# maksimt/rri_nmf

Hardware: NVIDIA B200
Metric: RRI sweeps/sec (higher is better)
Workload: dtype f32/tf32-mma

## Files before the change

### rri_nmf_b200/csrc/api.cu

```cuda
#include <dlfcn.h>
#include <stdarg.h>
#include <stdio.h>
#include <string.h>

#include <string>
#include <vector>

#include "../../include/rri_b200.h"
#include "gemm_tf32_sm100.h"
#include "common.cuh"
#include "devmem.h"
#include "kernels.h"
#include "wrri_tc_sm100.h"

using namespace rri;

static thread_local char g_err[1024] = "";
static int fail(const char* fmt, ...)
{
    va_list ap;
    va_start(ap, fmt);
    vsnprintf(g_err, sizeof(g_err), fmt, ap);
    va_end(ap);
    return 1;
}
#define CK(call)                                                                                \
    do {                                                                                        \
        cudaError_t e_ = (call);                                                                \
        if (e_ != cudaSuccess)                                                                  \
            return fail("%s failed: %s (%s:%d)", #call, cudaGetErrorString(e_), __FILE__, __LINE__); \
    } while (0)
#define CKL() CK(cudaGetLastError())

extern "C" const char* rri_last_error(void) { return g_err; }
extern "C" const char* rri_version(void) { return "rri_b200 0.1 (sm_100a; tcgen05 tf32 + simt f32/f64)"; }

struct Id128 { char b[128]; };
struct NcclApi {
    void* lib = nullptr;
    int (*AllReduce)(const void*, void*, size_t, int, int, void*, cudaStream_t) = nullptr;
    int (*GetUniqueId)(void*) = nullptr;
    int (*CommInitRank)(void**, int,  Id128, int) = nullptr;
    int (*CommDestroy)(void*) = nullptr;
    const char* (*GetErrorString)(int) = nullptr;
};
static NcclApi g_nccl;

static int nccl_load(const char* path)
{
    if (g_nccl.lib) return 0;
    void* lib = nullptr;
    if (path && *path) lib = dlopen(path, RTLD_NOW | RTLD_GLOBAL);
    if (!lib) lib = dlopen("libnccl.so.2", RTLD_NOW | RTLD_GLOBAL);
    if (!lib) return fail("cannot load NCCL (%s): %s", path ? path : "libnccl.so.2", dlerror());
    g_nccl.AllReduce = (decltype(g_nccl.AllReduce))dlsym(lib, "ncclAllReduce");
    g_nccl.GetUniqueId = (decltype(g_nccl.GetUniqueId))dlsym(lib, "ncclGetUniqueId");
    g_nccl.CommInitRank = (decltype(g_nccl.CommInitRank))dlsym(lib, "ncclCommInitRank");
    g_nccl.CommDestroy = (decltype(g_nccl.CommDestroy))dlsym(lib, "ncclCommDestroy");
    g_nccl.GetErrorString = (decltype(g_nccl.GetErrorString))dlsym(lib, "ncclGetErrorString");
    if (!g_nccl.AllReduce || !g_nccl.GetUniqueId || !g_nccl.CommInitRank || !g_nccl.CommDestroy)
        return fail("NCCL symbols missing in %s", path ? path : "libnccl.so.2");
    g_nccl.lib = lib;
    return 0;
}
#define NCK(call)                                                                                \
    do {                                                                                         \
        int r_ = (call);                                                                         \
        if (r_ != 0)                                                                             \
            return fail("%s failed: %s", #call, g_nccl.GetErrorString ? g_nccl.GetErrorString(r_) : "?"); \
    } while (0)

extern "C" int rri_nccl_unique_id(char id_out[128], const char* nccl_lib_path)
{
    if (nccl_load(nccl_lib_path)) return 1;
    NCK(g_nccl.GetUniqueId(id_out));
    return 0;
}
extern "C" int rri_nccl_comm_create(void** comm_out, const char id[128], int32_t rank, int32_t world,
                                    int32_t device, const char* nccl_lib_path)
{
    if (nccl_load(nccl_lib_path)) return 1;
    CK(cudaSetDevice(device));
    Id128 u;
    memcpy(u.b, id, 128);
    NCK(g_nccl.CommInitRank(comm_out, world, u, rank));
    return 0;
}
extern "C" int rri_nccl_comm_destroy(void* comm)
{
    if (!g_nccl.lib) return fail("NCCL not loaded");
    NCK(g_nccl.CommDestroy(comm));
    return 0;
}

struct PeerGroup {
    bool used = false;
    int device = -1, world = 0, rank = 0;
    void* xbuf = nullptr; size_t bytes = 0;
    void* peer_base[16] = {nullptr}; bool peer_open[16] = {false};
    char handles[16 * 64] = {0};
    bool mapped = false;
    unsigned epoch = 0;
};


struct rri_handle_s {
    int64_t n = 0, d = 0;
    int k = 0, dtype = 0, math = 0, order = 0, device = 0, sm_count = 148;
    size_t es = 4;
    const void* X = nullptr; int64_t ldx = 0;
    const void* M = nullptr; int mk = 0; int64_t ldm = 0;
    void* comm = nullptr; int rank = 0, world = 1;
    void* xbuf = nullptr; size_t xbuf_bytes = 0, xslot_elems = 0;
    size_t x_off_tt = 0, x_off_tk = 0, x_off_tsum = 0, x_off_flags = 0;
    int64_t ldtk = 0;
    void* peer_base[16] = {nullptr}; bool peer_open[16] = {false};
    void* Tt_own = nullptr;
    unsigned epoch = 0;
    bool p2p = false, peer_mapped = false;
    int* p2p_err = nullptr;
    char handles[16 * 64] = {0};
    PeerGroup parked; bool have_parked = false;
    unsigned* counters = nullptr;
    std::vector<void*> allocs;
    int64_t ws_bytes = 0, launches = 0;
    PassPlan pp{};
    int hb = 0, gbw = 0;
    void *ypart = nullptr, *ppart = nullptr, *gpart = nullptr, *hpart = nullptr, *stat = nullptr;
    void *Xt = nullptr; int64_t ldxt = 0, ldwt = 0;
    void* Xt_ext = nullptr; int64_t ldxt_ext = 0;
    bool x16 = false; int x_exp = 0;
    void *X16 = nullptr, *Xt16 = nullptr; int64_t ldx16 = 0, ldxt16 = 0;
    void* F16 = nullptr;
    unsigned *x16_scan = nullptr, *f16_part = nullptr; int* f16_exp = nullptr;
    void *Wt = nullptr, *Tt = nullptr, *Cpart = nullptr, *cg = nullptr , *Hm = nullptr;
    void *gram_part = nullptr, *colsum_part = nullptr;
    int splits_t = 1, splits_w = 1, ub_blocks_t = 1, ub_blocks_w = 1, gchunks_w = 1, gchunks_t = 1;
    double* sx_slots = nullptr;
    Tf32Gemm* tf32 = nullptr;
    bool fixT_cached = false;
    TilePlan tpl{}, wpl{};
    void *numer_part = nullptr, *denom_part = nullptr, *mstat = nullptr;
    WrriTc* wtc = nullptr; int wtc_groups_t = 1, wtc_groups_w = 1;
    bool sparse = false; int64_t nnz = 0;
    SpSide csr{}, csc{};
    void *sp_quad = nullptr;
    void *sp_told = nullptr;
    void *sp_wold = nullptr;
    void *sp_npart = nullptr, *sp_dpart = nullptr;
    uint32_t* sp_perm = nullptr;
    int sp_ldt = 0;
    bool sp_refresh_v2 = true;
    bool sp_batched_sums = true;
    int* sp_err = nullptr;
    bool zero_csr = false;
    SpmmPlan zrow{}, zcol{};
    SparsePassPlan spp{};
    bool spmm_planned = false;
    void* spmm_slots = nullptr; int spmm_slot_w = 0;
    double* sums = nullptr;
    int* flags = nullptr;
    double *obj_part = nullptr, *obj_out = nullptr;
    int oblocks = 1;
    bool xsq_valid = false, c2_valid = false;
    void* Gobj = nullptr;
};

static int ws_alloc(rri_handle_t h, void** p, size_t bytes)
{
    if (bytes == 0) bytes = 16;
    CK(cached_malloc(p, bytes));
    CK(cudaMemsetAsync(*p, 0, bytes, 0));
    h->allocs.push_back(*p);
    h->ws_bytes += (int64_t)bytes;
    return 0;
}

static void ws_release(rri_handle_t h, void* p, size_t bytes)
{
    if (bytes == 0) bytes = 16;
    for (size_t i = 0; i < h->allocs.size(); ++i)
        if (h->allocs[i] == p) { h->allocs.erase(h->allocs.begin() + (long)i); break; }
    cached_free(p);
    h->ws_bytes -= (int64_t)bytes;
}

extern "C" int rri_create(rri_handle_t* out, int64_t n_local, int64_t d, int32_t k, int32_t dtype,
                          int32_t math, int32_t order, int32_t device)
{
    if (!out) return fail("null handle pointer");
    if (n_local <= 0 || d <= 0) return fail("n_local and d must be positive (got %lld, %lld)", (long long)n_local, (long long)d);
    if (k <= 0 || k > 256) return fail("k must be in [1,256] (got %d)", k);
    if (dtype != RRI_F32 && dtype != RRI_F64) return fail("bad dtype %d", dtype);
    if (order != RRI_ORDER_RRI && order != RRI_ORDER_HALS) return fail("bad order %d", order);
    if (math != RRI_MATH_IEEE && math != RRI_MATH_TF32) return fail("bad math %d", math);
    if (math == RRI_MATH_TF32 && dtype != RRI_F32) return fail("TF32 math needs f32 data");
    int ndev = 0;
    cudaError_t e = cudaGetDeviceCount(&ndev);
    if (e != cudaSuccess || ndev == 0)
        return fail("no CUDA device available (%s); this library has no CPU fallback", cudaGetErrorString(e));
    if (device < 0 || device >= ndev) return fail("bad device %d", device);
    CK(cudaSetDevice(device));
    cudaDeviceProp prop;
    CK(cudaGetDeviceProperties(&prop, device));
    if (prop.major != 10)
        return fail("device %d is sm_%d%d; this build contains sm_100a code only", device, prop.major, prop.minor);
    rri_handle_t h = new rri_handle_s();
    h->n = n_local; h->d = d; h->k = k; h->dtype = dtype; h->math = math; h->order = order;
    h->device = device; h->sm_count = prop.multiProcessorCount;
    h->es = dtype == RRI_F32 ? 4 : 8;
    if (ws_alloc(h, (void**)&h->sums, sizeof(double) * 2 * k) || ws_alloc(h, (void**)&h->flags, sizeof(int) * 4) ||
        ws_alloc(h, (void**)&h->counters, sizeof(unsigned) * 8)) {
        rri_destroy(h);
        return 1;
    }
    cudaStreamSynchronize(0);
    *out = h;
    return 0;
}

static void peer_release(rri_handle_t h);

extern "C" int rri_destroy(rri_handle_t h)
{
    if (!h) return 0;
    cudaSetDevice(h->device);
    cudaDeviceSynchronize();
    peer_release(h);
    for (void* p : h->allocs) cached_free(p);
    if (h->tf32) tf32_gemm_destroy(h->tf32);
    if (h->wtc) wrri_tc_destroy(h->wtc);
    delete h;
    return 0;
}

extern "C" int rri_set_comm(rri_handle_t h, void* nccl_comm, int32_t rank, int32_t world, const char* nccl_lib_path)
{
    if (!h) return fail("null handle");
    if (world > 1) {
        if (!nccl_comm) return fail("world > 1 needs a communicator");
        if (nccl_load(nccl_lib_path)) return 1;
    }
    h->comm = nccl_comm; h->rank = rank; h->world = world;
    return 0;
}

static size_t round_up(size_t v, size_t a) { return (v + a - 1) / a * a; }

static PeerGroup g_groups[64];

static PeerGroup* group_take(int device, size_t bytes)
{
    for (PeerGroup& g : g_groups)
        if (g.used && g.device == device && g.bytes == bytes) { g.used = false; return &g; }
    return nullptr;
}
static PeerGroup* group_slot()
{
    for (PeerGroup& g : g_groups) if (!g.used) return &g;
    return nullptr;
}

static bool peer_rank_supported(rri_handle_t h)
{
    return h->dtype == RRI_F32 ? h->k <= 128 : h->k <= 64;
}

extern "C" int rri_peer_export(rri_handle_t h, char handle_out[64])
{
    if (!h) return fail("null handle");
    if (!h->X) return fail("rri_bind has not been called");
    if (h->order != RRI_ORDER_HALS || h->mk != MK_NONE) return fail("the peer-memory exchange serves unmasked hals handles");
    if (h->zero_csr) return fail("the peer-memory exchange serves dense data; zero-filled sparse handles use the NCCL all-reduce");
    if (!peer_rank_supported(h)) return fail("the fused peer-memory T update supports k <= 128 (f32) / 64 (f64)");
    CK(cudaSetDevice(h->device));
    if (!h->xbuf) {
        const size_t es = h->es;
        const int64_t v = 16 / (int64_t)es;
        h->ldtk = (h->d + v - 1) / v * v;
        h->xslot_elems = ((size_t)h->d * h->k + (size_t)h->k * h->k + 63) / 64 * 64;
        h->x_off_tt = round_up(2 * h->xslot_elems * es, 256);
        h->x_off_tk = round_up(h->x_off_tt + (size_t)h->d * h->k * es, 256);
        h->x_off_tsum = round_up(h->x_off_tk + (size_t)h->k * h->ldtk * es, 256);
        h->x_off_flags = round_up(h->x_off_tsum + (size_t)16 * h->k * es, 256);
        h->xbuf_bytes = h->x_off_flags + 2 * 16 * 32 * sizeof(unsigned);
        if (PeerGroup* g = group_take(h->device, h->xbuf_bytes)) {
            h->xbuf = g->xbuf;
// ... 60 lines not shown
    if (!h->xbuf) return;
    if (h->have_parked) {
        if (PeerGroup* g = group_slot()) { *g = h->parked; g->used = true; h->xbuf = nullptr; h->have_parked = false; return; }
    }
    PeerGroup* g = group_slot();
    if (g) {
        g->used = true; g->device = h->device; g->world = h->world; g->rank = h->rank;
        g->xbuf = h->xbuf; g->bytes = h->xbuf_bytes; g->mapped = h->peer_mapped; g->epoch = h->epoch;
        for (int r = 0; r < 16; ++r) { g->peer_base[r] = h->peer_base[r]; g->peer_open[r] = h->peer_open[r]; }
        memcpy(g->handles, h->handles, sizeof(g->handles));
    } else {
        for (int r = 0; r < 16; ++r)
            if (h->peer_open[r] && h->peer_base[r]) cudaIpcCloseMemHandle(h->peer_base[r]);
        cudaFree(h->xbuf);
    }
    h->xbuf = nullptr; h->peer_mapped = false;
    for (int r = 0; r < 16; ++r) { h->peer_open[r] = false; h->peer_base[r] = nullptr; }
}

extern "C" int rri_peer_close(rri_handle_t h)
{
    if (!h) return fail("null handle");
    CK(cudaSetDevice(h->device));
    h->p2p = false;
    if (h->Tt_own) { h->Tt = h->Tt_own; h->Tt_own = nullptr; }
    peer_release(h);
    return 0;
}

extern "C" int rri_peer_enable(rri_handle_t h, int32_t on)
{
    if (!h) return fail("null handle");
    if (on && !h->peer_mapped) return fail("rri_peer_import has not succeeded on this rank");
    h->p2p = on != 0;
    if (h->p2p) {
        if (!h->Tt_own) h->Tt_own = h->Tt;
        h->Tt = (char*)h->xbuf + h->x_off_tt;
    } else if (h->Tt_own) {
        h->Tt = h->Tt_own; h->Tt_own = nullptr;
    }
    return 0;
}

static void peer_row_range(int64_t d, int world, int r, int64_t& lo, int64_t& hi)
{
    const int64_t nb = (d + 127) / 128;
    const int64_t q = nb / world, rem = nb % world;
    const int64_t b0 = q * r + (r < rem ? r : rem), b1 = b0 + q + (r < rem ? 1 : 0);
    lo = b0 * 128 < d ? b0 * 128 : d;
    hi = b1 * 128 < d ? b1 * 128 : d;
}

static PeerExchange peer_args(rri_handle_t h, unsigned epoch)
{
    PeerExchange px;
    memset(&px, 0, sizeof(px));
    px.world = h->world; px.rank = h->rank; px.epoch = epoch; px.ldtk = h->ldtk; px.err = h->p2p_err;
    peer_row_range(h->d, h->world, h->rank, px.row_lo, px.row_hi);
    const int b = (int)(epoch & 1u);
    for (int r = 0; r < h->world; ++r) {
        char* base = (char*)h->peer_base[r];
        px.part[r] = base + (size_t)b * h->xslot_elems * h->es;
        px.Tt[r] = base + h->x_off_tt;
        px.Tk[r] = base + h->x_off_tk;
        px.tsum[r] = base + h->x_off_tsum;
        px.flag1[r] = (unsigned*)(base + h->x_off_flags);
        px.flag2[r] = (unsigned*)(base + h->x_off_flags) + 16 * 32;
    }
    return px;
}

static int allreduce(rri_handle_t h, void* buf, size_t count, cudaStream_t st)
{
    if (h->world <= 1) return 0;
    NCK(g_nccl.AllReduce(buf, buf, count, h->dtype == RRI_F32 ? 7 : 8,  0, h->comm, st));
    h->launches++;
    return 0;
}

static int alloc_halfstep_ws(rri_handle_t h)
{
    const int64_t n = h->n, d = h->d;
    const int k = h->k;
    const size_t es = h->es;
    const size_t a = (size_t)h->splits_w * n * k, b = (size_t)h->splits_t * d * k;
    if (ws_alloc(h, &h->Cpart, es * (a > b ? a : b))) return 1;
    const int64_t m = n > d ? n : d;
    if (ws_alloc(h, &h->cg, es * ((size_t)m * k + (size_t)k * k))) return 1;
    if (ws_alloc(h, &h->Hm, es * (size_t)k * k)) return 1;
    {
        const int64_t v = 16 / (int64_t)es;
        h->ldwt = (n + v - 1) / v * v;
    }
    if (ws_alloc(h, &h->Wt, es * (size_t)k * h->ldwt) || ws_alloc(h, &h->Tt, es * (size_t)d * k)) return 1;
    h->gchunks_w = gram_chunks(n, k, h->sm_count);
    h->gchunks_t = gram_chunks(d, k, h->sm_count);
    const int gc = h->gchunks_w > h->gchunks_t ? h->gchunks_w : h->gchunks_t;
    if (ws_alloc(h, &h->gram_part, es * (size_t)gc * k * k)) return 1;
    h->ub_blocks_w = update_rows_blocks(n, h->sm_count);
    h->ub_blocks_t = update_rows_blocks(d, h->sm_count);
    int ubm = h->ub_blocks_w > h->ub_blocks_t ? h->ub_blocks_w : h->ub_blocks_t;
    {
        const int pb = peer_update_blocks(d, h->sm_count);
        if (pb > ubm) ubm = pb;
    }
    if (ws_alloc(h, &h->colsum_part, es * (size_t)ubm * k)) return 1;
    if (h->order == RRI_ORDER_HALS && ws_alloc(h, (void**)&h->sx_slots, sizeof(double) * (size_t)simplex_T_slots(d))) return 1;
    return 0;
}

template <typename T>
static int bind_impl(rri_handle_t h, cudaStream_t st)
{
    const int64_t n = h->n, d = h->d;
    const int k = h->k, ks = k + 1;
    const size_t es = sizeof(T);
    h->oblocks = obj_blocks(n, d, h->sm_count);
    if (!h->obj_part) {
        size_t op = 2 * (size_t)(h->oblocks > 256 ? h->oblocks : 256);
        if (op < (size_t)8 * h->sm_count) op = (size_t)8 * h->sm_count;
        if (ws_alloc(h, (void**)&h->obj_part, sizeof(double) * op)) return 1;
        if (ws_alloc(h, (void**)&h->obj_out, sizeof(double) * 16)) return 1;
    }
    if (h->mk != MK_NONE) {
        if (!h->numer_part) {
            h->tpl = plan_tstats(n, d, h->sm_count);
            h->wpl = plan_wstats(n, d, h->sm_count);
            size_t a = (size_t)h->tpl.groups * d, b = (size_t)h->wpl.groups * n;
            if (h->math == RRI_MATH_TF32) {
                std::string err;
                h->wtc = wrri_tc_create(h->sm_count, n, d, k, err);
                if (!h->wtc) return fail("tensor-core WRRI path unavailable: %s", err.c_str());
                h->wtc_groups_t = wrri_tc_groups(h->wtc, 0);
                h->wtc_groups_w = wrri_tc_groups(h->wtc, 1);
                const size_t a2 = (size_t)h->wtc_groups_t * d, b2 = (size_t)h->wtc_groups_w * n;
                if (a2 > a) a = a2;
                if (b2 > b) b = b2;
            }
            const size_t m = a > b ? a : b;
            if (ws_alloc(h, &h->numer_part, es * m) || ws_alloc(h, &h->denom_part, es * m)) return 1;
            if (ws_alloc(h, &h->mstat, es * 2 * (size_t)d)) return 1;
        }
        return 0;
    }
    if (!h->Cpart) {
        h->splits_w = simt_gemm_splits(n, d, h->sm_count);
        h->splits_t = simt_gemm_splits(d, n, h->sm_count);
        if (h->math == RRI_MATH_TF32) { h->splits_w = 1; h->splits_t = 1; }
        if (alloc_halfstep_ws(h)) return 1;
        if (h->math == RRI_MATH_TF32) {
            std::string err;
            h->tf32 = tf32_gemm_create(h->sm_count, k + 16 < 256 ? k + 16 : 256, err);
            if (!h->tf32) return fail("tf32 contraction unavailable: %s", err.c_str());
            if (ws_alloc(h, (void**)&h->x16_scan, 4 * sizeof(unsigned)) || ws_alloc(h, (void**)&h->f16_exp, sizeof(int)) ||
                ws_alloc(h, (void**)&h->f16_part, sizeof(unsigned) * (size_t)f16_factor_parts(h->sm_count)))
                return 1;
            CK(cudaStreamSynchronize(0));
        }
    }
    if (h->order == RRI_ORDER_HALS) {
        const int64_t v = 16 / (int64_t)es;
        h->ldxt = (n + v - 1) / v * v;
        const int64_t ldx16 = (d + 7) / 8 * 8, ldxt16 = (n + 7) / 8 * 8;
        const size_t bytes16 = 2 * ((size_t)n * ldx16 + (size_t)d * ldxt16);
        size_t cap;
        if (h->Xt_ext) {
            if (h->ldxt_ext < h->ldxt || h->ldxt_ext % v != 0 || (reinterpret_cast<uintptr_t>(h->Xt_ext) & 15) != 0)
                return fail("caller-provided X' storage needs a 16-byte aligned base and a row stride >= %lld, multiple of %lld",
                            (long long)h->ldxt, (long long)v);
            h->Xt = h->Xt_ext; h->ldxt = h->ldxt_ext;
            cap = es * (size_t)d * h->ldxt;
        } else {
            cap = es * (size_t)d * h->ldxt > bytes16 ? es * (size_t)d * h->ldxt : bytes16;
            if (!h->Xt) {
                CK(cached_malloc(&h->Xt, cap));
                h->allocs.push_back(h->Xt);
                h->ws_bytes += (int64_t)cap;
            }
        }
        const char* ev = getenv("RRI_X16");
        h->x16 = false;
        if (h->math == RRI_MATH_TF32 && !(ev && *ev == '0') && bytes16 <= cap) {
            launch_x16_scan((const float*)h->X, n, d, h->ldx, h->x16_scan, h->sm_count, st);
            h->launches++;
            unsigned scan[3];
            CK(cudaMemcpyAsync(scan, h->x16_scan, sizeof(scan), cudaMemcpyDeviceToHost, st));
            CK(cudaStreamSynchronize(st));
            h->x16 = x16_exponent(scan, &h->x_exp);
        }
        if (h->x16) {
            if (!h->F16) {
                const int64_t m = n > d ? n : d;
                const int rows = k + 16 < 256 ? k + 16 : 256;
                if (ws_alloc(h, &h->F16, 2 * (size_t)rows * (size_t)((m + 7) / 8 * 8))) return 1;
                CK(cudaStreamSynchronize(0));
            }
            h->X16 = h->Xt; h->ldx16 = ldx16;
            h->Xt16 = (char*)h->Xt + 2 * (size_t)n * ldx16; h->ldxt16 = ldxt16;
            launch_x16_copy((const float*)h->X, n, d, h->ldx, h->x_exp, h->X16, ldx16, h->Xt16, ldxt16, st);
        } else {
            launch_transpose<T>((const T*)h->X, n, d, h->ldx, (T*)h->Xt, h->ldxt, st);
        }
        h->launches++;
        CKL();
    } else {
        h->pp = plan_pass(n, d, h->ldx, h->X, (int)es, h->sm_count);
        h->hb = tstep_blocks(d);
        h->gbw = wstep_blocks(n, h->sm_count);
        if (!h->ypart) {
            if (ws_alloc(h, &h->ypart, es * (size_t)h->pp.ct * n)) return 1;
            if (ws_alloc(h, &h->ppart, es * (size_t)h->pp.rg * d)) return 1;
            if (ws_alloc(h, &h->gpart, es * (size_t)h->gbw * ks)) return 1;
            if (ws_alloc(h, &h->hpart, es * (size_t)h->hb * ks)) return 1;
            if (ws_alloc(h, &h->stat, es * (size_t)(d + ks))) return 1;
        }
    }
    return 0;
}

extern "C" int rri_set_transpose_storage(rri_handle_t h, void* Xt_dev, int64_t ldXt)
{
    if (!h) return fail("null handle");
    if (h->X) return fail("rri_set_transpose_storage must be called before rri_bind");
    h->Xt_ext = Xt_dev; h->ldxt_ext = ldXt;
    return 0;
}

extern "C" int rri_bind(rri_handle_t h, const void* X_dev, int64_t ldX, const void* mask_dev,
                        int32_t mask_kind, int64_t ldM, void* stream)
{
    if (!h) return fail("null handle");
    if (!X_dev) return fail("X is null");
    if (ldX < h->d) return fail("ldX (%lld) < d (%lld)", (long long)ldX, (long long)h->d);
    if (mask_kind != RRI_MASK_NONE && !mask_dev) return fail("mask kind %d without a mask pointer", mask_kind);
    if (mask_kind != RRI_MASK_NONE && ldM < h->d) return fail("ldM < d");
    if (mask_kind < 0 || mask_kind > 2) return fail("bad mask kind %d", mask_kind);
    if (h->sparse) return fail("this handle is bound to observed-entries (CSR) data; create a new one for dense data");
    if (h->zero_csr) return fail("this handle is bound to zero-filled sparse (CSR) data; create a new one for dense data");
    if (h->X && ((h->mk != MK_NONE) != (mask_kind != RRI_MASK_NONE)))
        return fail("a handle cannot switch between masked and unmasked data; create a new one");
    CK(cudaSetDevice(h->device));
    h->X = X_dev; h->ldx = ldX;
    h->M = mask_kind == RRI_MASK_NONE ? nullptr : mask_dev;
    h->mk = mask_kind; h->ldm = ldM;
    h->fixT_cached = false;
    h->xsq_valid = false; h->c2_valid = false;
    cudaStream_t st = (cudaStream_t)stream;
    int rc = h->dtype == RRI_F32 ? bind_impl<float>(h, st) : bind_impl<double>(h, st);
    if (rc) return rc;
    CK(cudaStreamSynchronize(0));
    return 0;
}

template <typename T>
static int bind_csr_impl(rri_handle_t h, const int64_t* rowptr, const int32_t* col, const T* val, const T* wgt,
                         cudaStream_t st)
{
    const int64_t n = h->n, d = h->d, nnz = h->nnz;
    const int k = h->k;
    const size_t es = sizeof(T);
    const int64_t m = n > d ? n : d;
    const size_t ne = (size_t)(nnz > 0 ? nnz : 1);
    void *E_csr = nullptr, *E_csc = nullptr, *x_csc = nullptr, *w_csc = nullptr, *csc_row = nullptr, *colptr = nullptr;
    if (ws_alloc(h, (void**)&h->obj_part, sizeof(double) * 2 * 256) || ws_alloc(h, (void**)&h->obj_out, sizeof(double) * 8)) return 1;
    if (ws_alloc(h, &E_csr, es * ne) || ws_alloc(h, &E_csc, es * ne) || ws_alloc(h, &x_csc, es * ne)) return 1;
    if (wgt && ws_alloc(h, &w_csc, es * ne)) return 1;
    if (ws_alloc(h, &csc_row, sizeof(int32_t) * ne) || ws_alloc(h, &colptr, sizeof(int64_t) * (size_t)(d + 1))) return 1;
    if (ws_alloc(h, &h->sp_quad, 4 * es * (size_t)m) || ws_alloc(h, &h->sp_told, es * 2 * (size_t)d) ||
        ws_alloc(h, &h->sp_wold, es * 2 * (size_t)n) || ws_alloc(h, &h->mstat, es * 2 * (size_t)m) ||
        ws_alloc(h, (void**)&h->sp_err, sizeof(int)))
        return 1;
    {
        const int64_t v = 16 / (int64_t)es;
        h->ldwt = (n + v - 1) / v * v;
    }
    {
        const char* env = getenv("RRI_SP_REFRESH_V2");
        h->sp_refresh_v2 = !(env && *env == '0');
        const char* envb = getenv("RRI_SP_BATCHED_SUMS");
        h->sp_batched_sums = !(envb && *envb == '0');
        const int v = 16 / (int)es;
        h->sp_ldt = h->sp_refresh_v2 ? (k + v - 1) / v * v : k;
    }
    if (ws_alloc(h, &h->Wt, es * (size_t)k * h->ldwt) || ws_alloc(h, &h->Tt, es * (size_t)d * h->sp_ldt)) return 1;
    if (ws_alloc(h, (void**)&h->sp_perm, sizeof(uint32_t) * ne)) return 1;
    CK(cudaStreamSynchronize(0));
    const int rc = sp_build_csc<T>(rowptr, col, val, wgt, n, d, nnz, (int64_t*)colptr, (int32_t*)csc_row, (T*)x_csc,
                                   (T*)w_csc, h->sp_perm, h->sm_count, h->sp_err, st);
    if (rc < 0)
        return fail("malformed CSR input:%s%s%s", (-rc & 1) ? " rowptr is not a monotone [0..nnz] sequence;" : "",
                    (-rc & 2) ? " column index outside [0,d);" : "",
                    (-rc & 4) ? " column indices must be strictly ascending inside every row (sort and merge duplicates);" : "");
    if (rc > 0) return fail("building the column orientation failed: %s", cudaGetErrorString((cudaError_t)rc));
    h->csr = SpSide{n, rowptr, col, val, wgt, E_csr, nnz / n >= 512 ? 256 : 32, nullptr, 1, 0, d, nullptr};
    h->csc = SpSide{d, (const int64_t*)colptr, (const int32_t*)csc_row, x_csc, w_csc, E_csc, nnz / d >= 512 ? 256 : 32,
                    nullptr, 1, 0, n, nullptr};
    h->launches += 8;
    const char* env = getenv("RRI_SP_BLOCKED");
    const bool blocked = !(env && *env == '0');
    const char* env16 = getenv("RRI_SP_IDX16");
    const bool use16 = !(env16 && *env16 == '0');
    size_t part_elems = (size_t)m;
    for (SpSide* sd : {&h->csr, &h->csc}) {
        int nblk = 1;
        const int nb = sp_block_len((int)es, sd->nother, &nblk);
        if (!blocked || nblk > 64) continue;
        void* p2 = nullptr;
        void* i16 = nullptr;
        if (ws_alloc(h, &p2, sizeof(int64_t) * (size_t)sd->nseg * (size_t)(nblk + 1))) return 1;
        if (use16 && ws_alloc(h, &i16, sizeof(uint16_t) * ne)) return 1;
        CK(cudaStreamSynchronize(0));
        launch_sp_subptr(sd->ptr, sd->idx, sd->nseg, nblk, nb, (int64_t*)p2, h->sm_count, st);
        if (use16 && nnz > 0) {
            launch_sp_local_index(sd->idx, nnz, nb, (uint16_t*)i16, h->sm_count, st);
            sd->idx16 = (const uint16_t*)i16;
            h->launches++;
        }
        sd->ptr2 = (const int64_t*)p2; sd->nblk = nblk; sd->nb = nb;
        if ((size_t)nblk * (size_t)sd->nseg > part_elems) part_elems = (size_t)nblk * (size_t)sd->nseg;
        h->launches++;
    }
    if (ws_alloc(h, &h->sp_npart, es * part_elems) || ws_alloc(h, &h->sp_dpart, es * part_elems)) return 1;
    CK(cudaStreamSynchronize(0));
    CKL();
    CK(cudaStreamSynchronize(st));
    return 0;
}

extern "C" int rri_bind_csr(rri_handle_t h, int64_t nnz, const int64_t* rowptr_dev, const int32_t* col_dev,
                            const void* val_dev, const void* weight_dev, void* stream)
{
    if (!h) return fail("null handle");
    if (h->X) return fail("the handle is already bound; create a new one");
    if (nnz < 0 || nnz >= ((int64_t)1 << 31)) return fail("nnz must be in [0, 2^31) (got %lld)", (long long)nnz);
    if (!rowptr_dev) return fail("rowptr is null");
    if (nnz > 0 && (!col_dev || !val_dev)) return fail("col/val is null");
    if (h->math == RRI_MATH_TF32) return fail("the observed-entries path has no contraction: create the handle with RRI_MATH_IEEE");
    CK(cudaSetDevice(h->device));
    h->nnz = nnz;
    cudaStream_t st = (cudaStream_t)stream;
    const int rc = h->dtype == RRI_F32
                       ? bind_csr_impl<float>(h, rowptr_dev, col_dev, (const float*)val_dev, (const float*)weight_dev, st)
                       : bind_csr_impl<double>(h, rowptr_dev, col_dev, (const double*)val_dev, (const double*)weight_dev, st);
    if (rc) return rc;
    h->sparse = true;
    h->mk = MK_SPARSE;
    h->X = val_dev ? val_dev : (const void*)rowptr_dev;
// ... 141 lines not shown
            CK(cudaStreamSynchronize(0));
            h->spmm_slot_w = pw;
        }
        pl.slots = h->spmm_slots;
    }
    launch_spmm<T>(pl, B, ldb, width, C, ldc, st);
    h->launches += (width + SPMM_PANEL - 1) / SPMM_PANEL;
    CKL();
    return 0;
}

extern "C" int rri_spmm(rri_handle_t h, int32_t transpose, const void* B_dev, int64_t ldb, void* C_dev, int64_t ldc,
                        int32_t width, void* stream)
{
    if (!h) return fail("null handle");
    if (!h->X) return fail("rri_bind_csr / rri_bind_csr_zero has not been called");
    if (!h->sparse && !h->zero_csr)
        return fail("rri_spmm serves sparse handles (rri_bind_csr or rri_bind_csr_zero); this handle holds dense data");
    if (transpose != 0 && transpose != 1) return fail("transpose must be 0 or 1 (got %d)", transpose);
    if (width < 1) return fail("width must be at least 1 (got %d)", width);
    if (!B_dev || !C_dev) return fail("B and C must not be null");
    if (ldb < width || ldc < width)
        return fail("ldb and ldc must be at least width = %d (got %lld, %lld)", width, (long long)ldb, (long long)ldc);
    if (ldb >= ((int64_t)1 << 31) || ldc >= ((int64_t)1 << 31)) return fail("ldb and ldc must be below 2^31");
    if (((uintptr_t)B_dev % h->es) || ((uintptr_t)C_dev % h->es))
        return fail("B and C must be aligned to their %d-byte elements", (int)h->es);
    CK(cudaSetDevice(h->device));
    cudaStream_t st = (cudaStream_t)stream;
    return h->dtype == RRI_F32 ? spmm_impl<float>(h, transpose, (const float*)B_dev, ldb, (float*)C_dev, ldc, width, st)
                               : spmm_impl<double>(h, transpose, (const double*)B_dev, ldb, (double*)C_dev, ldc, width, st);
}

static SolveArgs solve_args(const rri_params_t* p, bool forT)
{
    SolveArgs a;
    a.reg_l1 = forT ? p->reg_t_l1 : p->reg_w_l1;
    a.reg_l2 = forT ? p->reg_t_l2 : p->reg_w_l2;
    a.eps = p->eps;
    const double ub = forT ? p->ub_t : p->ub_w;
    a.has_ub = ub > 0 ? 1 : 0;
    a.ub = ub > 0 ? ub : 0.0;
    return a;
}

static int check_params(rri_handle_t h, const rri_params_t* p)
{
    if (!p) return fail("null params");
    if (!h->X) return fail("rri_bind has not been called");
    if (p->fix_W && p->fix_T) return fail("fix_W and fix_T both set: nothing to update");
    if (p->fix_W) return fail("fix_W=True is not supported on the device path (the reference's T-only sweep also rescales W, nmf.py:450-452)");
    if (p->simplex_T && !(p->ub_t > 0)) return fail("simplex_T needs t_row_sum > 0");
    return 0;
}

template <typename T>
static void rri_pass(rri_handle_t h, const T* tvec, const T* W, int tn, bool do_y, bool do_p, cudaStream_t st)
{
    if (h->zero_csr)
        launch_sparse_rri_pass<T>(h->spp, h->zrow, h->zcol, tvec, W, h->k, tn, (T*)h->ypart, (T*)h->ppart, do_y, do_p, st);
    else
        launch_rri_pass<T>((const T*)h->X, h->ldx, h->n, h->d, tvec, W, h->k, tn, (T*)h->ypart, (T*)h->ppart, do_y, do_p,
                           h->pp, st);
    h->launches++;
}

template <typename T>
static int rri_prologue(rri_handle_t h, T* W, int t0, const rri_params_t* p, cudaStream_t st)
{
    rri_pass<T>(h, nullptr, W, t0, false, true, st);
    launch_rri_wstep<T>(W, h->n, h->k, 0, t0, (const T*)h->ypart, h->pp.ct, h->n, (const T*)h->hpart, h->hb,
                        solve_args(p, false), (T*)h->gpart, h->sums, h->flags, false, h->gbw, st);
    h->launches++;
    CKL();
    return 0;
}

template <typename T>
static int rri_finish(rri_handle_t h, int t_last, cudaStream_t st)
{
    if (h->world > 1) {
        launch_reduce_stat<T>((const T*)h->ppart, 0, 0, (const T*)h->gpart, h->gbw, h->k, (T*)h->stat, st);
        if (allreduce(h, h->stat, (size_t)(h->k + 1), st)) return 1;
        launch_finalize_sums<T>((const T*)h->stat, 1, h->k, t_last, h->sums, h->flags, st);
        h->launches += 2;
    } else {
        launch_finalize_sums<T>((const T*)h->gpart, h->gbw, h->k, t_last, h->sums, h->flags, st);
        h->launches++;
    }
    CKL();
    return 0;
}

template <typename T>
static int rri_topic_range(rri_handle_t h, T* W, T* Tm, int t0, int t1, bool first_has_prev,
                           const rri_params_t* p, cudaStream_t st)
{
    const int k = h->k;
    const int64_t n = h->n, d = h->d;
    const SolveArgs at = solve_args(p, true), aw = solve_args(p, false);
    for (int t = t0; t < t1; ++t) {
        const int tn = (t + 1) % k;
        const int t_prev = ((t == t0 && !first_has_prev) || k == 1) ? -1 : (t + k - 1) % k;
        const T* pp = (const T*)h->ppart; int rg = h->pp.rg;
        const T* gp = (const T*)h->gpart; int gb = h->gbw;
        if (h->world > 1) {
            launch_reduce_stat<T>(pp, rg, d, gp, gb, k, (T*)h->stat, st);
            h->launches++;
            if (allreduce(h, h->stat, (size_t)(d + k + 1), st)) return 1;
            pp = (const T*)h->stat; rg = 1;
            gp = (const T*)h->stat + d; gb = 1;
        }
        launch_rri_tstep<T>(Tm, d, k, t, pp, rg, d, gp, gb, at, (T*)h->hpart, h->sums, t_prev, h->flags, true, st);
        if (p->simplex_T) {
            launch_project_rows_simplex<T>(Tm + (int64_t)t * d, 1, d, p->ub_t, st);
            launch_rri_tstep<T>(Tm, d, k, t, pp, rg, d, gp, gb, at, (T*)h->hpart, h->sums, -1, h->flags, false, st);
            h->launches += 2;
        }
        rri_pass<T>(h, Tm + (int64_t)t * d, W, tn, true, k > 1, st);
        launch_rri_wstep<T>(W, n, k, t, tn, (const T*)h->ypart, h->pp.ct, n, (const T*)h->hpart, h->hb, aw,
                            (T*)h->gpart, h->sums, h->flags, true, h->gbw, st);
        h->launches += 2;
        if (k == 1) {
            if (rri_finish<T>(h, 0, st)) return 1;
            if (rri_prologue<T>(h, W, 0, p, st)) return 1;
        }
    }
    CKL();
    return 0;
}

template <typename T>
static int contraction(rri_handle_t h, const T* A, int64_t lda, const T* B, int64_t ldb, T* Cpart,
                       int64_t M, int N, int64_t K, int splits, cudaStream_t st, T* G = nullptr)
{
    if (h->math == RRI_MATH_TF32) {
        std::string err;
        int nl = tf32_gemm_run(h->tf32, (const float*)A, lda, (const float*)B, ldb, (float*)Cpart, N, M, N, K, st, err,
                               G ? (const float*)B : nullptr, ldb, G ? N : 0, (float*)G, N);
        if (nl < 0) return fail("tf32 contraction failed: %s", err.c_str());
        h->launches += nl;
    } else {
        launch_simt_gemm_nt<T>(A, lda, B, ldb, Cpart, M, N, K, splits, st);
        h->launches++;
    }
    return 0;
}

static bool gram_in_contraction(rri_handle_t h)
{
    static const bool off = [] { const char* e = getenv("RRI_TC_GRAM"); return e && *e == '0'; }();
    return h->math == RRI_MATH_TF32 && !off;
}

template <typename T>
static int data_contraction(rri_handle_t h, bool transpose, const T* B, int64_t ldb, int N, T* C, cudaStream_t st,
                            T* G = nullptr, bool convert = true)
{
    const int64_t M = transpose ? h->d : h->n, K = transpose ? h->n : h->d;
    if (!h->x16)
        return transpose ? contraction<T>(h, (const T*)h->Xt, h->ldxt, B, ldb, C, M, N, K, h->splits_t, st, G)
                         : contraction<T>(h, (const T*)h->X, h->ldx, B, ldb, C, M, N, K, h->splits_w, st, G);
    const int64_t ldf = (K + 7) / 8 * 8;
    if (convert) {
        launch_f16_factor((const float*)B, N, K, ldb, h->f16_part, f16_factor_parts(h->sm_count), h->F16, ldf, h->f16_exp, st);
        h->launches += 2;
    }
    const __half* F = (const __half*)h->F16;
    std::string err;
    const int nl = f16_gemm_run(h->tf32, (const __half*)(transpose ? h->Xt16 : h->X16), transpose ? h->ldxt16 : h->ldx16,
                                h->x_exp, F, ldf, h->f16_exp, (float*)C, N, M, N, K, st, err, G ? F : nullptr, ldf, G ? N : 0,
                                (float*)G, N);
    if (nl < 0) return fail("16-bit contraction failed: %s", err.c_str());
    h->launches += nl;
    return 0;
}

template <typename T>
static int hals_W_half(rri_handle_t h, T* W, const T* Tk, int64_t ldtk, const rri_params_t* p, bool recompute, cudaStream_t st)
{
    const int k = h->k;
    const int64_t n = h->n, d = h->d;
    if (recompute) {
        const bool tc_gram = gram_in_contraction(h);
        if (!tc_gram) { launch_gram<T>((const T*)h->Tt, d, k, (T*)h->gram_part, h->gchunks_t, (T*)h->Hm, st); h->launches += 2; }
        if (h->zero_csr) {
            launch_spmm<T>(h->zrow, (const T*)h->Tt, k, k, (T*)h->Cpart, k, st);
            h->launches++;
        } else if (data_contraction<T>(h, false, Tk, ldtk, k, (T*)h->Cpart, st, tc_gram ? (T*)h->Hm : nullptr)) {
            return 1;
        }
    }
    const int parts = h->math == RRI_MATH_TF32 ? 1 : h->splits_w;
    launch_update_rows<T>(W, n, k, (const T*)h->Cpart, parts, n * k, nullptr, (const T*)h->Hm, solve_args(p, false),
                          (T*)h->Wt, h->ldwt, (T*)h->colsum_part, h->flags, h->ub_blocks_w,
                          ColsumOut{nullptr, k, 0, h->counters + 0}, st);
    h->launches++;
    CKL();
    return 0;
}

template <typename T>
static int hals_T_half(rri_handle_t h, T* W, T* Tk, int64_t ldtk, const rri_params_t* p, cudaStream_t st)
{
    const int k = h->k;
    const int64_t n = h->n, d = h->d;
    T* cg = (T*)h->cg;
    T* G = cg + (size_t)d * k;
    const bool tc_gram = gram_in_contraction(h);
    const int psplits = h->math == RRI_MATH_TF32 ? 1 : h->splits_t;
    if (h->world > 1 && h->p2p && !p->simplex_T) {
        const unsigned e = ++h->epoch;
        const int b = (int)(e & 1u);
        T* myC = (T*)((char*)h->xbuf + (size_t)b * h->xslot_elems * h->es);
        T* myG = myC + (size_t)d * k;
        if (!tc_gram) { launch_gram<T>(W, n, k, (T*)h->gram_part, h->gchunks_w, myG, st); h->launches += 2; }
        T* Cdst = psplits == 1 ? myC : (T*)h->Cpart;
        if (data_contraction<T>(h, true, (const T*)h->Wt, h->ldwt, k, Cdst, st, tc_gram ? myG : nullptr)) return 1;
        if (psplits > 1) { launch_reduce_parts<T>((const T*)h->Cpart, psplits, d * k, d * k, myC, st); h->launches++; }
        const PeerExchange px = peer_args(h, e);
        const int blocks = peer_update_blocks(px.row_hi - px.row_lo, h->sm_count);
        const int nl = launch_peer_update_rows<T>(px, d, k, solve_args(p, true), G, (T*)h->colsum_part, h->flags, h->sums,
                                                  h->counters + 1, blocks, st);
        if (!nl) return fail("the fused peer-memory T update does not support k = %d", k);
        h->launches += nl;
        CKL();
        return 0;
    }
    if (!tc_gram) { launch_gram<T>(W, n, k, (T*)h->gram_part, h->gchunks_w, G, st); h->launches += 2; }
    T* Cout = (h->world > 1 && psplits == 1) ? cg : (T*)h->Cpart;
    if (h->zero_csr) {
        launch_spmm<T>(h->zcol, W, k, k, Cout, k, st);
        h->launches++;
    } else if (data_contraction<T>(h, true, (const T*)h->Wt, h->ldwt, k, Cout, st, tc_gram ? G : nullptr)) {
        return 1;
    }
    const T* C = Cout;
    int parts = psplits;
    if (h->world > 1) {
        if (psplits > 1) { launch_reduce_parts<T>(C, parts, d * k, d * k, cg, st); h->launches++; }
        if (allreduce(h, cg, (size_t)d * k + (size_t)k * k, st)) return 1;
        C = cg; parts = 1;
    }
    if (p->simplex_T) {
        const char* e = getenv("RRI_SIMPLEX_FUSED");
        int nl = 0;
        const int rc = launch_simplex_T_update<T>((T*)h->Tt, d, k, C, parts, d * k, G, solve_args(p, true), p->ub_t, Tk,
                                                  ldtk, h->sx_slots, h->flags, h->sm_count, !(e && *e == '0'), &nl, st);
        if (rc) return fail("constrained T update failed: %s", cudaGetErrorString((cudaError_t)rc));
        h->launches += nl;
        return 0;
    }
    launch_update_rows<T>((T*)h->Tt, d, k, C, parts, d * k, nullptr, G, solve_args(p, true), Tk, ldtk, (T*)h->colsum_part,
                          h->flags, h->ub_blocks_t, ColsumOut{nullptr, 0, 0, h->counters + 2}, st);
    h->launches++;
    CKL();
    return 0;
}

template <typename T>
static int hals_finish_sums(rri_handle_t h, const T* Tm, bool t_sums, cudaStream_t st)
{
    launch_rowsum_flag<T>((const T*)h->Wt, h->k, h->n, h->ldwt, h->sums, h->k, h->world > 1 ? 0 : 2, h->flags, st);
    h->launches++;
    if (t_sums) {
        launch_rowsum_flag<T>(Tm, h->k, h->d, h->d, h->sums, 0, 1, h->flags, st);
        h->launches++;
    }
    if (h->world <= 1) return 0;
    NCK(g_nccl.AllReduce(h->sums + h->k, h->sums + h->k, (size_t)h->k, 8, 0, h->comm, st));
    launch_flag_from_sums(h->sums, h->k, h->k, 2, h->flags, st);
    h->launches += 2;
    return 0;
}

template <typename T>
static void scale_row_to_sum(rri_handle_t h, T* row, T* row2, int64_t ld2, int t, const rri_params_t* p, cudaStream_t st)
{
    launch_vec_scale_to_sum<T>(row, h->d, 1, h->sums, t, p->ub_t, st);
    if (row2) { launch_vec_scale_to_sum<T>(row2, h->d, ld2, h->sums, t, p->ub_t, st); h->launches++; }
    launch_vec_sum_flag<T>(row, h->d, 1, h->sums, t, 1, h->flags, st);
    h->launches += 2;
}

template <typename T>
static int wrri_T_step(rri_handle_t h, T* W, T* Tm, int t, const rri_params_t* p, cudaStream_t st)
{
    const int64_t n = h->n, d = h->d;
    int parts = h->tpl.groups;
    if (h->wtc) {
        std::string err;
        parts = h->wtc_groups_t;
        if (wrri_tc_stats(h->wtc, 0, (const float*)h->X, h->ldx, h->M, h->mk, h->ldm, t, (const float*)Tm + (int64_t)t * d, (float*)h->numer_part,
                          (float*)h->denom_part, parts, st, err) < 0)
            return fail("tensor-core WRRI T statistics failed: %s", err.c_str());
    } else {
        launch_wrri_tstats<T>((const T*)h->X, h->ldx, h->M, h->mk, h->ldm, W, Tm, n, d, h->k, t, (T*)h->numer_part,
                              (T*)h->denom_part, h->tpl, st);
    }
    h->launches++;
    const T* nu = (const T*)h->numer_part; const T* de = (const T*)h->denom_part;
    if (h->world > 1) {
        T* ms = (T*)h->mstat;
        launch_reduce_parts<T>(nu, parts, d, d, ms, st);
        launch_reduce_parts<T>(de, parts, d, d, ms + d, st);
        h->launches += 2;
        if (allreduce(h, ms, (size_t)2 * d, st)) return 1;
        nu = ms; de = ms + d; parts = 1;
    }
    T* tp2 = h->wtc ? (T*)wrri_tc_Tp(h->wtc) + t : nullptr;
    launch_wrri_final<T>(nu, de, parts, d, solve_args(p, true), Tm + (int64_t)t * d, 1, tp2,
                         h->wtc ? wrri_tc_KP(h->wtc) : 0, h->flags, st);
    launch_vec_sum_flag<T>(Tm + (int64_t)t * d, d, 1, h->sums, t, p->simplex_T ? 0 : 1, h->flags, st);
    h->launches += 2;
    if (p->simplex_T) scale_row_to_sum<T>(h, Tm + (int64_t)t * d, tp2, h->wtc ? wrri_tc_KP(h->wtc) : 0, t, p, st);
    return 0;
}

template <typename T>
static int wrri_W_step(rri_handle_t h, T* W, T* Tm, int t, const rri_params_t* p, cudaStream_t st)
{
    const int64_t n = h->n, d = h->d;
    int parts = h->wpl.groups;
    if (h->wtc) {
        std::string err;
        parts = h->wtc_groups_w;
        if (wrri_tc_stats(h->wtc, 1, (const float*)h->X, h->ldx, h->M, h->mk, h->ldm, t, (const float*)Tm + (int64_t)t * d, (float*)h->numer_part,
                          (float*)h->denom_part, parts, st, err) < 0)
            return fail("tensor-core WRRI W statistics failed: %s", err.c_str());
    } else {
        launch_wrri_wstats<T>((const T*)h->X, h->ldx, h->M, h->mk, h->ldm, W, Tm, n, d, h->k, t, (T*)h->numer_part,
                              (T*)h->denom_part, h->wpl, st);
    }
    T* wp2 = h->wtc ? (T*)wrri_tc_Wp(h->wtc) + t : nullptr;
    launch_wrri_final<T>((const T*)h->numer_part, (const T*)h->denom_part, parts, n, solve_args(p, false),
                         W + t, h->k, wp2, h->wtc ? wrri_tc_KP(h->wtc) : 0, h->flags, st);
    launch_vec_sum_flag<T>(W + t, n, h->k, h->sums, h->k + t, h->world > 1 ? 0 : 2, h->flags, st);
    h->launches += 3;
    if (h->world > 1) {
        NCK(g_nccl.AllReduce(h->sums + h->k + t, h->sums + h->k + t, 1, 8, 0, h->comm, st));
        launch_flag_from_sums(h->sums, h->k + t, 1, 2, h->flags, st);
        h->launches += 2;
    }
    return 0;
}

struct SpPending {
    const void *wo = nullptr, *wn = nullptr, *to = nullptr, *tn = nullptr;
};
struct SpState {
    SpPending csr, csc;
    int ct = 0, cw = 0;
    const void* told_cur = nullptr;
};

template <typename T>
static void sp_refresh(rri_handle_t h, bool need_csr, bool need_csc, const T* W, cudaStream_t st)
{
    if (h->sp_refresh_v2) {
        launch_sp_residual_rows<T>(h->csr, W, h->k, (const T*)h->Tt, h->sp_ldt, h->k, h->sm_count, st);
        h->launches++;
        if (need_csc && h->nnz > 0) {
            launch_sp_gather<T>(h->sp_perm, (const T*)h->csr.E, (T*)h->csc.E, h->nnz, h->sm_count, st);
            h->launches++;
        }
        return;
    }
    if (need_csc) { launch_sp_residual<T>(h->csc, (const T*)h->Tt, W, h->k, h->sm_count, st); h->launches++; }
    if (need_csr) { launch_sp_residual<T>(h->csr, W, (const T*)h->Tt, h->k, h->sm_count, st); h->launches++; }
}

template <typename T>
static int sp_T_step(rri_handle_t h, T* W, T* Tm, int t, const rri_params_t* p, SpState& S, cudaStream_t st)
{
    const int64_t n = h->n, d = h->d;
    const T* wt = (const T*)h->Wt + (int64_t)t * h->ldwt;
    T* trow = Tm + (int64_t)t * d;
    T* told = (T*)h->sp_told + (int64_t)(S.ct & 1) * d;
    T* ms = (T*)h->mstat;
    launch_sp_pack<T>((const T*)S.csc.wo, (const T*)S.csc.wn, wt, wt, h->sp_quad, n, st);
    const T* nu = (const T*)h->sp_npart; const T* de = (const T*)h->sp_dpart;
    int parts = launch_sp_pass<T>(h->csc, h->sp_quad, (const T*)S.csc.to, (const T*)S.csc.tn, trow, told, (T*)h->sp_npart,
                                  (T*)h->sp_dpart, h->sm_count, st);
    h->launches += 2;
    if (h->world > 1) {
        launch_reduce_parts<T>(nu, parts, d, d, ms, st);
        launch_reduce_parts<T>(de, parts, d, d, ms + d, st);
        h->launches += 2;
        if (allreduce(h, ms, (size_t)2 * d, st)) return 1;
        nu = ms; de = ms + d; parts = 1;
    }
    launch_wrri_final<T>(nu, de, parts, d, solve_args(p, true), trow, 1, (T*)h->Tt + t, h->sp_ldt, h->flags, st);
    h->launches++;
    if (!h->sp_batched_sums || p->simplex_T) {
        launch_vec_sum_flag<T>(trow, d, 1, h->sums, t, p->simplex_T ? 0 : 1, h->flags, st);
        h->launches++;
    }
    if (p->simplex_T) scale_row_to_sum<T>(h, trow, (T*)h->Tt + t, h->sp_ldt, t, p, st);
    S.csc = SpPending{wt, wt, told, trow};
    S.told_cur = told;
    S.ct++;
    return 0;
}

template <typename T>
static int sp_W_step(rri_handle_t h, T* W, T* Tm, int t, const rri_params_t* p, SpState& S, cudaStream_t st)
{
    const int64_t n = h->n, d = h->d;
    T* wt = (T*)h->Wt + (int64_t)t * h->ldwt;
    const T* trow = Tm + (int64_t)t * d;
    const T* told = S.told_cur ? (const T*)S.told_cur : trow;
    T* wold = (T*)h->sp_wold + (int64_t)(S.cw & 1) * n;
    launch_sp_pack<T>((const T*)S.csr.to, (const T*)S.csr.tn, told, trow, h->sp_quad, d, st);
    const int parts = launch_sp_pass<T>(h->csr, h->sp_quad, (const T*)S.csr.wo, (const T*)S.csr.wn, wt, wold,
                                        (T*)h->sp_npart, (T*)h->sp_dpart, h->sm_count, st);
    launch_wrri_final<T>((const T*)h->sp_npart, (const T*)h->sp_dpart, parts, n, solve_args(p, false), W + t, h->k, wt, 1,
                         h->flags, st);
    h->launches += 3;
    if (!h->sp_batched_sums) {
        launch_vec_sum_flag<T>(wt, n, 1, h->sums, h->k + t, h->world > 1 ? 0 : 2, h->flags, st);
        h->launches++;
        if (h->world > 1) {
            NCK(g_nccl.AllReduce(h->sums + h->k + t, h->sums + h->k + t, 1, 8, 0, h->comm, st));
            launch_flag_from_sums(h->sums, h->k + t, 1, 2, h->flags, st);
            h->launches += 2;
        }
    }
    S.csr = SpPending{wold, wt, told, trow};
    if (S.told_cur) S.csc = S.csr;
    S.told_cur = nullptr;
    S.cw++;
    return 0;
}

template <typename T>
static int sp_topic_sums(rri_handle_t h, const T* Tm, int t0, int t1, bool did_T, bool did_W, cudaStream_t st)
{
    if (!h->sp_batched_sums) return 0;
    if (did_T) { launch_rowsum_flag<T>(Tm + (int64_t)t0 * h->d, t1 - t0, h->d, h->d, h->sums, t0, 1, h->flags, st); h->launches++; }
    if (did_W) {
        launch_rowsum_flag<T>((const T*)h->Wt + (int64_t)t0 * h->ldwt, t1 - t0, h->n, h->ldwt, h->sums, h->k + t0,
                              h->world > 1 ? 0 : 2, h->flags, st);
        h->launches++;
        if (h->world > 1) {
            NCK(g_nccl.AllReduce(h->sums + h->k + t0, h->sums + h->k + t0, (size_t)(t1 - t0), 8, 0, h->comm, st));
            launch_flag_from_sums(h->sums, h->k + t0, t1 - t0, 2, h->flags, st);
            h->launches += 2;
        }
    }
    return 0;
}

template <typename T>
static int sp_load_factors(rri_handle_t h, const T* W, const T* Tm, cudaStream_t st)
{
    launch_transpose<T>(Tm, h->k, h->d, h->d, (T*)h->Tt, h->sp_ldt, st);
    launch_transpose<T>(W, h->n, h->k, h->k, (T*)h->Wt, h->ldwt, st);
    h->launches += 2;
    CKL();
    return 0;
}

template <typename T>
static int sp_topic_range(rri_handle_t h, T* W, T* Tm, int t0, int t1, const rri_params_t* p, cudaStream_t st,
                          SpState* carried = nullptr, bool restart = true)
{
    SpState local;
    SpState& S = carried ? *carried : local;
    if (restart) { S = SpState(); sp_refresh<T>(h, true, true, W, st); }
    for (int t = t0; t < t1; ++t) {
        if (sp_T_step<T>(h, W, Tm, t, p, S, st)) return 1;
        if (sp_W_step<T>(h, W, Tm, t, p, S, st)) return 1;
    }
    if (sp_topic_sums<T>(h, Tm, t0, t1, true, true, st)) return 1;
    CKL();
    return 0;
}

template <typename T>
static int sp_sweeps(rri_handle_t h, T* W, T* Tm, int n_sweeps, const rri_params_t* p, cudaStream_t st)
{
    const int k = h->k;
    if (sp_load_factors<T>(h, W, Tm, st)) return 1;
    const int every = p->sp_refresh_every > 1 ? p->sp_refresh_every : 1;
    SpState carried;
    for (int s = 0; s < n_sweeps; ++s) {
        if (!p->fix_T && h->order == RRI_ORDER_RRI) {
            if (sp_topic_range<T>(h, W, Tm, 0, k, p, st, &carried, s % every == 0)) return 1;
            continue;
        }
        if (!p->fix_T) {
            SpState S;
            sp_refresh<T>(h, false, true, W, st);
            for (int t = 0; t < k; ++t) {
                if (sp_T_step<T>(h, W, Tm, t, p, S, st)) return 1;
                S.told_cur = nullptr;
            }
        }
        SpState S;
        sp_refresh<T>(h, true, false, W, st);
        for (int t = 0; t < k; ++t)
            if (sp_W_step<T>(h, W, Tm, t, p, S, st)) return 1;
        if (sp_topic_sums<T>(h, Tm, 0, k, !p->fix_T, true, st)) return 1;
    }
    CKL();
    return 0;
}

template <typename T>
static int sweeps_impl(rri_handle_t h, T* W, T* Tm, int n_sweeps, const rri_params_t* p, cudaStream_t st)
{
    const int k = h->k;
    const int64_t n = h->n, d = h->d;
    if (h->sparse) return sp_sweeps<T>(h, W, Tm, n_sweeps, p, st);
    if (h->mk != MK_NONE) {
        if (h->wtc) { wrri_tc_load_factors(h->wtc, (const float*)W, (const float*)Tm, st); h->launches += 2; }
        for (int s = 0; s < n_sweeps; ++s) {
            if (h->order == RRI_ORDER_RRI) {
                for (int t = 0; t < k; ++t) {
                    if (!p->fix_T && wrri_T_step<T>(h, W, Tm, t, p, st)) return 1;
                    if (!p->fix_W && wrri_W_step<T>(h, W, Tm, t, p, st)) return 1;
                }
            } else {
                if (!p->fix_T) for (int t = 0; t < k; ++t) if (wrri_T_step<T>(h, W, Tm, t, p, st)) return 1;
                if (!p->fix_W) for (int t = 0; t < k; ++t) if (wrri_W_step<T>(h, W, Tm, t, p, st)) return 1;
            }
        }
        CKL();
        return 0;
    }
    if (p->fix_T) {
        launch_transpose<T>(Tm, k, d, d, (T*)h->Tt, k, st);
        h->launches++;
        for (int s = 0; s < n_sweeps; ++s)
            if (hals_W_half<T>(h, W, Tm, d, p, s == 0, st)) return 1;
        return n_sweeps > 0 ? hals_finish_sums<T>(h, Tm, false, st) : 0;
    }
    if (h->order == RRI_ORDER_HALS) {
        launch_transpose<T>(Tm, k, d, d, (T*)h->Tt, k, st);
        launch_transpose<T>(W, n, k, k, (T*)h->Wt, h->ldwt, st);
        h->launches += 2;
        const bool px = h->world > 1 && h->p2p;
        T* Tk = px ? (T*)((char*)h->xbuf + h->x_off_tk) : Tm;
        const int64_t ldtk = px ? h->ldtk : d;
        if (px) CK(cudaMemcpy2DAsync(Tk, (size_t)ldtk * sizeof(T), Tm, (size_t)d * sizeof(T), (size_t)d * sizeof(T), (size_t)k,
                                     cudaMemcpyDeviceToDevice, st));
        for (int s = 0; s < n_sweeps; ++s) {
            if (hals_T_half<T>(h, W, Tk, ldtk, p, st)) return 1;
            if (hals_W_half<T>(h, W, Tk, ldtk, p, true, st)) return 1;
        }
        if (px) CK(cudaMemcpy2DAsync(Tm, (size_t)d * sizeof(T), Tk, (size_t)ldtk * sizeof(T), (size_t)d * sizeof(T), (size_t)k,
                                     cudaMemcpyDeviceToDevice, st));
        h->c2_valid = n_sweeps > 0;
        return n_sweeps > 0 ? hals_finish_sums<T>(h, Tm, !(px && !p->simplex_T), st) : 0;
    }
    if (rri_prologue<T>(h, W, 0, p, st)) return 1;
    for (int s = 0; s < n_sweeps; ++s)
        if (rri_topic_range<T>(h, W, Tm, 0, k, s > 0, p, st)) return 1;
    return k == 1 ? 0 : rri_finish<T>(h, k - 1, st);
}

static int read_flags(rri_handle_t h, int32_t* flags_host, cudaStream_t st)
{
    if (!flags_host) return 0;
    CK(cudaMemcpyAsync(flags_host, h->flags, sizeof(int), cudaMemcpyDeviceToHost, st));
    CK(cudaStreamSynchronize(st));
    return 0;
}

extern "C" int rri_sweeps(rri_handle_t h, void* W_dev, void* T_dev, int32_t n_sweeps, const rri_params_t* p,
                          int32_t* flags_host, void* stream)
{
    if (!h) return fail("null handle");
    if (!W_dev || !T_dev) return fail("W or T is null");
    if (n_sweeps < 0) return fail("n_sweeps < 0");
    if (check_params(h, p)) return 1;
    CK(cudaSetDevice(h->device));
    cudaStream_t st = (cudaStream_t)stream;
    CK(cudaMemsetAsync(h->flags, 0, sizeof(int), st));
    h->c2_valid = false;
    if (n_sweeps > 0) {
        int rc = h->dtype == RRI_F32 ? sweeps_impl<float>(h, (float*)W_dev, (float*)T_dev, n_sweeps, p, st)
                                     : sweeps_impl<double>(h, (double*)W_dev, (double*)T_dev, n_sweeps, p, st);
        if (rc) return rc;
    }
    return read_flags(h, flags_host, st);
}

template <typename T>
static int topics_impl(rri_handle_t h, T* W, T* Tm, int t0, int t1, const rri_params_t* p, cudaStream_t st)
{
    if (h->sparse) {
        if (sp_load_factors<T>(h, W, Tm, st)) return 1;
        return sp_topic_range<T>(h, W, Tm, t0, t1, p, st);
    }
    if (h->mk != MK_NONE) {
        if (h->wtc) { wrri_tc_load_factors(h->wtc, (const float*)W, (const float*)Tm, st); h->launches += 2; }
        for (int t = t0; t < t1; ++t) {
            if (wrri_T_step<T>(h, W, Tm, t, p, st)) return 1;
            if (wrri_W_step<T>(h, W, Tm, t, p, st)) return 1;
        }
        CKL();
        return 0;
    }
    if (rri_prologue<T>(h, W, t0, p, st)) return 1;
    if (rri_topic_range<T>(h, W, Tm, t0, t1, false, p, st)) return 1;
    return h->k == 1 ? 0 : rri_finish<T>(h, t1 - 1, st);
}

extern "C" int rri_topics(rri_handle_t h, void* W_dev, void* T_dev, int32_t t_begin, int32_t t_end,
                          const rri_params_t* p, int32_t* flags_host, void* stream)
{
    if (!h) return fail("null handle");
    if (!W_dev || !T_dev) return fail("W or T is null");
    if (check_params(h, p)) return 1;
    if (h->zero_csr && h->order != RRI_ORDER_RRI)
        return fail("rri_topics does not serve zero-filled sparse handles of the block order (create one with RRI_ORDER_RRI)");
    if (h->order != RRI_ORDER_RRI) return fail("rri_topics needs a handle created with RRI_ORDER_RRI");
    if (p->fix_T) return fail("rri_topics does not take fix_T");
    if (t_begin < 0 || t_end > h->k || t_begin >= t_end) return fail("bad topic range [%d,%d)", t_begin, t_end);
    CK(cudaSetDevice(h->device));
    cudaStream_t st = (cudaStream_t)stream;
    CK(cudaMemsetAsync(h->flags, 0, sizeof(int), st));
    int rc = h->dtype == RRI_F32 ? topics_impl<float>(h, (float*)W_dev, (float*)T_dev, t_begin, t_end, p, st)
                                 : topics_impl<double>(h, (double*)W_dev, (double*)T_dev, t_begin, t_end, p, st);
    if (rc) return rc;
    return read_flags(h, flags_host, st);
}

extern "C" int rri_topic_sums(rri_handle_t h, double* sum_T_host, double* sum_W_host, void* stream)
{
    if (!h) return fail("null handle");
    cudaStream_t st = (cudaStream_t)stream;
    CK(cudaSetDevice(h->device));
    if (sum_T_host) CK(cudaMemcpyAsync(sum_T_host, h->sums, sizeof(double) * h->k, cudaMemcpyDeviceToHost, st));
    if (sum_W_host) CK(cudaMemcpyAsync(sum_W_host, h->sums + h->k, sizeof(double) * h->k, cudaMemcpyDeviceToHost, st));
    CK(cudaStreamSynchronize(st));
    return 0;
}

template <typename T>
static int objective_contraction_impl(rri_handle_t h, const T* W, const T* Tm, bool reuse, cudaStream_t st);

template <typename T>
static int objective_impl(rri_handle_t h, const T* W, const T* Tm, cudaStream_t st)
{
    if (h->zero_csr) return objective_contraction_impl<T>(h, W, Tm, false, st);
    if (h->sparse) {
        launch_transpose<T>(Tm, h->k, h->d, h->d, (T*)h->Tt, h->sp_ldt, st);
        sp_refresh<T>(h, true, false, W, st);
        launch_sp_objective<T>(h->csr, h->nnz, h->obj_part, h->obj_out, st);
        launch_norms<T>(W, h->n * h->k, h->obj_part, h->obj_out + 2, st);
        launch_norms<T>(Tm, (int64_t)h->k * h->d, h->obj_part, h->obj_out + 4, st);
        h->launches += 7;
        CKL();
        return 0;
    }
    launch_objective<T>((const T*)h->X, h->ldx, h->M, h->mk, h->ldm, W, Tm, h->n, h->d, h->k, h->obj_part,
                        h->oblocks, h->obj_out, st);
    launch_norms<T>(W, h->n * h->k, h->obj_part, h->obj_out + 2, st);
    launch_norms<T>(Tm, (int64_t)h->k * h->d, h->obj_part, h->obj_out + 4, st);
    h->launches += 6;
    CKL();
    return 0;
}

extern "C" int rri_objective(rri_handle_t h, const void* W_dev, const void* T_dev, double* out_host, void* stream)
{
    if (!h) return fail("null handle");
    if (!h->X) return fail("rri_bind has not been called");
    if (!W_dev || !T_dev || !out_host) return fail("null argument");
    CK(cudaSetDevice(h->device));
    cudaStream_t st = (cudaStream_t)stream;
    int rc = h->dtype == RRI_F32 ? objective_impl<float>(h, (const float*)W_dev, (const float*)T_dev, st)
                                 : objective_impl<double>(h, (const double*)W_dev, (const double*)T_dev, st);
    if (rc) return rc;
    CK(cudaMemcpyAsync(out_host, h->obj_out, sizeof(double) * 6, cudaMemcpyDeviceToHost, st));
    CK(cudaStreamSynchronize(st));
    return 0;
}

template <typename T>
static int objective_contraction_impl(rri_handle_t h, const T* W, const T* Tm, bool reuse, cudaStream_t st)
{
    const int64_t n = h->n, d = h->d;
    const int k = h->k;
    if (!h->Gobj && ws_alloc(h, &h->Gobj, sizeof(T) * 2 * (size_t)k * k)) return 1;
    CK(cudaStreamSynchronize(0));
    double* acc = h->obj_out + 8;
    if (!h->xsq_valid) {
        if (h->zero_csr) launch_sumsq_rows<T>((const T*)h->zrow.val, 1, h->nnz, h->nnz, h->obj_part, acc, h->sm_count, st);
        else launch_sumsq_rows<T>((const T*)h->X, n, d, h->ldx, h->obj_part, acc, h->sm_count, st);
        h->xsq_valid = true;
        h->launches += 2;
// ... 82 lines not shown
        T* G = (T*)h->cg + (size_t)d * k;
        launch_spmm<T>(h->zcol, W, k, k, (T*)h->Cpart, k, st);
        launch_gram<T>(W, h->n, k, (T*)h->gram_part, h->gchunks_w, G, st);
        partials_unmasked_kernel<T><<<(unsigned)((d + 255) / 256), 256, 0, st>>>((const T*)h->Cpart + t, k, G + (size_t)t * k,
                                                                                  Tm, d, k, t, wR, nw);
        h->launches += 4;
        CKL();
        return 0;
    }
    if (h->mk != MK_NONE) {
        launch_wrri_tstats<T>((const T*)h->X, h->ldx, h->M, h->mk, h->ldm, W, Tm, h->n, d, h->k, t,
                              (T*)h->numer_part, (T*)h->denom_part, h->tpl, st);
        launch_reduce_parts<T>((const T*)h->numer_part, h->tpl.groups, d, d, wR, st);
        launch_reduce_parts<T>((const T*)h->denom_part, h->tpl.groups, d, d, nw, st);
        h->launches += 3;
    } else {
        if (h->order != RRI_ORDER_RRI) return fail("rri_partials_T (unmasked) needs a handle created with RRI_ORDER_RRI");
        if (rri_prologue<T>(h, const_cast<T*>(W), t, &p, st)) return 1;
        launch_reduce_stat<T>((const T*)h->ppart, h->pp.rg, d, (const T*)h->gpart, h->gbw, h->k, (T*)h->stat, st);
        partials_unmasked_kernel<T><<<(unsigned)((d + 255) / 256), 256, 0, st>>>((const T*)h->stat, 1, (const T*)h->stat + d,
                                                                                  Tm, d, h->k, t, wR, nw);
        h->launches += 2;
    }
    CKL();
    return 0;
}

extern "C" int rri_partials_T(rri_handle_t h, const void* W_dev, const void* T_dev, int32_t t, void* out_wR_dev,
                              void* out_nw_dev, void* stream)
{
    if (!h) return fail("null handle");
    if (!h->X) return fail("rri_bind has not been called");
    if (t < 0 || t >= h->k) return fail("bad topic %d", t);
    CK(cudaSetDevice(h->device));
    cudaStream_t st = (cudaStream_t)stream;
    return h->dtype == RRI_F32
               ? partials_impl<float>(h, (const float*)W_dev, (const float*)T_dev, t, (float*)out_wR_dev, (float*)out_nw_dev, st)
               : partials_impl<double>(h, (const double*)W_dev, (const double*)T_dev, t, (double*)out_wR_dev, (double*)out_nw_dev, st);
}

extern "C" int rri_project_rows_simplex(rri_handle_t h, void* A_dev, int64_t rows, int64_t cols, double s, void* stream)
{
    if (!h) return fail("null handle");
    if (!A_dev || rows <= 0 || cols <= 0) return fail("bad matrix");
    if (!(s > 0)) return fail("Radius s must be strictly positive");
    CK(cudaSetDevice(h->device));
    cudaStream_t st = (cudaStream_t)stream;
    if (h->dtype == RRI_F32) launch_project_rows_simplex<float>((float*)A_dev, rows, cols, s, st);
    else launch_project_rows_simplex<double>((double*)A_dev, rows, cols, s, st);
    h->launches++;
    CKL();
    return 0;
}

extern "C" int rri_cache_trim(int32_t device)
{
    CK(cudaSetDevice(device));
    cache_trim();
    for (PeerGroup& g : g_groups) {
        if (!g.used || g.device != device) continue;
        for (int r = 0; r < 16; ++r)
            if (g.peer_open[r] && g.peer_base[r]) cudaIpcCloseMemHandle(g.peer_base[r]);
        cudaFree(g.xbuf);
        g = PeerGroup();
    }
    return 0;
}

extern "C" int rri_stats(rri_handle_t h, int64_t* kernel_launches, int64_t* workspace_bytes)
{
    if (!h) return fail("null handle");
    if (kernel_launches) *kernel_launches = h->launches;
    if (workspace_bytes) *workspace_bytes = h->ws_bytes;
    return 0;
}

extern "C" int rri_x_operand_bits(rri_handle_t h, int32_t* bits)
{
    if (!h || !bits) return fail("null argument");
    *bits = h->x16 ? 16 : 8 * (int32_t)h->es;
    return 0;
}

template <typename T>
static int contract_x_impl(rri_handle_t h, bool transpose, const T* B, int64_t ldb, int N, T* C, cudaStream_t st)
{
    if (h->math == RRI_MATH_TF32) return data_contraction<T>(h, transpose, B, ldb, N, C, st);
    const int64_t M = transpose ? h->d : h->n, K = transpose ? h->n : h->d;
    launch_simt_gemm_nt<T>(transpose ? (const T*)h->Xt : (const T*)h->X, transpose ? h->ldxt : h->ldx, B, ldb, C, M, N, K, 1, st);
    h->launches++;
    return 0;
}

extern "C" int rri_contract_x(rri_handle_t h, int32_t transpose, const void* B_dev, int64_t ldb, int32_t N, void* C_dev,
                              void* stream)
{
    if (!h) return fail("null handle");
    if (!h->X) return fail("rri_bind has not been called");
    if (h->order != RRI_ORDER_HALS || h->mk != MK_NONE || !h->Xt)
        return fail("rri_contract_x needs a dense, unmasked handle created with RRI_ORDER_HALS");
    const int nmax = h->k + 16 < 256 ? h->k + 16 : 256;
    if (N < 1 || N > nmax) return fail("N must be in [1, %d] (got %d)", nmax, N);
    if (!B_dev || !C_dev || ldb < (transpose ? h->n : h->d)) return fail("bad operand");
    CK(cudaSetDevice(h->device));
    cudaStream_t st = (cudaStream_t)stream;
    const int rc = h->dtype == RRI_F32
                       ? contract_x_impl<float>(h, transpose != 0, (const float*)B_dev, ldb, N, (float*)C_dev, st)
                       : contract_x_impl<double>(h, transpose != 0, (const double*)B_dev, ldb, N, (double*)C_dev, st);
    if (rc) return rc;
    CKL();
    return 0;
}

extern "C" int rri_gemm_nt(rri_handle_t h, const void* A_dev, int64_t lda, const void* B_dev, int64_t ldb,
                           void* C_dev, int64_t ldc, int64_t M, int32_t N, int64_t K, void* stream)
{
    if (!h) return fail("null handle");
    if (N <= 0 || N > 256 || M <= 0 || K <= 0) return fail("bad shape");
    if (ldc != N) return fail("ldc must equal N");
    CK(cudaSetDevice(h->device));
    cudaStream_t st = (cudaStream_t)stream;
    if (h->math == RRI_MATH_TF32) {
        if (!h->tf32) {
            std::string err;
            h->tf32 = tf32_gemm_create(h->sm_count, N > h->k ? N : h->k, err);
            if (!h->tf32) return fail("tf32 contraction unavailable: %s", err.c_str());
        }
        std::string err;
        int nl = tf32_gemm_run(h->tf32, (const float*)A_dev, lda, (const float*)B_dev, ldb, (float*)C_dev, N, M, N, K, st, err);
        if (nl < 0) return fail("tf32 contraction failed: %s", err.c_str());
        h->launches += nl;
    } else if (h->dtype == RRI_F32) {
        launch_simt_gemm_nt<float>((const float*)A_dev, lda, (const float*)B_dev, ldb, (float*)C_dev, M, N, K, 1, st);
        h->launches++;
    } else {
        launch_simt_gemm_nt<double>((const double*)A_dev, lda, (const double*)B_dev, ldb, (double*)C_dev, M, N, K, 1, st);
        h->launches++;
    }
    CKL();
    return 0;
}

template <typename T>
static int profile_impl(rri_handle_t h, int which, const T* W, const T* Tm, int iters, float* avg_ms, cudaStream_t st)
{
    const int64_t n = h->n, d = h->d;
    const int k = h->k;
    cudaEvent_t e0, e1;
    CK(cudaEventCreate(&e0));
    CK(cudaEventCreate(&e1));
    if (which == 2 && h->mk == MK_NONE && h->order == RRI_ORDER_HALS) {
        launch_transpose<T>(W, n, k, k, (T*)h->Wt, h->ldwt, st);
        h->launches++;
    }
    if (which == 1 && h->zero_csr) {
        launch_transpose<T>(Tm, k, d, d, (T*)h->Tt, k, st);
        h->launches++;
    }
    rri_params_t prm;
    memset(&prm, 0, sizeof(prm));
    prm.eps = 1.7763568394002505e-15;
    const bool halves = which == 3 || which == 4;
    T* Tk = const_cast<T*>(Tm);
    int64_t ldtk = d;
    if (halves) {
        if (h->mk != MK_NONE || h->order != RRI_ORDER_HALS) return fail("which=3/4 need an unmasked hals-order handle");
        launch_transpose<T>(Tm, k, d, d, (T*)h->Tt, k, st);
        launch_transpose<T>(W, n, k, k, (T*)h->Wt, h->ldwt, st);
        h->launches += 2;
        if (h->world > 1 && h->p2p) {
            Tk = (T*)((char*)h->xbuf + h->x_off_tk); ldtk = h->ldtk;
            CK(cudaMemcpy2DAsync(Tk, (size_t)ldtk * sizeof(T), Tm, (size_t)d * sizeof(T), (size_t)d * sizeof(T), (size_t)k,
                                 cudaMemcpyDeviceToDevice, st));
        }
    }
    SpState spS;
    if (which == 5 || which == 6) {
        if (h->mk == MK_NONE) return fail("which=5/6 need a masked or observed-entries handle");
        prm.ub_t = 1.0;
        if (h->sparse) {
            if (sp_load_factors<T>(h, W, Tm, st)) return 1;
            sp_refresh<T>(h, true, true, W, st);
        } else if (h->wtc) {
            wrri_tc_load_factors(h->wtc, (const float*)W, (const float*)Tm, st);
            h->launches += 2;
        }
    }
    for (int it = -1; it < iters; ++it) {
        if (it == 0) CK(cudaEventRecord(e0, st));
        if (which == 5 || which == 6) {
            T* Wm = const_cast<T*>(W); T* Tw = const_cast<T*>(Tm);
            int rc;
            if (h->sparse) rc = which == 5 ? sp_T_step<T>(h, Wm, Tw, 0, &prm, spS, st) : sp_W_step<T>(h, Wm, Tw, 0, &prm, spS, st);
            else rc = which == 5 ? wrri_T_step<T>(h, Wm, Tw, 0, &prm, st) : wrri_W_step<T>(h, Wm, Tw, 0, &prm, st);
            if (rc) return 1;
            continue;
        }
        if (which == 0) {
            if (h->mk != MK_NONE || h->order != RRI_ORDER_RRI) return fail("which=0 needs an unmasked rri-order handle");
            rri_pass<T>(h, Tm, W, 1 % k, true, true, st);
        } else if (which == 1) {
            if (h->mk != MK_NONE) return fail("which=1 needs an unmasked handle");
            if (h->zero_csr) { launch_spmm<T>(h->zrow, (const T*)h->Tt, k, k, (T*)h->Cpart, k, st); h->launches++; continue; }
            if (data_contraction<T>(h, false, Tm, d, k, (T*)h->Cpart, st, nullptr, it < 0)) return 1;
        } else if (which == 2) {
            if (h->mk != MK_NONE || h->order != RRI_ORDER_HALS) return fail("which=2 needs an unmasked hals-order handle");
            if (h->zero_csr) { launch_spmm<T>(h->zcol, W, k, k, (T*)h->Cpart, k, st); h->launches++; continue; }
            if (data_contraction<T>(h, true, (const T*)h->Wt, h->ldwt, k, (T*)h->Cpart, st, nullptr, it < 0)) return 1;
        } else if (which == 3) {
            if (hals_T_half<T>(h, const_cast<T*>(W), Tk, ldtk, &prm, st)) return 1;
        } else if (which == 4) {
            if (hals_W_half<T>(h, const_cast<T*>(W), Tk, ldtk, &prm, true, st)) return 1;
        } else {
            return fail("bad kernel selector %d", which);
        }
    }
    CK(cudaEventRecord(e1, st));
    CK(cudaEventSynchronize(e1));
    float ms = 0.f;
    CK(cudaEventElapsedTime(&ms, e0, e1));
    CK(cudaEventDestroy(e0));
    CK(cudaEventDestroy(e1));
    CKL();
    *avg_ms = ms / (float)iters;
    return 0;
}

extern "C" int rri_profile_kernel(rri_handle_t h, int32_t which, const void* W_dev, const void* T_dev, int32_t iters,
                                  float* avg_ms_host, void* stream)
{
    if (!h) return fail("null handle");
    if (!h->X) return fail("rri_bind has not been called");
    if (!W_dev || !T_dev || !avg_ms_host || iters <= 0) return fail("bad argument");
    CK(cudaSetDevice(h->device));
    cudaStream_t st = (cudaStream_t)stream;
    return h->dtype == RRI_F32 ? profile_impl<float>(h, which, (const float*)W_dev, (const float*)T_dev, iters, avg_ms_host, st)
                               : profile_impl<double>(h, which, (const double*)W_dev, (const double*)T_dev, iters, avg_ms_host, st);
}
```

### rri_nmf_b200/csrc/common.cuh

```cuda
#pragma once
#include <cuda_runtime.h>
#include <stdint.h>

#define RRI_DEVINL __device__ __forceinline__

namespace rri {

constexpr int WARP = 32;

template <typename T> struct Vec;
template <> struct Vec<float>  { using type = float4;  static constexpr int N = 4; };
template <> struct Vec<double> { using type = double2; static constexpr int N = 2; };

template <typename T> RRI_DEVINL T warp_sum(T v) {
#pragma unroll
    for (int o = 16; o > 0; o >>= 1) v += __shfl_xor_sync(0xffffffffu, v, o);
    return v;
}

RRI_DEVINL float4 ld_stream(const float4* p) { return __ldcs(p); }
RRI_DEVINL double2 ld_stream(const double2* p) { return __ldcs(p); }
RRI_DEVINL float ld_stream(const float* p) { return __ldcs(p); }
RRI_DEVINL double ld_stream(const double* p) { return __ldcs(p); }

RRI_DEVINL void unpack(const float4& v, float* o) { o[0] = v.x; o[1] = v.y; o[2] = v.z; o[3] = v.w; }
RRI_DEVINL void unpack(const double2& v, double* o) { o[0] = v.x; o[1] = v.y; }

template <typename T> RRI_DEVINL T tmax(T a, T b) { return a > b ? a : b; }
template <typename T> RRI_DEVINL T tmin(T a, T b) { return a < b ? a : b; }

RRI_DEVINL void part_range(int64_t n, int parts, int p, int64_t& b, int64_t& e) {
    int64_t q = n / parts, r = n % parts;
    b = q * p + (p < r ? p : r);
    e = b + q + (p < r ? 1 : 0);
}

template <typename T>
RRI_DEVINL T solve_scalar_c(T numer, T denom, T eps, T ub, bool has_ub, bool& unbounded) {
    if (denom > T(0)) return tmax(numer, T(0)) / (denom + eps);
    if (!has_ub) { unbounded = true; return T(0); }
    return ((denom - numer) < T(0)) ? ub : T(0);
}

template <typename T>
RRI_DEVINL T solve_vector_c(T numer, T denom, T eps, T ub, bool has_ub, bool& unbounded) {
    T x = T(0);
    if (denom > T(0)) x = tmax(numer, T(0)) / (denom + eps);
    else if (denom < T(0) && !has_ub) unbounded = true;
    if (has_ub) x = tmin(x, ub);
    return x;
}

}
```

### rri_nmf_b200/csrc/gemm_tf32_sm100.cu

```cuda
#include <cuda.h>
#include <cuda_runtime.h>
#include <stdio.h>
#include <stdlib.h>

#include "devmem.h"
#include "gemm_tf32_sm100.h"
#include "tc_sm100.cuh"

namespace rri {

namespace {

constexpr int BM = 128;
constexpr int BK = 32;
constexpr int ROW_BYTES = 128;
constexpr int FLUSH = 4;
constexpr int A_TILE_BYTES = BM * ROW_BYTES;
constexpr int SMEM_LIMIT = 227 * 1024;

struct GemmParams {
    int64_t M, K;
    int N, NPAD;
    int64_t n_super, nk, units;
    int64_t n_super_main;
    float* C;
    int64_t ldc;
    float* C2;
    int64_t ldc2;
    int M2;
    float* ws;
    int* ctr;
    int stages;
    int tmem_cols;
    int nbuf;
    int flush;
    int reverse_tail;
    int a_exp;
    const int* b_exp;
};

using namespace tc;

__host__ __device__ __forceinline__ int64_t part_start(int64_t units, int parts, int64_t c)
{
    const int64_t q = units / parts, r = units % parts;
    return c * q + (c < r ? c : r);
}
__host__ __device__ __forceinline__ int64_t part_of(int64_t units, int parts, int64_t u)
{
    const int64_t q = units / parts, r = units % parts;
    if (u < r * (q + 1)) return u / (q + 1);
    return r + (u - r * (q + 1)) / q;
}

template <int MT, int NPAD, int EWQ, bool F16>
__global__ void __launch_bounds__(64 + 128 * EWQ, 1)
tf32_gemm_kernel(const __grid_constant__ CUtensorMap tmA, const __grid_constant__ CUtensorMap tmB,
                 const __grid_constant__ CUtensorMap tmA2, GemmParams p, int* err)
{
    constexpr int BKE = F16 ? 2 * BK : BK;
    constexpr int UK = F16 ? 16 : 8;
    extern __shared__ __align__(1024) uint8_t smem_raw[];
    uint8_t* smem = reinterpret_cast<uint8_t*>((reinterpret_cast<uintptr_t>(smem_raw) + 1023) & ~(uintptr_t)1023);
    constexpr int a_stage = MT * A_TILE_BYTES;
    constexpr int b_stage = NPAD * ROW_BYTES;
    uint8_t* smA = smem;
    uint8_t* smB = smem + (size_t)p.stages * a_stage;
    uint64_t* full = reinterpret_cast<uint64_t*>(smB + (size_t)p.stages * b_stage);
    uint64_t* empty = full + p.stages;
    uint64_t* tfull = empty + p.stages;
    uint64_t* tempty = tfull + 2;
    uint32_t* tmem_slot = reinterpret_cast<uint32_t*>(tempty + 2);
    int* fix_info = reinterpret_cast<int*>(tmem_slot + 1);
    const float** fix_src = reinterpret_cast<const float**>(full + 64);

    const int warp = threadIdx.x >> 5, lane = threadIdx.x & 31;
    const int64_t u_begin = part_start(p.units, gridDim.x, blockIdx.x);
    const int64_t u_end = part_start(p.units, gridDim.x, blockIdx.x + 1);

    if (warp == 0 && lane == 0) {
        prefetch_tmap(&tmA);
        prefetch_tmap(&tmB);
        if (p.n_super > p.n_super_main) prefetch_tmap(&tmA2);
        for (int s = 0; s < p.stages; ++s) { mbar_init(&full[s], 1); mbar_init(&empty[s], 1); }
        for (int b = 0; b < 2; ++b) { mbar_init(&tfull[b], 1); mbar_init(&tempty[b], 4 * EWQ); }
        fence_barrier_init();
    }
    if (warp == 1) {
        asm volatile("tcgen05.alloc.cta_group::1.sync.aligned.shared::cta.b32 [%0], %1;" ::"r"(smem_u32(tmem_slot)), "r"(p.tmem_cols) : "memory");
        asm volatile("tcgen05.relinquish_alloc_permit.cta_group::1.sync.aligned;" ::: "memory");
    }
    tc_fence_before();
    __syncthreads();
    tc_fence_after();
    const uint32_t tmem_base = *tmem_slot;

    if (warp == 0) {
        if (lane == 0) {
            const uint64_t polA = policy_evict_first(), polB = policy_evict_last();
            int stage = 0; uint32_t phase = 0;
            for (int64_t u = u_begin; u < u_end;) {
                const int64_t s = u / p.nk, kc0 = u % p.nk;
                const int64_t len = (u_end - u) < (p.nk - kc0) ? (u_end - u) : (p.nk - kc0);
                const bool down = p.reverse_tail && kc0 != 0;
                for (int64_t i = 0; i < len; ++i) {
                    const int64_t kc = down ? (kc0 + len - 1 - i) : (kc0 + i);
                    mbar_wait(&empty[stage], phase ^ 1, err, 1);
                    mbar_expect_tx(&full[stage], (uint32_t)(a_stage + b_stage));
                    if (s < p.n_super_main)
                        tma_load_2d(&tmA, smA + (size_t)stage * a_stage, &full[stage], (int)(kc * BKE), (int)(s * MT * BM), polA);
                    else
                        tma_load_2d(&tmA2, smA + (size_t)stage * a_stage, &full[stage], (int)(kc * BKE),
                                    (int)((s - p.n_super_main) * MT * BM), polB);
                    tma_load_2d(&tmB, smB + (size_t)stage * b_stage, &full[stage], (int)(kc * BKE), 0, polB);
                    if (++stage == p.stages) { stage = 0; phase ^= 1; }
                }
                u += len;
            }
        }
    } else if (warp == 1) {
        if (lane == 0) {
            const uint32_t idesc = F16 ? make_idesc_f16(BM, NPAD) : make_idesc_tf32(BM, NPAD);
            int stage = 0; uint32_t phase = 0;
            uint32_t run = 0;
            for (int64_t u = u_begin; u < u_end;) {
                const int64_t kc0 = u % p.nk;
                const int64_t len = (u_end - u) < (p.nk - kc0) ? (u_end - u) : (p.nk - kc0);
                for (int64_t i0 = 0; i0 < len; i0 += p.flush, ++run) {
                    const int64_t i1 = (i0 + p.flush) < len ? (i0 + p.flush) : len;
                    const uint32_t b = p.nbuf == 2 ? (run & 1u) : 0u;
                    const uint32_t use = p.nbuf == 2 ? (run >> 1) : run;
                    mbar_wait(&tempty[b], (use & 1u) ^ 1u, err, 2);
                    tc_fence_after();
                    const uint32_t tacc = tmem_base + b * (uint32_t)(MT * NPAD);
                    for (int64_t i = i0; i < i1; ++i) {
                        mbar_wait(&full[stage], phase, err, 3);
                        tc_fence_after();
                        const uint32_t a0 = smem_u32(smA + (size_t)stage * a_stage);
                        const uint32_t b0 = smem_u32(smB + (size_t)stage * b_stage);
#pragma unroll
                        for (int mt = 0; mt < MT; ++mt) {
#pragma unroll
                            for (int ks = 0; ks < BKE / UK; ++ks) {
                                const uint64_t ad = make_desc(a0 + mt * A_TILE_BYTES + ks * 32);
                                const uint64_t bd = make_desc(b0 + ks * 32);
                                const uint32_t accum = (i > i0 || ks > 0) ? 1u : 0u;
                                if (F16) umma_f16(tacc + (uint32_t)(mt * NPAD), ad, bd, idesc, accum);
                                else umma_tf32(tacc + (uint32_t)(mt * NPAD), ad, bd, idesc, accum);
                            }
                        }
                        umma_commit(&empty[stage]);
                        if (++stage == p.stages) { stage = 0; phase ^= 1; }
                    }
                    umma_commit(&tfull[b]);
                }
                u += len;
            }
        }
    } else {
        const int q = warp & 3;
        const int h = (warp - 2) >> 2;
        constexpr int HC = NPAD / EWQ;
        constexpr int EPI_THREADS = 128 * EWQ;
        constexpr int NACC = MT * HC;
        float acc[NACC];
        uint32_t run = 0;
        const int64_t slot_elems = (int64_t)MT * BM * p.N;
        for (int64_t u = u_begin; u < u_end;) {
            const int64_t s = u / p.nk, kc0 = u % p.nk;
            const int64_t len = (u_end - u) < (p.nk - kc0) ? (u_end - u) : (p.nk - kc0);
            const bool complete = (len == p.nk);
#pragma unroll
            for (int i = 0; i < NACC; ++i) acc[i] = 0.f;
            for (int64_t i0 = 0; i0 < len; i0 += p.flush, ++run) {
                const uint32_t b = p.nbuf == 2 ? (run & 1u) : 0u;
                const uint32_t use = p.nbuf == 2 ? (run >> 1) : run;
                mbar_wait(&tfull[b], use & 1u, err, 4);
                tc_fence_after();
                const uint32_t tacc = tmem_base + ((uint32_t)(q * 32) << 16) + b * (uint32_t)(MT * NPAD) + (uint32_t)(h * HC);
#pragma unroll
                for (int mt = 0; mt < MT; ++mt) {
#pragma unroll
                    for (int c0 = 0; c0 < HC; c0 += 16) {
                        float v[16];
                        tmem_ld16(tacc + (uint32_t)(mt * NPAD + c0), v);
#pragma unroll
                        for (int j = 0; j < 16; ++j) acc[mt * HC + c0 + j] += v[j];
                    }
                }
                tc_fence_before();
                __syncwarp();
                if (lane == 0) mbar_arrive(&tempty[b]);
            }
            const bool aux = s >= p.n_super_main;
            if (F16) {
                const float sb = __int_as_float((127 - *p.b_exp) << 23);
                const float sa = aux ? sb : __int_as_float((127 - p.a_exp) << 23);
#pragma unroll
                for (int i = 0; i < NACC; ++i) acc[i] = acc[i] * sa * sb;
            }
            float* out = aux ? p.C2 : p.C;
            const int64_t out_ld = aux ? p.ldc2 : p.ldc;
            const int64_t out_row0 = (aux ? s - p.n_super_main : s) * MT * BM;
            const int64_t out_rows = aux ? (int64_t)p.M2 : p.M;
            int c_lo = 0, c_hi = 0;
            if (!complete) {
                const int slot = (u == u_begin) ? 0 : 1;
                float* dst = p.ws + ((int64_t)blockIdx.x * 2 + slot) * slot_elems;
#pragma unroll
                for (int mt = 0; mt < MT; ++mt) {
                    const int row = mt * BM + q * 32 + lane;
#pragma unroll
                    for (int c0 = 0; c0 < HC; c0 += 4) {
                        const int col = h * HC + c0;
                        float* o = dst + (int64_t)row * p.N + col;
                        if ((col + 4 <= p.N) && ((p.N & 3) == 0)) {
                            __stcg(reinterpret_cast<float4*>(o), make_float4(acc[mt * HC + c0], acc[mt * HC + c0 + 1], acc[mt * HC + c0 + 2], acc[mt * HC + c0 + 3]));
                        } else {
#pragma unroll
                            for (int j = 0; j < 4; ++j) if (col + j < p.N) __stcg(o + j, acc[mt * HC + c0 + j]);
                        }
                    }
                }
                __threadfence();
                asm volatile("bar.sync 1, %0;" ::"n"(EPI_THREADS) : "memory");
                if (threadIdx.x == 64) {
                    const int64_t u0 = s * p.nk;
                    const int lo = (int)part_of(p.units, gridDim.x, u0), hi = (int)part_of(p.units, gridDim.x, u0 + p.nk - 1);
                    fix_info[0] = atomicAdd(p.ctr + s, 1);
                    fix_info[1] = lo; fix_info[2] = hi;
                }
                asm volatile("bar.sync 1, %0;" ::"n"(EPI_THREADS) : "memory");
                c_lo = fix_info[1]; c_hi = fix_info[2];
                if (fix_info[0] == c_hi - c_lo) {
                    __threadfence();
                    const int et = (int)threadIdx.x - 64;
                    const int64_t u0 = s * p.nk;
                    const int ncontrib = c_hi - c_lo + 1;
                    for (int i = et; i < ncontrib; i += EPI_THREADS) {
                        const int64_t cta = c_lo + i;
                        const int cslot = part_start(p.units, gridDim.x, cta) >= u0 ? 0 : 1;
                        fix_src[i] = p.ws + (cta * 2 + cslot) * slot_elems;
                    }
                    asm volatile("bar.sync 1, %0;" ::"n"(EPI_THREADS) : "memory");
                    const int64_t rows_left = out_rows - out_row0;
                    const int nvalid = (int)(rows_left < (int64_t)MT * BM ? rows_left : (int64_t)MT * BM) * p.N;
                    float* tile = out + out_row0 * out_ld;
                    if (out_ld == p.N && (p.N & 3) == 0) {
                        for (int e = et * 4; e < nvalid; e += EPI_THREADS * 4) {
                            float4 a4 = make_float4(0.f, 0.f, 0.f, 0.f);
                            for (int i = 0; i < ncontrib; ++i) {
                                const float4 v = __ldcg(reinterpret_cast<const float4*>(fix_src[i] + e));
                                a4.x += v.x; a4.y += v.y; a4.z += v.z; a4.w += v.w;
                            }
                            *reinterpret_cast<float4*>(tile + e) = a4;
                        }
                    } else {
                        for (int e = et; e < nvalid; e += EPI_THREADS) {
                            float a1 = 0.f;
                            for (int i = 0; i < ncontrib; ++i) a1 += __ldcg(fix_src[i] + e);
                            const int r = e / p.N, c = e - r * p.N;
                            tile[(int64_t)r * out_ld + c] = a1;
                        }
                    }
                    if (threadIdx.x == 64) p.ctr[s] = 0;
                }
                asm volatile("bar.sync 1, %0;" ::"n"(EPI_THREADS) : "memory");
            }
            if (complete) {
#pragma unroll
                for (int mt = 0; mt < MT; ++mt) {
                    const int64_t row = out_row0 + mt * BM + q * 32 + lane;
                    if (row < out_rows) {
#pragma unroll
                        for (int c0 = 0; c0 < HC; c0 += 4) {
                            const int col = h * HC + c0;
                            float* o = out + row * out_ld + col;
                            if ((col + 4 <= p.N) && ((out_ld & 3) == 0)) {
                                *reinterpret_cast<float4*>(o) = make_float4(acc[mt * HC + c0], acc[mt * HC + c0 + 1], acc[mt * HC + c0 + 2], acc[mt * HC + c0 + 3]);
                            } else {
#pragma unroll
                                for (int j = 0; j < 4; ++j) if (col + j < p.N) o[j] = acc[mt * HC + c0 + j];
                            }
                        }
                    }
                }
            }
            u += len;
        }
    }
    tc_fence_before();
    __syncthreads();
    if (warp == 1) {
        tc_fence_after();
        asm volatile("tcgen05.dealloc.cta_group::1.sync.aligned.b32 %0, %1;" ::"r"(tmem_base), "r"(p.tmem_cols) : "memory");
    }
}

typedef CUresult (*EncodeTiledFn)(CUtensorMap*, CUtensorMapDataType, cuuint32_t, void*, const cuuint64_t*, const cuuint64_t*,
                                  const cuuint32_t*, const cuuint32_t*, CUtensorMapInterleave, CUtensorMapSwizzle,
                                  CUtensorMapL2promotion, CUtensorMapFloatOOBfill);

}

struct Tf32Gemm {
    int sm_count = 148;
    int nmax = 0;
    EncodeTiledFn encode = nullptr;
    float* ws = nullptr;
    size_t ws_bytes = 0;
    int* err = nullptr;
    CUtensorMapDataType dtype = CU_TENSOR_MAP_DATA_TYPE_TFLOAT32;
    int force_mt = 0;
    int flush = FLUSH;
    int reverse_tail = -1;
    int* ctr = nullptr;
    size_t ctr_len = 0;
};

Tf32Gemm* tf32_gemm_create(int sm_count, int nmax, std::string& err)
{
    Tf32Gemm* g = new Tf32Gemm();
    g->sm_count = sm_count;
    g->nmax = nmax;
    void* fn = nullptr;
    cudaDriverEntryPointQueryResult qres;
    cudaError_t e = cudaGetDriverEntryPoint("cuTensorMapEncodeTiled", &fn, cudaEnableDefault, &qres);
    if (e != cudaSuccess || qres != cudaDriverEntryPointSuccess || !fn) {
        err = "cuTensorMapEncodeTiled is not available from the driver";
        delete g;
        return nullptr;
    }
    g->encode = (EncodeTiledFn)fn;
    g->ws_bytes = (size_t)sm_count * 2 * 2 * BM * (size_t)(nmax < 32 ? 32 : nmax) * sizeof(float);
    if (cached_malloc((void**)&g->ws, g->ws_bytes) != cudaSuccess || cached_malloc((void**)&g->err, sizeof(int)) != cudaSuccess) {
        err = "workspace allocation failed";
        delete g;
        return nullptr;
    }
    cudaMemset(g->err, 0, sizeof(int));
    const char* ev = getenv("RRI_TMA_F32");
    if (ev && ev[0] == '1') g->dtype = CU_TENSOR_MAP_DATA_TYPE_FLOAT32;
    const char* mt = getenv("RRI_GEMM_MT");
    if (mt) g->force_mt = atoi(mt);
    const char* rt = getenv("RRI_GEMM_REVERSE_TAIL");
    if (rt) g->reverse_tail = atoi(rt);
    const char* fl = getenv("RRI_GEMM_FLUSH");
    if (fl) g->flush = atoi(fl);
    return g;
}

void tf32_gemm_destroy(Tf32Gemm* g)
{
    if (!g) return;
    if (g->ws) cached_free(g->ws);
    if (g->err) cached_free(g->err);
    if (g->ctr) cached_free(g->ctr);
    delete g;
}

static bool encode_2d(Tf32Gemm* g, CUtensorMap* tm, const void* base, int64_t rows, int64_t cols, int64_t ld,
                      int box_rows, bool f16, std::string& err)
{
    const int es = f16 ? 2 : 4;
    if ((reinterpret_cast<uintptr_t>(base) & 15) != 0 || (ld * es) % 16 != 0) {
        err = "TMA needs 16-byte aligned rows (leading dimension a multiple of 16 bytes, base 16-byte aligned)";
        return false;
    }
    cuuint64_t gdim[2] = {(cuuint64_t)cols, (cuuint64_t)rows};
    cuuint64_t gstr[1] = {(cuuint64_t)(ld * es)};
    cuuint32_t box[2] = {(cuuint32_t)(ROW_BYTES / es), (cuuint32_t)box_rows};
    cuuint32_t estr[2] = {1, 1};
    CUresult r = g->encode(tm, f16 ? CU_TENSOR_MAP_DATA_TYPE_FLOAT16 : g->dtype, 2, const_cast<void*>(base), gdim, gstr, box,
                           estr, CU_TENSOR_MAP_INTERLEAVE_NONE,
                           CU_TENSOR_MAP_SWIZZLE_128B, CU_TENSOR_MAP_L2_PROMOTION_L2_256B, CU_TENSOR_MAP_FLOAT_OOB_FILL_NONE);
    if (r != CUDA_SUCCESS) {
        char buf[128];
        snprintf(buf, sizeof(buf), "cuTensorMapEncodeTiled failed with CUresult %d (rows=%lld cols=%lld ld=%lld box=%d)", (int)r,
                 (long long)rows, (long long)cols, (long long)ld, box_rows);
        err = buf;
        return false;
    }
    return true;
}

template <int MT, int NPAD, bool F16>
static int run_cfg(Tf32Gemm* g, const CUtensorMap& tmA, const CUtensorMap& tmB, const CUtensorMap& tmA2, GemmParams p,
                   cudaStream_t st, std::string& err)
{
    const int a_stage = MT * A_TILE_BYTES, b_stage = NPAD * ROW_BYTES;
    const int bar_bytes = 4096;
    int stages = (SMEM_LIMIT - 1024  - bar_bytes) / (a_stage + b_stage);
    if (stages > 8) stages = 8;
    if (stages < 2) { err = "not enough shared memory for two pipeline stages"; return -1; }
    p.stages = stages;
    const size_t smem = (size_t)stages * (a_stage + b_stage) + bar_bytes + 1024;
    p.nbuf = (2 * MT * NPAD <= 512) ? 2 : 1;
    int cols = 32;
    while (cols < p.nbuf * MT * NPAD) cols <<= 1;
    p.tmem_cols = cols;
    p.flush = g->flush > 0 ? (F16 ? (g->flush + 1) / 2 : g->flush) : (1 << 30);
    p.reverse_tail = g->reverse_tail >= 0 ? g->reverse_tail : (NPAD >= 128 ? 1 : 0);
    int64_t grid = p.units < g->sm_count ? p.units : g->sm_count;
    constexpr int EWQ = NPAD >= 128 ? 4 : 2;
    auto kern = tf32_gemm_kernel<MT, NPAD, EWQ, F16>;
    if (cudaFuncSetAttribute(kern, cudaFuncAttributeMaxDynamicSharedMemorySize, (int)smem) != cudaSuccess) {
        err = "cudaFuncSetAttribute(max dynamic smem) failed";
        return -1;
    }
    kern<<<(unsigned)grid, 64 + 128 * EWQ, smem, st>>>(tmA, tmB, tmA2, p, g->err);
    cudaError_t e = cudaGetLastError();
    if (e != cudaSuccess) { err = cudaGetErrorString(e); return -1; }
    return 1;
}

static int gemm_run(Tf32Gemm* g, bool f16, const void* A, int64_t lda, int a_exp, const void* B, int64_t ldb,
                    const int* b_exp, float* C, int64_t ldc, int64_t M, int N, int64_t K, cudaStream_t st, std::string& err,
                    const void* A2, int64_t lda2, int M2, float* C2, int64_t ldc2)
{
    if (!g) { err = "null contraction handle"; return -1; }
    if (N < 1 || N > 256) { err = "N must be in [1,256]"; return -1; }
    const int npad = N <= 32 ? 32 : (N <= 64 ? 64 : (N <= 128 ? 128 : 256));
    if (N > g->nmax && N > 32) { err = "N exceeds the rank this handle was created for"; return -1; }
    int mt = (M > BM) ? 2 : 1;
    if (npad == 256) mt = 1;
    if (npad <= 64 && (M + 2 * BM - 1) / (2 * BM) < g->sm_count && (int64_t)npad * K * 4 <= ((int64_t)16 << 20)) mt = 1;
    if (g->force_mt == 1 || (g->force_mt == 2 && npad < 256)) mt = g->force_mt;
    CUtensorMap tmA, tmB, tmA2;
    if (!encode_2d(g, &tmA, A, M, K, lda, mt * BM, f16, err)) return -1;
    if (!encode_2d(g, &tmB, B, N, K, ldb, npad, f16, err)) return -1;
    const bool aux = A2 != nullptr && M2 > 0 && C2 != nullptr;
    if (aux) { if (!encode_2d(g, &tmA2, A2, M2, K, lda2, mt * BM, f16, err)) return -1; }
    else tmA2 = tmA;
    GemmParams p;
    p.M = M; p.K = K; p.N = N; p.NPAD = npad;
    p.n_super_main = (M + (int64_t)mt * BM - 1) / ((int64_t)mt * BM);
    p.n_super = p.n_super_main + (aux ? (M2 + mt * BM - 1) / (mt * BM) : 0);
    const int bke = f16 ? 2 * BK : BK;
    p.nk = (K + bke - 1) / bke;
    p.units = p.n_super * p.nk;
    p.C = C; p.ldc = ldc; p.ws = g->ws;
    p.C2 = aux ? C2 : C; p.ldc2 = aux ? ldc2 : ldc; p.M2 = aux ? M2 : 0;
    if (p.n_super > (int64_t)g->ctr_len) {
        if (g->ctr) cached_free(g->ctr);
        g->ctr = nullptr; g->ctr_len = 0;
        const size_t len = (size_t)(p.n_super + 1023) / 1024 * 1024;
        if (cached_malloc((void**)&g->ctr, len * sizeof(int)) != cudaSuccess) { err = "tile counter allocation failed"; return -1; }
        if (cudaMemsetAsync(g->ctr, 0, len * sizeof(int), st) != cudaSuccess) { err = "tile counter reset failed"; return -1; }
        g->ctr_len = len;
    }
    p.ctr = g->ctr;
    p.stages = 0; p.tmem_cols = 0;
    p.nbuf = 1; p.flush = 0;
    p.a_exp = a_exp; p.b_exp = b_exp;
#define RRI_GEMM_CASE(MTv, NP)                                                                              \
    if (mt == MTv && npad == NP)                                                                            \
        return f16 ? run_cfg<MTv, NP, true>(g, tmA, tmB, tmA2, p, st, err) : run_cfg<MTv, NP, false>(g, tmA, tmB, tmA2, p, st, err)
    RRI_GEMM_CASE(2, 32); RRI_GEMM_CASE(2, 64); RRI_GEMM_CASE(2, 128);
    RRI_GEMM_CASE(1, 32); RRI_GEMM_CASE(1, 64); RRI_GEMM_CASE(1, 128); RRI_GEMM_CASE(1, 256);
#undef RRI_GEMM_CASE
    err = "no contraction kernel for this shape";
    return -1;
}

int tf32_gemm_run(Tf32Gemm* g, const float* A, int64_t lda, const float* B, int64_t ldb, float* C, int64_t ldc,
                  int64_t M, int N, int64_t K, cudaStream_t st, std::string& err, const float* A2, int64_t lda2, int M2,
                  float* C2, int64_t ldc2)
{
    return gemm_run(g, false, A, lda, 0, B, ldb, nullptr, C, ldc, M, N, K, st, err, A2, lda2, M2, C2, ldc2);
}

int f16_gemm_run(Tf32Gemm* g, const __half* A, int64_t lda, int a_exp, const __half* B, int64_t ldb, const int* b_exp,
                 float* C, int64_t ldc, int64_t M, int N, int64_t K, cudaStream_t st, std::string& err, const __half* A2,
                 int64_t lda2, int M2, float* C2, int64_t ldc2)
{
    if (!b_exp) { err = "16-bit contraction without the factor's scale"; return -1; }
    return gemm_run(g, true, A, lda, a_exp, B, ldb, b_exp, C, ldc, M, N, K, st, err, A2, lda2, M2, C2, ldc2);
}

}
```

### rri_nmf_b200/csrc/hals_kernels.cu

```cuda
#include "common.cuh"
#include "kernels.h"

namespace rri {

constexpr int G_BM = 64, G_BK = 16, G_THREADS = 256;

template <typename T, int KT>
__global__ void __launch_bounds__(G_THREADS)
simt_gemm_nt_kernel(const T* __restrict__ A, int64_t lda, const T* __restrict__ B, int64_t ldb,
                    T* __restrict__ Cpart, int64_t M, int N, int64_t K)
{
    constexpr int BN = 16 * KT;
    __shared__ T As[G_BK][G_BM + 4];
    __shared__ T Bs[G_BK][BN + 4];
    const int tid = threadIdx.x, tx = tid & 15, ty = tid >> 4;
    const int64_t m0 = (int64_t)blockIdx.x * G_BM;
    int64_t k0, k1;
    part_range((K + G_BK - 1) / G_BK, gridDim.y, blockIdx.y, k0, k1);
    k0 *= G_BK; k1 = (k1 * G_BK < K) ? k1 * G_BK : K;

    T acc[4][KT];
#pragma unroll
    for (int i = 0; i < 4; ++i)
#pragma unroll
        for (int j = 0; j < KT; ++j) acc[i][j] = T(0);

    const int arow = tid >> 2, akk = (tid & 3) * 4;
    for (int64_t kb = k0; kb < k1; kb += G_BK) {
        {
            const int64_t gm = m0 + arow;
#pragma unroll
            for (int e = 0; e < 4; ++e) {
                const int64_t gk = kb + akk + e;
                As[akk + e][arow] = (gm < M && gk < k1) ? ld_stream(A + gm * lda + gk) : T(0);
            }
        }
        for (int e = tid; e < BN * G_BK; e += G_THREADS) {
            const int row = e / G_BK, kk = e % G_BK;
            const int64_t gk = kb + kk;
            Bs[kk][row] = (row < N && gk < k1) ? B[(int64_t)row * ldb + gk] : T(0);
        }
        __syncthreads();
#pragma unroll
        for (int kk = 0; kk < G_BK; ++kk) {
            T a[4], b[KT];
#pragma unroll
            for (int i = 0; i < 4; ++i) a[i] = As[kk][ty * 4 + i];
#pragma unroll
            for (int j = 0; j < KT; ++j) b[j] = Bs[kk][tx + 16 * j];
#pragma unroll
            for (int i = 0; i < 4; ++i)
#pragma unroll
                for (int j = 0; j < KT; ++j) acc[i][j] = fma(a[i], b[j], acc[i][j]);
        }
        __syncthreads();
    }
    T* C = Cpart + (int64_t)blockIdx.y * M * N;
#pragma unroll
    for (int i = 0; i < 4; ++i) {
        const int64_t gm = m0 + ty * 4 + i;
        if (gm < M) {
#pragma unroll
            for (int j = 0; j < KT; ++j) {
                const int gn = tx + 16 * j;
                if (gn < N) C[gm * N + gn] = acc[i][j];
            }
        }
    }
}

int simt_gemm_splits(int64_t M, int64_t K, int sm_count)
{
    const int64_t tiles = (M + G_BM - 1) / G_BM;
    int64_t s = (2 * sm_count + tiles - 1) / tiles;
    const int64_t maxs = (K + 8 * G_BK - 1) / (8 * G_BK);
    if (s > maxs) s = maxs;
    if (s > 64) s = 64;
    return (int)(s < 1 ? 1 : s);
}

template <typename T>
void launch_simt_gemm_nt(const T* A, int64_t lda, const T* B, int64_t ldb, T* Cpart, int64_t M, int N,
                         int64_t K, int splits, cudaStream_t st)
{
    dim3 grid((unsigned)((M + G_BM - 1) / G_BM), splits);
    const int kt = (N + 15) / 16;
#define RRI_G_CASE(KT) simt_gemm_nt_kernel<T, KT><<<grid, G_THREADS, 0, st>>>(A, lda, B, ldb, Cpart, M, N, K)
    if (kt <= 1) RRI_G_CASE(1);
    else if (kt <= 2) RRI_G_CASE(2);
    else if (kt <= 4) RRI_G_CASE(4);
    else if (kt <= 8) RRI_G_CASE(8);
    else RRI_G_CASE(16);
#undef RRI_G_CASE
}

template <typename T>
__device__ __forceinline__ void colsum_tail(const T* __restrict__ colsum_part, int k, double* __restrict__ sums, int off,
                                            int zero_flag, int* __restrict__ flags, unsigned* __restrict__ counter)
{
    __shared__ unsigned s_arrival;
    __threadfence();
    __syncthreads();
    if (threadIdx.x == 0) s_arrival = atomicAdd(counter, 1u);
    __syncthreads();
    if (s_arrival != gridDim.x - 1) return;
    __threadfence();
    const int warp = threadIdx.x >> 5, lane = threadIdx.x & 31, nw = blockDim.x >> 5;
    for (int col = warp; col < k; col += nw) {
        T s = T(0);
        for (int b = lane; b < (int)gridDim.x; b += 32) s += __ldcg(colsum_part + (int64_t)b * k + col);
        s = warp_sum(s);
        if (lane == 0) {
            const double v = (double)s;
            sums[off + col] = v;
            if (zero_flag && !(v > 1e-10)) atomicOr(flags, zero_flag);
            if (!isfinite(v)) atomicOr(flags, 8);
        }
    }
    if (threadIdx.x == 0) *counter = 0u;
}

constexpr int U_THREADS = 256, U_NW = U_THREADS / WARP, U_GROUP = 32;

int update_rows_blocks(int64_t m, int sm_count)
{
    int64_t b = (m + 127) / 128;
    if (b > 4 * sm_count) b = 4 * sm_count;
    return (int)(b < 1 ? 1 : b);
}

template <typename T, int KL, bool S_SMEM>
__global__ void __launch_bounds__(U_THREADS)
update_rows_kernel(T* __restrict__ F, int64_t m, int k, const T* __restrict__ Cpart, int parts,
                   int64_t part_stride, const T* const* __restrict__ srcs, const T* __restrict__ S,
                   T reg_l1, T reg_l2, T eps, T ub, int has_ub,
                   T* __restrict__ Ft, int64_t ldft, T* __restrict__ colsum_part, int* __restrict__ flags,
                   double* __restrict__ sums, int sums_off, int zero_flag, unsigned* __restrict__ counter)
{
    extern __shared__ __align__(16) unsigned char smem_raw[];
    T* ftile = reinterpret_cast<T*>(smem_raw);
    T* csm = ftile + (size_t)k * (U_GROUP + 1);
    T* Ss = csm + (size_t)U_NW * k;
    const int tid = threadIdx.x, lane = tid & 31, warp = tid >> 5;
    if (S_SMEM) {
        for (int e = tid; e < k * k; e += U_THREADS) Ss[e] = S[e];
        __syncthreads();
    }
    const T* Sp = S_SMEM ? Ss : S;

    T csum[KL];
#pragma unroll
    for (int l = 0; l < KL; ++l) csum[l] = T(0);
// ... 220 lines not shown
        __syncthreads();
        {
            const int tot = nrow * k;
            int rr = tid / k, cc = tid - rr * k;
            const int dr = TPR_ROWS / k, dc = TPR_ROWS - dr * k;
            T* Frow = F + i0 * k;
            for (int e = tid; e < tot; e += TPR_ROWS) {
                Frow[e] = ftile[rr * LD + cc];
                rr += dr; cc += dc;
                if (cc >= k) { cc -= k; ++rr; }
            }
            if (tid < k) {
                T cs = T(0);
#pragma unroll 8
                for (int ii = 0; ii < nrow; ++ii) cs += ftile[ii * LD + tid];
                csum += cs;
            }
            if (Ft) {
                if (tid < nrow)
                    for (int tp = 0; tp < k; ++tp) Ft[(int64_t)tp * ldft + i0 + tid] = ftile[tid * LD + tp];
            }
        }
        __syncthreads();
    }
    if (unb) atomicOr(flags, 4);
    if (tid < k) colsum_part[(int64_t)blockIdx.x * k + tid] = csum;
    if (sums) colsum_tail<T>(colsum_part, k, sums, sums_off, zero_flag, flags, counter);
}

template <typename T, int KM>
static void launch_update_rows_tpr(T* F, int64_t m, int k, const T* Cpart, int parts, int64_t part_stride,
                                   const T* const* srcs, const T* S, const SolveArgs& a, T* Ft, int64_t ldft, T* colsum_part,
                                   int* flags, int blocks, const ColsumOut& co, cudaStream_t st)
{
    const size_t smem = sizeof(T) * ((size_t)KM * KM + 2 * (size_t)TPR_ROWS * (KM + 1));
    auto kern = update_rows_tpr_kernel<T, KM>;
    if (smem > 48 * 1024) cudaFuncSetAttribute(kern, cudaFuncAttributeMaxDynamicSharedMemorySize, (int)smem);
    kern<<<blocks, TPR_ROWS, smem, st>>>(F, m, k, Cpart, parts, part_stride, srcs, S, (T)a.reg_l1, (T)a.reg_l2,
                                        (T)a.eps, (T)a.ub, a.has_ub, Ft, ldft, colsum_part, flags, co.sums, co.off,
                                        co.zero_flag, co.counter);
}

template <typename T, int KM>
__global__ void __launch_bounds__(128)
update_rows_reg_kernel(T* __restrict__ F, int64_t m, int k, const T* __restrict__ C, const T* __restrict__ S,
                       T reg_l1, T reg_l2, T eps, T ub, int has_ub, T* __restrict__ Ft, int64_t ldft,
                       int* __restrict__ flags)
{
    using V = typename Vec<T>::type;
    constexpr int VN = Vec<T>::N;
    extern __shared__ __align__(16) unsigned char smem_raw[];
    T* Ss = reinterpret_cast<T*>(smem_raw);
    const int tid = threadIdx.x;
    for (int e = tid; e < KM * KM; e += 128) {
        const int a = e / KM, b = e % KM;
        Ss[e] = (a < k && b < k) ? S[a * k + b] : T(0);
    }
    __syncthreads();
    bool unb = false;
    for (int64_t row = (int64_t)blockIdx.x * 128 + tid; row < m; row += (int64_t)gridDim.x * 128) {
        T f[KM];
        const V* frowv = reinterpret_cast<const V*>(F + row * k);
#pragma unroll
        for (int jv = 0; jv < KM / VN; ++jv) {
            T fv[VN];
#pragma unroll
            for (int v = 0; v < VN; ++v) fv[v] = T(0);
            if (VN * jv < k) unpack(frowv[jv], fv);
#pragma unroll
            for (int v = 0; v < VN; ++v) f[VN * jv + v] = fv[v];
        }
        const V* crowv = reinterpret_cast<const V*>(C + row * k);
        constexpr int GV = 8 / VN;
        T cn[8];
#pragma unroll
        for (int v = 0; v < GV; ++v) {
            T cv[VN];
#pragma unroll
            for (int x = 0; x < VN; ++x) cv[x] = T(0);
            if (VN * v < k) unpack(crowv[v], cv);
#pragma unroll
            for (int x = 0; x < VN; ++x) cn[VN * v + x] = cv[x];
        }
#pragma unroll 1
        for (int c = 0; c < (k + 7) / 8; ++c) {
            T cc[8];
#pragma unroll
            for (int u = 0; u < 8; ++u) cc[u] = cn[u];
#pragma unroll
            for (int v = 0; v < GV; ++v) {
                const int jv = GV * (c + 1) + v;
                if (VN * jv < k) {
                    T cv[VN];
                    unpack(crowv[jv], cv);
#pragma unroll
                    for (int x = 0; x < VN; ++x) cn[VN * v + x] = cv[x];
                }
            }
#pragma unroll
            for (int u = 0; u < 8; ++u) {
                const int t = 8 * c + u;
                if (t < k) {
                    const V* srow = reinterpret_cast<const V*>(Ss + t * KM);
                    T acc[4] = {T(0), T(0), T(0), T(0)};
#pragma unroll
                    for (int jv = 0; jv < KM / VN; ++jv) {
                        T sv[VN];
                        unpack(srow[jv], sv);
#pragma unroll
                        for (int v = 0; v < VN; ++v) acc[(jv * VN + v) & 3] = fma(f[jv * VN + v], sv[v], acc[(jv * VN + v) & 3]);
                    }
                    T ft = f[u];
#pragma unroll
                    for (int jj = 1; jj < KM / 8; ++jj) ft = (jj == c) ? f[8 * jj + u] : ft;
                    const T stt = Ss[t * KM + t];
                    const T dot = ((acc[0] + acc[1]) + (acc[2] + acc[3])) - ft * stt;
                    const T x = solve_scalar_c<T>(cc[u] - dot - reg_l1, stt + reg_l2, eps, ub, has_ub != 0, unb);
#pragma unroll
                    for (int jj = 0; jj < KM / 8; ++jj) f[8 * jj + u] = (jj == c) ? x : f[8 * jj + u];
                }
            }
        }
        V* fout = reinterpret_cast<V*>(F + row * k);
#pragma unroll
        for (int jv = 0; jv < KM / VN; ++jv)
            if (VN * jv < k) {
                V o;
                T* op = reinterpret_cast<T*>(&o);
#pragma unroll
                for (int v = 0; v < VN; ++v) op[v] = f[VN * jv + v];
                fout[jv] = o;
            }
        if (Ft) {
#pragma unroll
            for (int t = 0; t < KM; ++t)
                if (t < k) Ft[(int64_t)t * ldft + row] = f[t];
        }
    }
    if (unb) atomicOr(flags, 4);
}

__device__ __forceinline__ void ffma2(unsigned long long& acc, unsigned long long a, unsigned long long b)
{
    asm("fma.rn.f32x2 %0, %1, %2, %0;" : "+l"(acc) : "l"(a), "l"(b));
}
__device__ __forceinline__ float lo_f(unsigned long long v) { return __uint_as_float((unsigned)v); }
__device__ __forceinline__ float hi_f(unsigned long long v) { return __uint_as_float((unsigned)(v >> 32)); }
__device__ __forceinline__ unsigned long long pack_f(float lo, float hi)
{
    return (unsigned long long)__float_as_uint(lo) | ((unsigned long long)__float_as_uint(hi) << 32);
}

template <int KM>
__global__ void __launch_bounds__(128)
update_rows_reg_x2_kernel(float* __restrict__ F, int64_t m, int k, const float* __restrict__ C, const float* __restrict__ S,
                          float reg_l1, float reg_l2, float eps, float ub, int has_ub, float* __restrict__ Ft, int64_t ldft,
                          int* __restrict__ flags)
{
    using U64 = unsigned long long;
    extern __shared__ __align__(16) unsigned char smem_raw[];
    float* Ss = reinterpret_cast<float*>(smem_raw);
    const int tid = threadIdx.x;
    for (int e = tid; e < KM * KM; e += 128) {
        const int a = e / KM, b = e % KM;
        Ss[e] = (a < k && b < k) ? S[a * k + b] : 0.f;
    }
    __syncthreads();
    bool unb = false;
    for (int64_t row = (int64_t)blockIdx.x * 128 + tid; row < m; row += (int64_t)gridDim.x * 128) {
        U64 fp[KM / 2];
        const ulonglong2* frowv = reinterpret_cast<const ulonglong2*>(F + row * k);
#pragma unroll
        for (int jv = 0; jv < KM / 4; ++jv) {
            ulonglong2 v = make_ulonglong2(0ull, 0ull);
            if (4 * jv < k) v = frowv[jv];
            fp[2 * jv] = v.x; fp[2 * jv + 1] = v.y;
        }
        const float4* crowv = reinterpret_cast<const float4*>(C + row * k);
        float cn[8];
#pragma unroll
        for (int v = 0; v < 2; ++v) {
            float4 cv = make_float4(0.f, 0.f, 0.f, 0.f);
            if (4 * v < k) cv = crowv[v];
            cn[4 * v] = cv.x; cn[4 * v + 1] = cv.y; cn[4 * v + 2] = cv.z; cn[4 * v + 3] = cv.w;
        }
#pragma unroll 1
        for (int c = 0; c < (k + 7) / 8; ++c) {
            float cc[8];
#pragma unroll
            for (int u = 0; u < 8; ++u) cc[u] = cn[u];
#pragma unroll
            for (int v = 0; v < 2; ++v) {
                const int jv = 2 * (c + 1) + v;
                if (4 * jv < k) {
                    const float4 cv = crowv[jv];
                    cn[4 * v] = cv.x; cn[4 * v + 1] = cv.y; cn[4 * v + 2] = cv.z; cn[4 * v + 3] = cv.w;
                }
            }
#pragma unroll
            for (int u = 0; u < 8; ++u) {
                const int t = 8 * c + u;
                if (t < k) {
                    const ulonglong2* srow = reinterpret_cast<const ulonglong2*>(Ss + t * KM);
                    U64 a01 = 0ull, a23 = 0ull;
#pragma unroll
                    for (int jv = 0; jv < KM / 4; ++jv) {
                        const ulonglong2 sv = srow[jv];
                        ffma2(a01, fp[2 * jv], sv.x);
                        ffma2(a23, fp[2 * jv + 1], sv.y);
                    }
                    U64 fpair = fp[u / 2];
#pragma unroll
                    for (int jj = 1; jj < KM / 8; ++jj) fpair = (jj == c) ? fp[4 * jj + u / 2] : fpair;
                    const float ft = (u & 1) ? hi_f(fpair) : lo_f(fpair);
                    const float stt = Ss[t * KM + t];
                    const float dot = ((lo_f(a01) + hi_f(a01)) + (lo_f(a23) + hi_f(a23))) - ft * stt;
                    const float x = solve_scalar_c<float>(cc[u] - dot - reg_l1, stt + reg_l2, eps, ub, has_ub != 0, unb);
#pragma unroll
                    for (int jj = 0; jj < KM / 8; ++jj) {
                        const U64 old = fp[4 * jj + u / 2];
                        const U64 upd = (u & 1) ? pack_f(lo_f(old), x) : pack_f(x, hi_f(old));
                        fp[4 * jj + u / 2] = (jj == c) ? upd : old;
                    }
                }
            }
        }
        ulonglong2* fout = reinterpret_cast<ulonglong2*>(F + row * k);
#pragma unroll
        for (int jv = 0; jv < KM / 4; ++jv)
            if (4 * jv < k) fout[jv] = make_ulonglong2(fp[2 * jv], fp[2 * jv + 1]);
        if (Ft) {
#pragma unroll
            for (int t = 0; t < KM; ++t)
                if (t < k) Ft[(int64_t)t * ldft + row] = (t & 1) ? hi_f(fp[t / 2]) : lo_f(fp[t / 2]);
        }
    }
    if (unb) atomicOr(flags, 4);
}

template <typename T, int KM>
static void launch_update_rows_reg(T* F, int64_t m, int k, const T* C, const T* S, const SolveArgs& a, T* Ft, int64_t ldft,
                                   int* flags, const ColsumOut& co, cudaStream_t st)
{
    const size_t smem = sizeof(T) * KM * KM;
    const int64_t nb = (m + 127) / 128;
    if constexpr (sizeof(T) == 4) {
        static const bool x2 = [] { const char* e = getenv("RRI_UPDATE_X2"); return !(e && *e == '0'); }();
        if (x2) {
            auto kx = update_rows_reg_x2_kernel<KM>;
            if (smem > 48 * 1024) cudaFuncSetAttribute(kx, cudaFuncAttributeMaxDynamicSharedMemorySize, (int)smem);
            kx<<<(unsigned)nb, 128, smem, st>>>(F, m, k, C, S, (T)a.reg_l1, (T)a.reg_l2, (T)a.eps, (T)a.ub, a.has_ub, Ft, ldft, flags);
            if (co.sums) launch_rowsum_flag<T>(Ft, k, m, ldft, co.sums, co.off, co.zero_flag, flags, st);
            return;
        }
    }
    auto kern = update_rows_reg_kernel<T, KM>;
    if (smem > 48 * 1024) cudaFuncSetAttribute(kern, cudaFuncAttributeMaxDynamicSharedMemorySize, (int)smem);
    kern<<<(unsigned)nb, 128, smem, st>>>(F, m, k, C, S, (T)a.reg_l1, (T)a.reg_l2, (T)a.eps, (T)a.ub, a.has_ub, Ft, ldft, flags);
    if (co.sums) launch_rowsum_flag<T>(Ft, k, m, ldft, co.sums, co.off, co.zero_flag, flags, st);
}

__device__ __forceinline__ void peer_flag_store(unsigned* p, unsigned v)
{
    asm volatile("st.release.sys.global.u32 [%0], %1;" ::"l"(p), "r"(v) : "memory");
}
__device__ __forceinline__ unsigned peer_flag_load(const unsigned* p)
{
    unsigned v;
    asm volatile("ld.acquire.sys.global.u32 %0, [%1];" : "=r"(v) : "l"(p) : "memory");
    return v;
}
__device__ __forceinline__ void peer_wait_all(const unsigned* flags_local, int world, unsigned epoch, int* err)
{
    const int r = threadIdx.x;
    if (r < world) {
        const long long t0 = clock64();
        while ((int)(peer_flag_load(flags_local + 32 * r) - epoch) < 0) {
            if (clock64() - t0 > 200000000000LL) {
                atomicExch(err, 1 + r);
                __trap();
            }
            __nanosleep(100);
        }
    }
}

template <typename T>
__global__ void __launch_bounds__(256)
peer_gram_kernel(PeerExchange px, int64_t d, int k, T* __restrict__ Gsum)
{
    const int tid = threadIdx.x;
    const int world = px.world, rank = px.rank;
    if (blockIdx.x == 0 && tid < world) {
        __threadfence_system();
        peer_flag_store(px.flag1[tid] + 32 * rank, px.epoch);
    }
    peer_wait_all(px.flag1[rank], world, px.epoch, px.err);
    __syncthreads();
    const int64_t goff = d * (int64_t)k;
    constexpr int GB = 4;
    const int e0 = (blockIdx.x * 256 + tid) * GB;
    if (e0 >= k * k) return;
    T v[16][GB];
#pragma unroll
    for (int r = 0; r < 16; ++r)
        if (r < world) {
            const T* Gp = reinterpret_cast<const T*>(px.part[r]) + goff;
#pragma unroll
            for (int u = 0; u < GB; ++u) v[r][u] = (e0 + u < k * k) ? __ldcg(Gp + e0 + u) : T(0);
        }
#pragma unroll
    for (int u = 0; u < GB; ++u)
        if (e0 + u < k * k) {
            T acc = T(0);
#pragma unroll
            for (int r = 0; r < 16; ++r)
                if (r < world) acc += v[r][u];
            Gsum[e0 + u] = acc;
        }
}

constexpr int PEER_ROWS = 32;
constexpr int PEER_THREADS = 128;

template <typename T, int KM>
__global__ void __launch_bounds__(PEER_THREADS)
peer_update_rows_kernel(PeerExchange px, int64_t d, int k, const T* __restrict__ Gsum, T reg_l1, T reg_l2, T eps, T ub,
                        int has_ub, T* __restrict__ colsum_part, int* __restrict__ flags, double* __restrict__ sums,
                        unsigned* __restrict__ counter)
{
    constexpr int LD = KM + 1;
    extern __shared__ __align__(16) unsigned char smem_raw[];
    T* Ss = reinterpret_cast<T*>(smem_raw);
    T* ctile = Ss + KM * KM;
    T* ftile = ctile + PEER_ROWS * LD;
    __shared__ unsigned s_arrival;
    const int tid = threadIdx.x;
    const int world = px.world, rank = px.rank;
    for (int e = tid; e < KM * KM; e += PEER_THREADS) {
        const int a = e / KM, b = e % KM;
        Ss[e] = (a < k && b < k) ? Gsum[a * k + b] : T(0);
    }
    T csum = T(0);
    bool unb = false;
    __syncthreads();
    const int64_t m = px.row_hi - px.row_lo;
    const int64_t ngroups = (m + PEER_ROWS - 1) / PEER_ROWS;
    T* Floc = reinterpret_cast<T*>(px.Tt[rank]);
    for (int64_t g = blockIdx.x; g < ngroups; g += gridDim.x) {
        const int64_t i0 = px.row_lo + g * PEER_ROWS;
        const int nrow = (int)((px.row_hi - i0) < PEER_ROWS ? (px.row_hi - i0) : PEER_ROWS);
        {
            const int tot = nrow * k;
            int rr = tid / k, cc = tid - rr * k;
            const int dr = PEER_THREADS / k, dc = PEER_THREADS - dr * k;
            const T* Frow = Floc + i0 * k;
            constexpr int UB = sizeof(T) == 8 ? 4 : 8;
            for (int e0 = tid; e0 < tot; e0 += UB * PEER_THREADS) {
                T acc[UB], fv[UB];
#pragma unroll
                for (int u = 0; u < UB; ++u) {
                    const int e = e0 + u * PEER_THREADS;
                    acc[u] = T(0);
                    fv[u] = e < tot ? Frow[e] : T(0);
                }
                for (int r0 = 0; r0 < world; r0 += 8) {
                    T cv[8][UB];
#pragma unroll
                    for (int r = 0; r < 8; ++r)
                        if (r0 + r < world) {
                            const T* Cp = reinterpret_cast<const T*>(px.part[r0 + r]) + i0 * k;
#pragma unroll
                            for (int u = 0; u < UB; ++u) {
                                const int e = e0 + u * PEER_THREADS;
                                cv[r][u] = e < tot ? __ldcg(Cp + e) : T(0);
                            }
                        }
#pragma unroll
                    for (int r = 0; r < 8; ++r)
                        if (r0 + r < world) {
#pragma unroll
                            for (int u = 0; u < UB; ++u) acc[u] += cv[r][u];
                        }
                }
#pragma unroll
                for (int u = 0; u < UB; ++u) {
                    const int e = e0 + u * PEER_THREADS;
                    if (e < tot) {
                        ctile[rr * LD + cc] = acc[u];
                        ftile[rr * LD + cc] = fv[u];
                    }
                    rr += dr; cc += dc;
                    while (cc >= k) { cc -= k; ++rr; }
                }
            }
        }
        __syncthreads();
        if (tid < nrow) tpr_solve_row<T, KM>(Ss, ctile, ftile, tid, k, reg_l1, reg_l2, eps, ub, has_ub != 0, unb);
        __syncthreads();
        {
            const int tot = nrow * k;
            for (int r = 0; r < world; ++r) {
                const int pr = (rank + r) % world;
                T* Frow = reinterpret_cast<T*>(px.Tt[pr]) + i0 * k;
                int rr = tid / k, cc = tid - rr * k;
                const int dr = PEER_THREADS / k, dc = PEER_THREADS - dr * k;
                for (int e = tid; e < tot; e += PEER_THREADS) {
                    Frow[e] = ftile[rr * LD + cc];
                    rr += dr; cc += dc;
                    while (cc >= k) { cc -= k; ++rr; }
                }
                T* Ft = reinterpret_cast<T*>(px.Tk[pr]);
                const int ii = tid % PEER_ROWS, tp0 = tid / PEER_ROWS;
                if (ii < nrow)
                    for (int tp = tp0; tp < k; tp += PEER_THREADS / PEER_ROWS) Ft[(int64_t)tp * px.ldtk + i0 + ii] = ftile[ii * LD + tp];
            }
            if (tid < k) {
                T cs = T(0);
#pragma unroll 8
                for (int ii = 0; ii < nrow; ++ii) cs += ftile[ii * LD + tid];
                csum += cs;
            }
        }
        __syncthreads();
    }
    if (unb) atomicOr(flags, 4);
    if (tid < k) colsum_part[(int64_t)blockIdx.x * k + tid] = csum;
    __threadfence_system();
    __syncthreads();
    if (tid == 0) s_arrival = atomicAdd(counter, 1u);
    __syncthreads();
    if (s_arrival != gridDim.x - 1) return;
    __threadfence();
    if (tid < k) {
        T s = T(0);
        for (int b = 0; b < (int)gridDim.x; ++b) s += __ldcg(colsum_part + (int64_t)b * k + tid);
        for (int r = 0; r < world; ++r) reinterpret_cast<T*>(px.tsum[r])[rank * k + tid] = s;
    }
    __threadfence_system();
    __syncthreads();
    if (tid < world) {
        __threadfence_system();
        peer_flag_store(px.flag2[tid] + 32 * rank, px.epoch);
    }
    peer_wait_all(px.flag2[rank], world, px.epoch, px.err);
    __syncthreads();
    if (tid < k) {
        const T* ts = reinterpret_cast<const T*>(px.tsum[rank]);
        T s = T(0);
        for (int r = 0; r < world; ++r) s += __ldcg(ts + r * k + tid);
        const double v = (double)s;
        sums[tid] = v;
        if (!(v > 1e-10)) atomicOr(flags, 1);
        if (!isfinite(v)) atomicOr(flags, 8);
    }
    if (tid == 0) *counter = 0u;
}

int peer_update_blocks(int64_t rows, int sm_count)
{
    int64_t b = (rows + PEER_ROWS - 1) / PEER_ROWS;
    if (b > 4 * sm_count) b = 4 * sm_count;
    return (int)(b < 1 ? 1 : b);
}

template <typename T>
int launch_peer_update_rows(const PeerExchange& px, int64_t d, int k, const SolveArgs& a, T* Gsum, T* colsum_part,
                            int* flags, double* sums, unsigned* counter, int blocks, cudaStream_t st)
{
    const bool ok = sizeof(T) == 4 ? k <= 128 : k <= 64;
    if (!ok) return 0;
    peer_gram_kernel<T><<<(k * k + 1023) / 1024, 256, 0, st>>>(px, d, k, Gsum);
#define RRI_PEER(KM)                                                                                                  \
    do {                                                                                                              \
        const size_t smem = sizeof(T) * ((size_t)KM * KM + 2 * (size_t)PEER_ROWS * (KM + 1));                         \
        auto kern = peer_update_rows_kernel<T, KM>;                                                                   \
        if (smem > 48 * 1024) cudaFuncSetAttribute(kern, cudaFuncAttributeMaxDynamicSharedMemorySize, (int)smem);     \
        kern<<<blocks, PEER_THREADS, smem, st>>>(px, d, k, Gsum, (T)a.reg_l1, (T)a.reg_l2, (T)a.eps, (T)a.ub,         \
                                                a.has_ub, colsum_part, flags, sums, counter);                         \
        return 2;                                                                                                     \
    } while (0)
    if (k <= 16) RRI_PEER(16);
    if (k <= 32) RRI_PEER(32);
    if (k <= 64) RRI_PEER(64);
    if constexpr (sizeof(T) == 4) { if (k <= 128) RRI_PEER(128); }
#undef RRI_PEER
    return 0;
}

template <typename T>
void launch_update_rows(T* F, int64_t m, int k, const T* Cpart, int parts, int64_t part_stride,
                        const T* const* srcs, const T* S, const SolveArgs& a, T* Ft, int64_t ldft,
                        T* colsum_part, int* flags, int blocks, const ColsumOut& co, cudaStream_t st)
{
    {
        static const bool reg_off = [] { const char* e = getenv("RRI_UPDATE_REG"); return e && *e == '0'; }();
        constexpr int VN = Vec<T>::N;
        if (!reg_off && parts == 1 && !srcs && Ft && (k % VN) == 0 && k <= (sizeof(T) == 4 ? 128 : 64)) {
            if (k <= 16) launch_update_rows_reg<T, 16>(F, m, k, Cpart, S, a, Ft, ldft, flags, co, st);
            else if (k <= 32) launch_update_rows_reg<T, 32>(F, m, k, Cpart, S, a, Ft, ldft, flags, co, st);
            else if (k <= 64) launch_update_rows_reg<T, 64>(F, m, k, Cpart, S, a, Ft, ldft, flags, co, st);
            else if constexpr (sizeof(T) == 4) launch_update_rows_reg<T, 128>(F, m, k, Cpart, S, a, Ft, ldft, flags, co, st);
            return;
        }
    }
#define RRI_TPR(KM) launch_update_rows_tpr<T, KM>(F, m, k, Cpart, parts, part_stride, srcs, S, a, Ft, ldft, colsum_part, flags, blocks, co, st)
    if (k <= 16) { RRI_TPR(16); return; }
    if (k <= 32) { RRI_TPR(32); return; }
    if (k <= 64) { RRI_TPR(64); return; }
    if (k <= 128 && sizeof(T) == 4) { RRI_TPR(128); return; }
#undef RRI_TPR
    const int kl = (k + 31) / 32;
    if (kl <= 1) launch_update_rows_kl<T, 1>(F, m, k, Cpart, parts, part_stride, srcs, S, a, Ft, ldft, colsum_part, flags, blocks, co, st);
    else if (kl <= 2) launch_update_rows_kl<T, 2>(F, m, k, Cpart, parts, part_stride, srcs, S, a, Ft, ldft, colsum_part, flags, blocks, co, st);
    else if (kl <= 4) launch_update_rows_kl<T, 4>(F, m, k, Cpart, parts, part_stride, srcs, S, a, Ft, ldft, colsum_part, flags, blocks, co, st);
    else launch_update_rows_kl<T, 8>(F, m, k, Cpart, parts, part_stride, srcs, S, a, Ft, ldft, colsum_part, flags, blocks, co, st);
}

constexpr int GR_ROWS = 32;

int gram_chunks(int64_t m, int k, int sm_count)
{
    const int kb = (k + 63) / 64;
    int64_t c = (2 * sm_count) / (kb * kb);
    const int64_t maxc = (m + 4 * GR_ROWS - 1) / (4 * GR_ROWS);
    if (c > maxc) c = maxc;
    return (int)(c < 1 ? 1 : c);
}

template <typename T>
__global__ void __launch_bounds__(256)
gram_kernel(const T* __restrict__ F, int64_t m, int k, T* __restrict__ part)
{
    __shared__ T Fa[GR_ROWS][64 + 1];
    __shared__ T Fb[GR_ROWS][64 + 1];
    const int kb = (k + 63) / 64;
    const int a0 = (blockIdx.y / kb) * 64, b0 = (blockIdx.y % kb) * 64;
    const int tid = threadIdx.x, tx = tid & 15, ty = tid >> 4;
    int64_t r0, r1;
    part_range(m, gridDim.x, blockIdx.x, r0, r1);
    T acc[4][4];
#pragma unroll
    for (int i = 0; i < 4; ++i)
#pragma unroll
        for (int j = 0; j < 4; ++j) acc[i][j] = T(0);
    for (int64_t rb = r0; rb < r1; rb += GR_ROWS) {
        {
            T va[GR_ROWS * 64 / 256], vb[GR_ROWS * 64 / 256];
#pragma unroll
            for (int u = 0; u < GR_ROWS * 64 / 256; ++u) {
                const int e = tid + u * 256;
                const int rr = e / 64, cc = e % 64;
                const int64_t gr = rb + rr;
                va[u] = (gr < r1 && a0 + cc < k) ? F[gr * k + a0 + cc] : T(0);
                vb[u] = (a0 == b0) ? va[u] : ((gr < r1 && b0 + cc < k) ? F[gr * k + b0 + cc] : T(0));
            }
#pragma unroll
            for (int u = 0; u < GR_ROWS * 64 / 256; ++u) {
                const int e = tid + u * 256;
                Fa[e / 64][e % 64] = va[u];
                Fb[e / 64][e % 64] = vb[u];
            }
        }
        __syncthreads();
#pragma unroll 8
        for (int rr = 0; rr < GR_ROWS; ++rr) {
            T a[4], b[4];
#pragma unroll
            for (int i = 0; i < 4; ++i) a[i] = Fa[rr][ty + 16 * i];
#pragma unroll
            for (int j = 0; j < 4; ++j) b[j] = Fb[rr][tx + 16 * j];
#pragma unroll
            for (int i = 0; i < 4; ++i)
#pragma unroll
                for (int j = 0; j < 4; ++j) acc[i][j] = fma(a[i], b[j], acc[i][j]);
        }
        __syncthreads();
    }
    T* P = part + (int64_t)blockIdx.x * k * k;
#pragma unroll
    for (int i = 0; i < 4; ++i)
#pragma unroll
        for (int j = 0; j < 4; ++j) {
            const int a = a0 + ty + 16 * i, b = b0 + tx + 16 * j;
            if (a < k && b < k) P[a * k + b] = acc[i][j];
        }
}

template <typename T>
__global__ void reduce_parts_kernel(const T* __restrict__ part, int parts, int64_t stride, int64_t len,
                                    T* __restrict__ out)
{
    const int64_t c = (int64_t)blockIdx.x * blockDim.x + threadIdx.x;
    if (c < len) {
        T s = T(0);
        for (int p = 0; p < parts; ++p) s += part[(int64_t)p * stride + c];
        out[c] = s;
    }
}

template <typename T>
__global__ void __launch_bounds__(256)
reduce_parts_warp_kernel(const T* __restrict__ part, int parts, int64_t stride, int64_t len, T* __restrict__ out)
{
    const int64_t c = ((int64_t)blockIdx.x * blockDim.x + threadIdx.x) >> 5;
    const int lane = threadIdx.x & 31;
    if (c >= len) return;
    T s = T(0);
    for (int p = lane; p < parts; p += 32) s += part[(int64_t)p * stride + c];
    s = warp_sum(s);
    if (lane == 0) out[c] = s;
}

template <typename T>
void launch_reduce_parts(const T* part, int parts, int64_t stride, int64_t len, T* out, cudaStream_t st)
{
    if (parts >= 16 && len <= 65536)
        reduce_parts_warp_kernel<T><<<(unsigned)((len * 32 + 255) / 256), 256, 0, st>>>(part, parts, stride, len, out);
    else
        reduce_parts_kernel<T><<<(unsigned)((len + 255) / 256), 256, 0, st>>>(part, parts, stride, len, out);
}

template <typename T>
__global__ void sum_sources_kernel(const T* const* __restrict__ srcs, int parts, int64_t len, T* __restrict__ out)
{
    const int64_t c = (int64_t)blockIdx.x * blockDim.x + threadIdx.x;
    if (c < len) {
        T s = T(0);
        for (int p = 0; p < parts; ++p) s += srcs[p][c];
        out[c] = s;
    }
}

template <typename T>
void launch_sum_sources(const T* const* srcs, int parts, int64_t len, T* out, cudaStream_t st)
{
    sum_sources_kernel<T><<<(unsigned)((len + 255) / 256), 256, 0, st>>>(srcs, parts, len, out);
}

template <typename T>
void launch_gram(const T* F, int64_t m, int k, T* part, int chunks, T* G, cudaStream_t st)
{
    const int kb = (k + 63) / 64;
    dim3 grid(chunks, kb * kb);
    gram_kernel<T><<<grid, 256, 0, st>>>(F, m, k, part);
    launch_reduce_parts<T>(part, chunks, (int64_t)k * k, (int64_t)k * k, G, st);
}

template <typename T>
__global__ void __launch_bounds__(256)
colsum_finalize_kernel(const T* __restrict__ colsum_part, int blocks, int k, double* __restrict__ sums,
                       int off, int zero_flag, int* __restrict__ flags)
{
    const int warp = (blockIdx.x * blockDim.x + threadIdx.x) >> 5, lane = threadIdx.x & 31;
    if (warp >= k) return;
    T s = T(0);
    for (int b = lane; b < blocks; b += 32) s += colsum_part[(int64_t)b * k + warp];
    s = warp_sum(s);
    if (lane == 0) {
        const double v = (double)s;
        sums[off + warp] = v;
        if (zero_flag && !(v > 1e-10)) atomicOr(flags, zero_flag);
        if (!isfinite(v)) atomicOr(flags, 8);
    }
}

template <typename T>
void launch_colsum_finalize(const T* colsum_part, int blocks, int k, double* sums, int off,
                            int zero_flag, int* flags, cudaStream_t st)
{
    colsum_finalize_kernel<T><<<(k * 32 + 255) / 256, 256, 0, st>>>(colsum_part, blocks, k, sums, off, zero_flag, flags);
}

template <typename T>
__global__ void __launch_bounds__(256)
transpose_kernel(const T* __restrict__ A, int64_t rows, int64_t cols, int64_t lda, T* __restrict__ B, int64_t ldb)
{
    __shared__ T tile[32][33];
    const int tx = threadIdx.x & 31, ty = threadIdx.x >> 5;
    const int64_t c0 = (int64_t)blockIdx.x * 32, r0 = (int64_t)blockIdx.y * 32;
#pragma unroll
    for (int j = 0; j < 32; j += 8) {
        const int64_t r = r0 + ty + j, c = c0 + tx;
        if (r < rows && c < cols) tile[ty + j][tx] = A[r * lda + c];
    }
    __syncthreads();
#pragma unroll
    for (int j = 0; j < 32; j += 8) {
        const int64_t c = c0 + ty + j, r = r0 + tx;
        if (r < rows && c < cols) B[c * ldb + r] = tile[tx][ty + j];
    }
}

template <typename T>
void launch_transpose(const T* A, int64_t rows, int64_t cols, int64_t lda, T* B, int64_t ldb, cudaStream_t st)
{
    const int64_t bx = (cols + 31) / 32, by = (rows + 31) / 32;
    if (by <= 65535) {
        dim3 grid((unsigned)bx, (unsigned)by);
        transpose_kernel<T><<<grid, 256, 0, st>>>(A, rows, cols, lda, B, ldb);
    } else {
        for (int64_t r = 0; r < rows; r += 65535LL * 32) {
            const int64_t rr = (rows - r) < 65535LL * 32 ? (rows - r) : 65535LL * 32;
            dim3 grid((unsigned)bx, (unsigned)((rr + 31) / 32));
            transpose_kernel<T><<<grid, 256, 0, st>>>(A + r * lda, rr, cols, lda, B + r, ldb);
        }
    }
}

#define RRI_INST(T)                                                                                       \
    template void launch_simt_gemm_nt<T>(const T*, int64_t, const T*, int64_t, T*, int64_t, int, int64_t, \
                                         int, cudaStream_t);                                              \
    template void launch_update_rows<T>(T*, int64_t, int, const T*, int, int64_t, const T* const*,        \
                                        const T*, const SolveArgs&, T*, int64_t, T*, int*, int,            \
                                        const ColsumOut&, cudaStream_t);                                   \
    template int launch_peer_update_rows<T>(const PeerExchange&, int64_t, int, const SolveArgs&, T*, T*,    \
                                            int*, double*, unsigned*, int, cudaStream_t);                  \
    template void launch_sum_sources<T>(const T* const*, int, int64_t, T*, cudaStream_t);                  \
    template void launch_gram<T>(const T*, int64_t, int, T*, int, T*, cudaStream_t);                      \
    template void launch_reduce_parts<T>(const T*, int, int64_t, int64_t, T*, cudaStream_t);              \
    template void launch_colsum_finalize<T>(const T*, int, int, double*, int, int, int*, cudaStream_t);   \
    template void launch_transpose<T>(const T*, int64_t, int64_t, int64_t, T*, int64_t, cudaStream_t);
RRI_INST(float)
RRI_INST(double)

}
```

### rri_nmf_b200/csrc/kernels.h

```cpp
#pragma once
#include <cuda_runtime.h>
#include <stdint.h>

namespace rri {

struct PassPlan {
    int vec;
    int nch;
    int ct;
    int rg;
    int64_t cw;
};
PassPlan plan_pass(int64_t n, int64_t d, int64_t ldx, const void* X, int elem_size, int sm_count);

template <typename T>
void launch_rri_pass(const T* X, int64_t ldx, int64_t n, int64_t d, const T* tvec, const T* W, int k,
                     int tn, T* ypart, T* ppart, bool do_y, bool do_p, const PassPlan& pl,
                     cudaStream_t st);

struct SolveArgs {
    double reg_l1, reg_l2, eps, ub;
    int has_ub;
};

int tstep_blocks(int64_t d);
int wstep_blocks(int64_t n, int sm_count);

template <typename T>
void launch_rri_tstep(T* Tm, int64_t d, int k, int t, const T* ppart, int rg, int64_t pstride,
                      const T* gpart, int gb, const SolveArgs& a, T* hpart, double* sums, int t_prev,
                      int* flags, bool do_update, cudaStream_t st);

template <typename T>
void launch_rri_wstep(T* W, int64_t n, int k, int t, int tn, const T* ypart, int ct, int64_t ystride,
                      const T* hpart, int hb, const SolveArgs& a, T* gpart, double* sums, int* flags,
                      bool do_update, int blocks, cudaStream_t st);

template <typename T>
void launch_reduce_stat(const T* ppart, int rg, int64_t d, const T* gpart, int gb, int k, T* stat,
                        cudaStream_t st);

template <typename T>
void launch_finalize_sums(const T* gpart, int gb, int k, int t_prev, double* sums, int* flags,
                          cudaStream_t st);

}

namespace rri {
int simt_gemm_splits(int64_t M, int64_t K, int sm_count);
template <typename T>
void launch_simt_gemm_nt(const T* A, int64_t lda, const T* B, int64_t ldb, T* Cpart, int64_t M, int N,
                         int64_t K, int splits, cudaStream_t st);

int update_rows_blocks(int64_t m, int sm_count);
struct ColsumOut {
    double* sums;
    int off, zero_flag;
    unsigned* counter;
};
template <typename T>
void launch_update_rows(T* F, int64_t m, int k, const T* Cpart, int parts, int64_t part_stride,
                        const T* const* srcs, const T* S, const SolveArgs& a, T* Ft, int64_t ldft,
                        T* colsum_part, int* flags, int blocks, const ColsumOut& co, cudaStream_t st);

struct PeerExchange {
    int world, rank;
    unsigned epoch;
    int64_t row_lo, row_hi;
    int64_t ldtk;
    const void* part[16];
    void* Tt[16];
    void* Tk[16];
    void* tsum[16];
    unsigned* flag1[16];
    unsigned* flag2[16];
    int* err;
};
int peer_update_blocks(int64_t rows, int sm_count);
template <typename T>
int launch_peer_update_rows(const PeerExchange& px, int64_t d, int k, const SolveArgs& a, T* Gsum, T* colsum_part,
                            int* flags, double* sums, unsigned* counter, int blocks, cudaStream_t st);

template <typename T>
void launch_sum_sources(const T* const* srcs, int parts, int64_t len, T* out, cudaStream_t st);

int gram_chunks(int64_t m, int k, int sm_count);
template <typename T>
void launch_gram(const T* F, int64_t m, int k, T* part, int chunks, T* G, cudaStream_t st);

template <typename T>
void launch_reduce_parts(const T* part, int parts, int64_t stride, int64_t len, T* out, cudaStream_t st);

template <typename T>
void launch_colsum_finalize(const T* colsum_part, int blocks, int k, double* sums, int off,
                            int zero_flag, int* flags, cudaStream_t st);

template <typename T>
void launch_transpose(const T* A, int64_t rows, int64_t cols, int64_t lda, T* B, int64_t ldb,
                      cudaStream_t st);

void launch_x16_scan(const float* X, int64_t rows, int64_t cols, int64_t ld, unsigned* out, int sm_count, cudaStream_t st);
bool x16_exponent(const unsigned scan[3], int* e);
void launch_x16_copy(const float* X, int64_t rows, int64_t cols, int64_t ldx, int e, void* Y, int64_t ldy, void* Yt,
                     int64_t ldyt, cudaStream_t st);
int f16_factor_parts(int sm_count);
void launch_f16_factor(const float* F, int rows, int64_t cols, int64_t ld, unsigned* part, int nparts, void* out,
                       int64_t ldo, int* e_out, cudaStream_t st);
}

namespace rri {
enum { MK_NONE = 0, MK_REAL = 1, MK_U8 = 2, MK_SPARSE = 3  };

struct TilePlan { int tiles_r, tiles_c, groups; };
TilePlan plan_tstats(int64_t n, int64_t d, int sm_count);
TilePlan plan_wstats(int64_t n, int64_t d, int sm_count);

template <typename T>
void launch_wrri_tstats(const T* X, int64_t ldx, const void* M, int mk, int64_t ldm, const T* W,
                        const T* Tm, int64_t n, int64_t d, int k, int t, T* numer_part, T* denom_part,
                        const TilePlan& pl, cudaStream_t st);
template <typename T>
void launch_wrri_wstats(const T* X, int64_t ldx, const void* M, int mk, int64_t ldm, const T* W,
                        const T* Tm, int64_t n, int64_t d, int k, int t, T* numer_part, T* denom_part,
                        const TilePlan& pl, cudaStream_t st);
template <typename T>
void launch_wrri_final(const T* numer_part, const T* denom_part, int parts, int64_t len,
                       const SolveArgs& a, T* out, int64_t out_stride, T* out2, int64_t out2_stride,
                       int* flags, cudaStream_t st);
template <typename T>
void launch_vec_sum_flag(const T* v, int64_t len, int64_t stride, double* sums, int slot, int zero_flag,
                         int* flags, cudaStream_t st);
template <typename T>
void launch_rowsum_flag(const T* A, int rows, int64_t len, int64_t ld, double* sums, int slot0, int zero_flag,
                        int* flags, cudaStream_t st);
template <typename T>
void launch_vec_scale_to_sum(T* v, int64_t len, int64_t stride, const double* sums, int slot, double s,
                             cudaStream_t st);

int obj_blocks(int64_t n, int64_t d, int sm_count);
template <typename T>
void launch_objective(const T* X, int64_t ldx, const void* M, int mk, int64_t ldm, const T* W,
                      const T* Tm, int64_t n, int64_t d, int k, double* part, int blocks, double* out,
                      cudaStream_t st);
template <typename T>
void launch_sumsq_rows(const T* A, int64_t rows, int64_t cols, int64_t lda, double* part, double* out, int sm_count,
                       cudaStream_t st);
template <typename T>
void launch_dot_parts(const T* C, int parts, int64_t stride, const T* W, int64_t len, double* part, double* out,
                      int sm_count, cudaStream_t st);
template <typename T>
void launch_objective_identity(const T* G, const T* H, int k, const double* acc, double* out, cudaStream_t st);
template <typename T>
void launch_norms(const T* v, int64_t len, double* part, double* out, cudaStream_t st);
}

namespace rri {
void launch_flag_from_sums(const double* sums, int off, int k, int zero_flag, int* flags, cudaStream_t st);

template <typename T>
void launch_project_rows_simplex(T* A, int64_t rows, int64_t cols, double s, cudaStream_t st);

int simplex_T_slots(int64_t d);
template <typename T>
int launch_simplex_T_update(T* Tt, int64_t d, int k, const T* C, int parts, int64_t pstride, const T* G, const SolveArgs& a,
                            double s, T* Tout, int64_t ldo, double* slots, int* flags, int sm_count, bool allow_fused,
                            int* launches, cudaStream_t st);
}

namespace rri {
struct SpSide {
    int64_t nseg;
    const int64_t* ptr;
    const int32_t* idx;
    const void* x;
    const void* wgt;
    void* E;
    int group;
    const int64_t* ptr2;
    int nblk, nb;
    int64_t nother;
    const uint16_t* idx16;
};
int sp_block_len(int elem_size, int64_t nother, int* nblk_out);
void launch_sp_local_index(const int32_t* idx, int64_t nnz, int nb, uint16_t* out, int sm_count, cudaStream_t st);
void launch_sp_subptr(const int64_t* ptr, const int32_t* idx, int64_t nseg, int nblk, int nb, int64_t* ptr2,
                      int sm_count, cudaStream_t st);

template <typename T>
int sp_build_csc(const int64_t* rowptr, const int32_t* col, const T* x, const T* w, int64_t n, int64_t d,
                 int64_t nnz, int64_t* colptr, int32_t* csc_row, T* x_csc, T* w_csc, uint32_t* perm, int sm_count,
                 int* err_dev, cudaStream_t st);

template <typename T>
void launch_sp_residual(const SpSide& s, const T* A, const T* B, int k, int sm_count, cudaStream_t st);

template <typename T>
void launch_sp_residual_rows(const SpSide& s, const T* A, int64_t lda, const T* B, int ldb, int k, int sm_count,
                             cudaStream_t st);
template <typename T>
void launch_sp_gather(const uint32_t* perm, const T* src, T* dst, int64_t nnz, int sm_count, cudaStream_t st);

template <typename T>
void launch_sp_pack(const T* po, const T* pn, const T* vold, const T* vnew, void* quad, int64_t len, cudaStream_t st);

template <typename T>
int launch_sp_pass(const SpSide& s, const void* quad, const T* own_po, const T* own_pn, const T* own_cur,
                    T* own_save, T* numer, T* denom, int sm_count, cudaStream_t st);

template <typename T>
void launch_sp_objective(const SpSide& s, int64_t nnz, double* part, double* out, cudaStream_t st);
}

namespace rri {
constexpr int SPMM_CHUNK = 1024;
constexpr int SPMM_PANEL = 256;
struct SpmmPlan {
    int64_t nseg;
    const int64_t* ptr;
    const int32_t* idx;
    const void* val;
    int64_t nlong_items;
    const int2* litem;
    const int32_t* lseg;
    const int64_t* lslot;
    void* slots;
    unsigned* counters;
};
template <typename T>
void launch_spmm(const SpmmPlan& p, const T* B, int64_t ldb, int width, T* C, int64_t ldc, cudaStream_t st);
template <typename T>
void launch_spmm_weighted_values(const T* x, const T* w, int64_t nnz, T* out, int sm_count, cudaStream_t st);

struct SparsePassPlan {
    int gy, gp;
    int blocks;
    int blocks_y, blocks_p;
};
template <typename T>
SparsePassPlan plan_sparse_rri_pass(const SpmmPlan& rows, const SpmmPlan& cols, int64_t nnz, int sm_count);
template <typename T>
void launch_sparse_rri_pass(const SparsePassPlan& pl, const SpmmPlan& rows, const SpmmPlan& cols, const T* trow,
                            const T* W, int k, int tn, T* y, T* p, bool do_y, bool do_p, cudaStream_t st);
}
```

### rri_nmf_b200/csrc/x16_kernels.cu

```cuda
#include <cuda_fp16.h>

#include "kernels.h"

namespace rri {

namespace {

__device__ __forceinline__ float to_tf32(float x)
{
    const uint32_t b = __float_as_uint(x);
    if ((b & 0x7f800000u) == 0x7f800000u) return x;
    return __uint_as_float((b + 0xfffu + ((b >> 13) & 1u)) & ~0x1fffu);
}

__device__ __forceinline__ float pow2(int e) { return __int_as_float((127 + e) << 23); }

__global__ void x16_scan_kernel(const float* __restrict__ X, int64_t rows, int64_t cols, int64_t ld, unsigned* out)
{
    unsigned mx = 0u, mn = 0xffffffffu, bad = 0u;
    for (int64_t r = blockIdx.x; r < rows; r += gridDim.x) {
        const float* row = X + r * ld;
        for (int64_t c = threadIdx.x; c < cols; c += blockDim.x) {
            const unsigned b = __float_as_uint(fabsf(to_tf32(__ldcs(row + c))));
            if (b >= 0x7f800000u) bad = 1u;
            else {
                mx = b > mx ? b : mx;
                if (b) mn = b < mn ? b : mn;
            }
        }
    }
    mx = __reduce_max_sync(0xffffffffu, mx);
    mn = __reduce_min_sync(0xffffffffu, mn);
    bad = __reduce_or_sync(0xffffffffu, bad);
    if ((threadIdx.x & 31) == 0) {
        if (mx) atomicMax(out + 0, mx);
        if (mn != 0xffffffffu) atomicMin(out + 1, mn);
        if (bad) atomicOr(out + 2, bad);
    }
}

__global__ void x16_copy_kernel(const float* __restrict__ X, int64_t rows, int64_t cols, int64_t ldx, int e,
                                __half* __restrict__ Y, int64_t ldy, __half* __restrict__ Yt, int64_t ldyt)
{
    __shared__ __half tile[32][34];
    const int64_t c0 = (int64_t)blockIdx.x * 32, r0 = (int64_t)blockIdx.y * 32;
    const int tx = threadIdx.x & 31, ty = threadIdx.x >> 5;
    const float s = pow2(e);
    for (int i = ty; i < 32; i += 8) {
        const int64_t r = r0 + i, c = c0 + tx;
        if (r < rows && c < cols) {
            const __half h = __float2half_rn(to_tf32(X[r * ldx + c]) * s);
            Y[r * ldy + c] = h;
            tile[i][tx] = h;
        }
    }
    __syncthreads();
    for (int i = ty; i < 32; i += 8) {
        const int64_t c = c0 + i, r = r0 + tx;
        if (r < rows && c < cols) Yt[c * ldyt + r] = tile[tx][i];
    }
}

__device__ __forceinline__ int factor_exp(unsigned m)
{
    if (m == 0u || m >= 0x7f800000u) return 0;
    const int e = 15 - ((int)(m >> 23) - 127);
    return e < -126 ? -126 : (e > 126 ? 126 : e);
}

__device__ __forceinline__ unsigned block_max(unsigned v, unsigned* sh)
{
    v = __reduce_max_sync(0xffffffffu, v);
    if ((threadIdx.x & 31) == 0) sh[threadIdx.x >> 5] = v;
    __syncthreads();
    if (threadIdx.x < 32) {
        unsigned w = threadIdx.x < (blockDim.x >> 5) ? sh[threadIdx.x] : 0u;
        w = __reduce_max_sync(0xffffffffu, w);
        if (threadIdx.x == 0) sh[32] = w;
    }
    __syncthreads();
    return sh[32];
}

__global__ void f16_absmax_kernel(const float* __restrict__ F, int rows, int64_t cols, int64_t ld, unsigned* __restrict__ part)
{
    __shared__ unsigned sh[33];
    unsigned m = 0u;
    for (int r = 0; r < rows; ++r)
        for (int64_t c = (int64_t)blockIdx.x * blockDim.x + threadIdx.x; c < cols; c += (int64_t)gridDim.x * blockDim.x) {
            const unsigned b = __float_as_uint(fabsf(to_tf32(F[(int64_t)r * ld + c])));
            m = b > m ? b : m;
        }
    m = block_max(m, sh);
    if (threadIdx.x == 0) part[blockIdx.x] = m;
}

__global__ void f16_factor_kernel(const float* __restrict__ F, int rows, int64_t cols, int64_t ld,
                                  const unsigned* __restrict__ part, int nparts, __half* __restrict__ out, int64_t ldo,
                                  int* __restrict__ e_out)
{
    __shared__ unsigned sh[33];
    unsigned m = 0u;
    for (int i = threadIdx.x; i < nparts; i += blockDim.x) m = part[i] > m ? part[i] : m;
    const int e = factor_exp(block_max(m, sh));
    const float s = pow2(e);
    for (int r = 0; r < rows; ++r)
        for (int64_t c = (int64_t)blockIdx.x * blockDim.x + threadIdx.x; c < cols; c += (int64_t)gridDim.x * blockDim.x)
            out[(int64_t)r * ldo + c] = __float2half_rn(to_tf32(F[(int64_t)r * ld + c]) * s);
    if (blockIdx.x == 0 && threadIdx.x == 0) *e_out = e;
}

}

void launch_x16_scan(const float* X, int64_t rows, int64_t cols, int64_t ld, unsigned* out, int sm_count, cudaStream_t st)
{
    cudaMemsetAsync(out, 0, 3 * sizeof(unsigned), st);
    cudaMemsetAsync(out + 1, 0xff, sizeof(unsigned), st);
    const int64_t blocks = rows < (int64_t)sm_count * 8 ? rows : (int64_t)sm_count * 8;
    x16_scan_kernel<<<(unsigned)blocks, 512, 0, st>>>(X, rows, cols, ld, out);
}

bool x16_exponent(const unsigned scan[3], int* e)
{
    const unsigned mx = scan[0], mn = scan[1];
    *e = 0;
    if (scan[2]) return false;
    if (mx == 0u) return true;
    if (mn < 0x00800000u) return false;
    const int emax = (int)(mx >> 23) - 127, emin = (int)(mn >> 23) - 127;
    int s = 15 - emax;
    if (s > 126) s = 126;
    *e = s;
    return emin + s >= -14;
}

void launch_x16_copy(const float* X, int64_t rows, int64_t cols, int64_t ldx, int e, void* Y, int64_t ldy, void* Yt,
                     int64_t ldyt, cudaStream_t st)
{
    const int64_t bx = (cols + 31) / 32;
    for (int64_t r = 0; r < rows; r += 65535LL * 32) {
        const int64_t rr = (rows - r) < 65535LL * 32 ? (rows - r) : 65535LL * 32;
        dim3 grid((unsigned)bx, (unsigned)((rr + 31) / 32));
        x16_copy_kernel<<<grid, 256, 0, st>>>(X + r * ldx, rr, cols, ldx, e, (__half*)Y + r * ldy, ldy, (__half*)Yt + r, ldyt);
    }
}

int f16_factor_parts(int sm_count) { return 4 * sm_count < 1024 ? 4 * sm_count : 1024; }

void launch_f16_factor(const float* F, int rows, int64_t cols, int64_t ld, unsigned* part, int nparts, void* out,
                       int64_t ldo, int* e_out, cudaStream_t st)
{
    f16_absmax_kernel<<<nparts, 256, 0, st>>>(F, rows, cols, ld, part);
    f16_factor_kernel<<<nparts, 256, 0, st>>>(F, rows, cols, ld, part, nparts, (__half*)out, ldo, e_out);
}

}
```

Baseline: 354.0.

## Use per-128-column fp16 factor groups and convert factors inside the row updates

Replaces the global two-kernel absmax+convert of the factor matrix with a single kernel that scales each 128-column group with its own exponent. The fp16 copy of W/T is now produced right after the factor update (fused into update_rows where possible) and stored persistently, so the contraction reuses it instead of re-converting. The GEMM MMA and epilogue loops are restructured so accumulation runs break at exponent-group boundaries (pairs of K chunks), and the per-group exponent is applied in the epilogue. This removes a grid-wide reduction pass and redundant conversions, at the cost of more TMEM accumulator flushes and extra workspace.

```diff
diff --git a/rri_nmf_b200/csrc/api.cu b/rri_nmf_b200/csrc/api.cu
--- a/rri_nmf_b200/csrc/api.cu
+++ b/rri_nmf_b200/csrc/api.cu
@@ -131,8 +131,9 @@
     void* Xt_ext = nullptr; int64_t ldxt_ext = 0;
     bool x16 = false; int x_exp = 0;
     void *X16 = nullptr, *Xt16 = nullptr; int64_t ldx16 = 0, ldxt16 = 0;
-    void* F16 = nullptr;
-    unsigned *x16_scan = nullptr, *f16_part = nullptr; int* f16_exp = nullptr;
+    F16Out t16{}, w16{};
+    void* F16 = nullptr; int* f16_exp = nullptr;
+    unsigned* x16_scan = nullptr;
     void *Wt = nullptr, *Tt = nullptr, *Cpart = nullptr, *cg = nullptr , *Hm = nullptr;
     void *gram_part = nullptr, *colsum_part = nullptr;
     int splits_t = 1, splits_w = 1, ub_blocks_t = 1, ub_blocks_w = 1, gchunks_w = 1, gchunks_t = 1;
@@ -499,9 +500,7 @@
             std::string err;
             h->tf32 = tf32_gemm_create(h->sm_count, k + 16 < 256 ? k + 16 : 256, err);
             if (!h->tf32) return fail("tf32 contraction unavailable: %s", err.c_str());
-            if (ws_alloc(h, (void**)&h->x16_scan, 4 * sizeof(unsigned)) || ws_alloc(h, (void**)&h->f16_exp, sizeof(int)) ||
-                ws_alloc(h, (void**)&h->f16_part, sizeof(unsigned) * (size_t)f16_factor_parts(h->sm_count)))
-                return 1;
+            if (ws_alloc(h, (void**)&h->x16_scan, 4 * sizeof(unsigned))) return 1;
             CK(cudaStreamSynchronize(0));
         }
     }
@@ -539,7 +538,15 @@
             if (!h->F16) {
                 const int64_t m = n > d ? n : d;
                 const int rows = k + 16 < 256 ? k + 16 : 256;
-                if (ws_alloc(h, &h->F16, 2 * (size_t)rows * (size_t)((m + 7) / 8 * 8))) return 1;
+                h->t16.ld = (d + 7) / 8 * 8;
+                h->w16.ld = (n + 7) / 8 * 8;
+                if (ws_alloc(h, &h->F16, 2 * (size_t)rows * (size_t)((m + 7) / 8 * 8)) ||
+                    ws_alloc(h, (void**)&h->f16_exp, sizeof(int) * (size_t)((m + 127) / 128)) ||
+                    ws_alloc(h, &h->t16.out, 2 * (size_t)k * (size_t)h->t16.ld) ||
+                    ws_alloc(h, (void**)&h->t16.exp, sizeof(int) * (size_t)((d + 127) / 128)) ||
+                    ws_alloc(h, &h->w16.out, 2 * (size_t)k * (size_t)h->w16.ld) ||
+                    ws_alloc(h, (void**)&h->w16.exp, sizeof(int) * (size_t)((n + 127) / 128)))
+                    return 1;
                 CK(cudaStreamSynchronize(0));
             }
             h->X16 = h->Xt; h->ldx16 = ldx16;
@@ -987,23 +994,32 @@
     return h->math == RRI_MATH_TF32 && !off;
 }
 
+static const F16Out* factor16(rri_handle_t h, bool w) { return h->x16 ? (w ? &h->w16 : &h->t16) : nullptr; }
+
+static void convert_factor16(rri_handle_t h, const float* B, int N, int64_t K, int64_t ldb, const F16Out& f, cudaStream_t st)
+{
+    launch_f16_groups(B, N, K, ldb, f.out, f.ld, f.exp, st);
+    h->launches++;
+}
+
 template <typename T>
 static int data_contraction(rri_handle_t h, bool transpose, const T* B, int64_t ldb, int N, T* C, cudaStream_t st,
-                            T* G = nullptr, bool convert = true)
+                            T* G = nullptr, const F16Out* b16 = nullptr)
 {
     const int64_t M = transpose ? h->d : h->n, K = transpose ? h->n : h->d;
     if (!h->x16)
         return transpose ? contraction<T>(h, (const T*)h->Xt, h->ldxt, B, ldb, C, M, N, K, h->splits_t, st, G)
                          : contraction<T>(h, (const T*)h->X, h->ldx, B, ldb, C, M, N, K, h->splits_w, st, G);
-    const int64_t ldf = (K + 7) / 8 * 8;
-    if (convert) {
-        launch_f16_factor((const float*)B, N, K, ldb, h->f16_part, f16_factor_parts(h->sm_count), h->F16, ldf, h->f16_exp, st);
-        h->launches += 2;
-    }
-    const __half* F = (const __half*)h->F16;
+    F16Out scratch{h->F16, (K + 7) / 8 * 8, h->f16_exp};
+    if (!b16) {
+        convert_factor16(h, (const float*)B, N, K, ldb, scratch, st);
+        b16 = &scratch;
+    }
+    const __half* F = (const __half*)b16->out;
+    const int64_t ldf = b16->ld;
     std::string err;
     const int nl = f16_gemm_run(h->tf32, (const __half*)(transpose ? h->Xt16 : h->X16), transpose ? h->ldxt16 : h->ldx16,
-                                h->x_exp, F, ldf, h->f16_exp, (float*)C, N, M, N, K, st, err, G ? F : nullptr, ldf, G ? N : 0,
+                                h->x_exp, F, ldf, b16->exp, (float*)C, N, M, N, K, st, err, G ? F : nullptr, ldf, G ? N : 0,
                                 (float*)G, N);
     if (nl < 0) return fail("16-bit contraction failed: %s", err.c_str());
     h->launches += nl;
@@ -1021,15 +1037,15 @@
         if (h->zero_csr) {
             launch_spmm<T>(h->zrow, (const T*)h->Tt, k, k, (T*)h->Cpart, k, st);
             h->launches++;
-        } else if (data_contraction<T>(h, false, Tk, ldtk, k, (T*)h->Cpart, st, tc_gram ? (T*)h->Hm : nullptr)) {
+        } else if (data_contraction<T>(h, false, Tk, ldtk, k, (T*)h->Cpart, st, tc_gram ? (T*)h->Hm : nullptr,
+                                       factor16(h, false))) {
             return 1;
         }
     }
     const int parts = h->math == RRI_MATH_TF32 ? 1 : h->splits_w;
-    launch_update_rows<T>(W, n, k, (const T*)h->Cpart, parts, n * k, nullptr, (const T*)h->Hm, solve_args(p, false),
-                          (T*)h->Wt, h->ldwt, (T*)h->colsum_part, h->flags, h->ub_blocks_w,
-                          ColsumOut{nullptr, k, 0, h->counters + 0}, st);
-    h->launches++;
+    h->launches += launch_update_rows<T>(W, n, k, (const T*)h->Cpart, parts, n * k, nullptr, (const T*)h->Hm,
+                                         solve_args(p, false), (T*)h->Wt, h->ldwt, (T*)h->colsum_part, h->flags,
+                                         h->ub_blocks_w, ColsumOut{nullptr, k, 0, h->counters + 0}, st, factor16(h, true));
     CKL();
     return 0;
 }
@@ -1050,7 +1066,8 @@
         T* myG = myC + (size_t)d * k;
         if (!tc_gram) { launch_gram<T>(W, n, k, (T*)h->gram_part, h->gchunks_w, myG, st); h->launches += 2; }
         T* Cdst = psplits == 1 ? myC : (T*)h->Cpart;
-        if (data_contraction<T>(h, true, (const T*)h->Wt, h->ldwt, k, Cdst, st, tc_gram ? myG : nullptr)) return 1;
+        if (data_contraction<T>(h, true, (const T*)h->Wt, h->ldwt, k, Cdst, st, tc_gram ? myG : nullptr, factor16(h, true)))
+            return 1;
         if (psplits > 1) { launch_reduce_parts<T>((const T*)h->Cpart, psplits, d * k, d * k, myC, st); h->launches++; }
         const PeerExchange px = peer_args(h, e);
         const int blocks = peer_update_blocks(px.row_hi - px.row_lo, h->sm_count);
@@ -1058,6 +1075,7 @@
                                                   h->counters + 1, blocks, st);
         if (!nl) return fail("the fused peer-memory T update does not support k = %d", k);
         h->launches += nl;
+        if (h->x16) convert_factor16(h, (const float*)Tk, k, d, ldtk, h->t16, st);
         CKL();
         return 0;
     }
@@ -1066,7 +1084,7 @@
     if (h->zero_csr) {
         launch_spmm<T>(h->zcol, W, k, k, Cout, k, st);
         h->launches++;
-    } else if (data_contraction<T>(h, true, (const T*)h->Wt, h->ldwt, k, Cout, st, tc_gram ? G : nullptr)) {
+    } else if (data_contraction<T>(h, true, (const T*)h->Wt, h->ldwt, k, Cout, st, tc_gram ? G : nullptr, factor16(h, true))) {
         return 1;
     }
     const T* C = Cout;
@@ -1083,11 +1101,12 @@
                                                   ldtk, h->sx_slots, h->flags, h->sm_count, !(e && *e == '0'), &nl, st);
         if (rc) return fail("constrained T update failed: %s", cudaGetErrorString((cudaError_t)rc));
         h->launches += nl;
+        if (h->x16) convert_factor16(h, (const float*)Tk, k, d, ldtk, h->t16, st);
         return 0;
     }
-    launch_update_rows<T>((T*)h->Tt, d, k, C, parts, d * k, nullptr, G, solve_args(p, true), Tk, ldtk, (T*)h->colsum_part,
-                          h->flags, h->ub_blocks_t, ColsumOut{nullptr, 0, 0, h->counters + 2}, st);
-    h->launches++;
+    h->launches += launch_update_rows<T>((T*)h->Tt, d, k, C, parts, d * k, nullptr, G, solve_args(p, true), Tk, ldtk,
+                                         (T*)h->colsum_part, h->flags, h->ub_blocks_t,
+                                         ColsumOut{nullptr, 0, 0, h->counters + 2}, st, factor16(h, false));
     CKL();
     return 0;
 }
@@ -1366,6 +1385,7 @@
     if (p->fix_T) {
         launch_transpose<T>(Tm, k, d, d, (T*)h->Tt, k, st);
         h->launches++;
+        if (h->x16) convert_factor16(h, (const float*)Tm, k, d, d, h->t16, st);
         for (int s = 0; s < n_sweeps; ++s)
             if (hals_W_half<T>(h, W, Tm, d, p, s == 0, st)) return 1;
         return n_sweeps > 0 ? hals_finish_sums<T>(h, Tm, false, st) : 0;
@@ -1374,6 +1394,7 @@
         launch_transpose<T>(Tm, k, d, d, (T*)h->Tt, k, st);
         launch_transpose<T>(W, n, k, k, (T*)h->Wt, h->ldwt, st);
         h->launches += 2;
+        if (h->x16) convert_factor16(h, (const float*)h->Wt, k, n, h->ldwt, h->w16, st);
         const bool px = h->world > 1 && h->p2p;
         T* Tk = px ? (T*)((char*)h->xbuf + h->x_off_tk) : Tm;
         const int64_t ldtk = px ? h->ldtk : d;
@@ -1762,7 +1783,9 @@
     if (which == 2 && h->mk == MK_NONE && h->order == RRI_ORDER_HALS) {
         launch_transpose<T>(W, n, k, k, (T*)h->Wt, h->ldwt, st);
         h->launches++;
-    }
+        if (h->x16) convert_factor16(h, (const float*)h->Wt, k, n, h->ldwt, h->w16, st);
+    }
+    if (which == 1 && h->x16) convert_factor16(h, (const float*)Tm, k, d, d, h->t16, st);
     if (which == 1 && h->zero_csr) {
         launch_transpose<T>(Tm, k, d, d, (T*)h->Tt, k, st);
         h->launches++;
@@ -1783,6 +1806,8 @@
             CK(cudaMemcpy2DAsync(Tk, (size_t)ldtk * sizeof(T), Tm, (size_t)d * sizeof(T), (size_t)d * sizeof(T), (size_t)k,
                                  cudaMemcpyDeviceToDevice, st));
         }
+        if (h->x16 && which == 3) convert_factor16(h, (const float*)h->Wt, k, n, h->ldwt, h->w16, st);
+        if (h->x16 && which == 4) convert_factor16(h, (const float*)Tk, k, d, ldtk, h->t16, st);
     }
     SpState spS;
     if (which == 5 || which == 6) {
@@ -1812,11 +1837,11 @@
         } else if (which == 1) {
             if (h->mk != MK_NONE) return fail("which=1 needs an unmasked handle");
             if (h->zero_csr) { launch_spmm<T>(h->zrow, (const T*)h->Tt, k, k, (T*)h->Cpart, k, st); h->launches++; continue; }
-            if (data_contraction<T>(h, false, Tm, d, k, (T*)h->Cpart, st, nullptr, it < 0)) return 1;
+            if (data_contraction<T>(h, false, Tm, d, k, (T*)h->Cpart, st, nullptr, factor16(h, false))) return 1;
         } else if (which == 2) {
             if (h->mk != MK_NONE || h->order != RRI_ORDER_HALS) return fail("which=2 needs an unmasked hals-order handle");
             if (h->zero_csr) { launch_spmm<T>(h->zcol, W, k, k, (T*)h->Cpart, k, st); h->launches++; continue; }
-            if (data_contraction<T>(h, true, (const T*)h->Wt, h->ldwt, k, (T*)h->Cpart, st, nullptr, it < 0)) return 1;
+            if (data_contraction<T>(h, true, (const T*)h->Wt, h->ldwt, k, (T*)h->Cpart, st, nullptr, factor16(h, true))) return 1;
         } else if (which == 3) {
             if (hals_T_half<T>(h, const_cast<T*>(W), Tk, ldtk, &prm, st)) return 1;
         } else if (which == 4) {
diff --git a/rri_nmf_b200/csrc/common.cuh b/rri_nmf_b200/csrc/common.cuh
--- a/rri_nmf_b200/csrc/common.cuh
+++ b/rri_nmf_b200/csrc/common.cuh
@@ -51,4 +51,20 @@
     return x;
 }
 
+RRI_DEVINL float to_tf32(float x)
+{
+    const uint32_t b = __float_as_uint(x);
+    if ((b & 0x7f800000u) == 0x7f800000u) return x;
+    return __uint_as_float((b + 0xfffu + ((b >> 13) & 1u)) & ~0x1fffu);
 }
+
+RRI_DEVINL float pow2(int e) { return __int_as_float((127 + e) << 23); }
+
+RRI_DEVINL int factor_exp(unsigned m)
+{
+    if (m == 0u || m >= 0x7f800000u) return 0;
+    const int e = 15 - ((int)(m >> 23) - 127);
+    return e < -126 ? -126 : (e > 126 ? 126 : e);
+}
+
+}
diff --git a/rri_nmf_b200/csrc/gemm_tf32_sm100.cu b/rri_nmf_b200/csrc/gemm_tf32_sm100.cu
--- a/rri_nmf_b200/csrc/gemm_tf32_sm100.cu
+++ b/rri_nmf_b200/csrc/gemm_tf32_sm100.cu
@@ -39,6 +39,26 @@
     const int* b_exp;
 };
 
+template <bool F16>
+__device__ __forceinline__ bool run_starts(int64_t i, int64_t kc, bool down, int flush)
+{
+    if (F16) return i == 0 || (kc & 1) == (down ? 1 : 0);
+    return i % flush == 0;
+}
+__device__ __forceinline__ int64_t segment_first_kc(const GemmParams& p, int64_t u, int64_t u_end)
+{
+    const int64_t kc0 = u % p.nk;
+    const int64_t len = (u_end - u) < (p.nk - kc0) ? (u_end - u) : (p.nk - kc0);
+    return (p.reverse_tail && kc0 != 0) ? kc0 + len - 1 : kc0;
+}
+template <bool F16>
+__device__ __forceinline__ bool run_ends(int64_t i, int64_t len, int64_t kc, bool down, int flush)
+{
+    if (i == len - 1) return true;
+    if (F16) return (kc & 1) == (down ? 0 : 1);
+    return (i + 1) % flush == 0;
+}
+
 using namespace tc;
 
 __host__ __device__ __forceinline__ int64_t part_start(int64_t units, int parts, int64_t c)
@@ -126,33 +146,39 @@
             for (int64_t u = u_begin; u < u_end;) {
                 const int64_t kc0 = u % p.nk;
                 const int64_t len = (u_end - u) < (p.nk - kc0) ? (u_end - u) : (p.nk - kc0);
-                for (int64_t i0 = 0; i0 < len; i0 += p.flush, ++run) {
-                    const int64_t i1 = (i0 + p.flush) < len ? (i0 + p.flush) : len;
-                    const uint32_t b = p.nbuf == 2 ? (run & 1u) : 0u;
-                    const uint32_t use = p.nbuf == 2 ? (run >> 1) : run;
-                    mbar_wait(&tempty[b], (use & 1u) ^ 1u, err, 2);
+                const bool down = p.reverse_tail && kc0 != 0;
+                uint32_t b = 0, tacc = 0;
+                for (int64_t i = 0; i < len; ++i) {
+                    const int64_t kc = down ? (kc0 + len - 1 - i) : (kc0 + i);
+                    const bool first = run_starts<F16>(i, kc, down, p.flush);
+                    if (first) {
+                        b = p.nbuf == 2 ? (run & 1u) : 0u;
+                        const uint32_t use = p.nbuf == 2 ? (run >> 1) : run;
+                        mbar_wait(&tempty[b], (use & 1u) ^ 1u, err, 2);
+                        tc_fence_after();
+                        tacc = tmem_base + b * (uint32_t)(MT * NPAD);
+                    }
+                    mbar_wait(&full[stage], phase, err, 3);
                     tc_fence_after();
-                    const uint32_t tacc = tmem_base + b * (uint32_t)(MT * NPAD);
-                    for (int64_t i = i0; i < i1; ++i) {
-                        mbar_wait(&full[stage], phase, err, 3);
-                        tc_fence_after();
-                        const uint32_t a0 = smem_u32(smA + (size_t)stage * a_stage);
-                        const uint32_t b0 = smem_u32(smB + (size_t)stage * b_stage);
-#pragma unroll
-                        for (int mt = 0; mt < MT; ++mt) {
-#pragma unroll
-                            for (int ks = 0; ks < BKE / UK; ++ks) {
-                                const uint64_t ad = make_desc(a0 + mt * A_TILE_BYTES + ks * 32);
-                                const uint64_t bd = make_desc(b0 + ks * 32);
-                                const uint32_t accum = (i > i0 || ks > 0) ? 1u : 0u;
-                                if (F16) umma_f16(tacc + (uint32_t)(mt * NPAD), ad, bd, idesc, accum);
-                                else umma_tf32(tacc + (uint32_t)(mt * NPAD), ad, bd, idesc, accum);
-                            }
+                    const uint32_t a0 = smem_u32(smA + (size_t)stage * a_stage);
+                    const uint32_t b0 = smem_u32(smB + (size_t)stage * b_stage);
+#pragma unroll
+                    for (int mt = 0; mt < MT; ++mt) {
+#pragma unroll
+                        for (int ks = 0; ks < BKE / UK; ++ks) {
+                            const uint64_t ad = make_desc(a0 + mt * A_TILE_BYTES + ks * 32);
+                            const uint64_t bd = make_desc(b0 + ks * 32);
+                            const uint32_t accum = (!first || ks > 0) ? 1u : 0u;
+                            if (F16) umma_f16(tacc + (uint32_t)(mt * NPAD), ad, bd, idesc, accum);
+                            else umma_tf32(tacc + (uint32_t)(mt * NPAD), ad, bd, idesc, accum);
                         }
-                        umma_commit(&empty[stage]);
-                        if (++stage == p.stages) { stage = 0; phase ^= 1; }
-                    }
-                    umma_commit(&tfull[b]);
+                    }
+                    umma_commit(&empty[stage]);
+                    if (++stage == p.stages) { stage = 0; phase ^= 1; }
+                    if (run_ends<F16>(i, len, kc, down, p.flush)) {
+                        umma_commit(&tfull[b]);
+                        ++run;
+                    }
                 }
                 u += len;
             }
@@ -166,15 +192,31 @@
         float acc[NACC];
         uint32_t run = 0;
         const int64_t slot_elems = (int64_t)MT * BM * p.N;
+        int e_run = (F16 && u_begin < u_end) ? __ldg(p.b_exp + (segment_first_kc(p, u_begin, u_end) >> 1)) : 0;
         for (int64_t u = u_begin; u < u_end;) {
-            const int64_t s = u / p.nk, kc0 = u % p.nk;
-            const int64_t len = (u_end - u) < (p.nk - kc0) ? (u_end - u) : (p.nk - kc0);
+            const int64_t s = u / p.nk;
+            const int kc0 = (int)(u % p.nk);
+            const int len = (int)((u_end - u) < (p.nk - kc0) ? (u_end - u) : (p.nk - kc0));
             const bool complete = (len == p.nk);
+            const bool aux = s >= p.n_super_main;
+            const bool down = p.reverse_tail && kc0 != 0;
 #pragma unroll
             for (int i = 0; i < NACC; ++i) acc[i] = 0.f;
-            for (int64_t i0 = 0; i0 < len; i0 += p.flush, ++run) {
+            for (int i = 0; i < len;) {
+                const int kc = down ? (kc0 + len - 1 - i) : (kc0 + i);
+                int nr = F16 ? (down ? (kc & 1) + 1 : 2 - (kc & 1)) : p.flush;
+                nr = nr < len - i ? nr : len - i;
+                i += nr;
                 const uint32_t b = p.nbuf == 2 ? (run & 1u) : 0u;
                 const uint32_t use = p.nbuf == 2 ? (run >> 1) : run;
+                ++run;
+                float s1 = 1.f, s2 = 1.f;
+                if (F16) {
+                    const int ea = aux ? e_run : p.a_exp;
+                    const int e = ea + e_run;
+                    if (e >= -127 && e <= 126) s1 = __int_as_float((127 - e) << 23);
+                    else { s1 = __int_as_float((127 - ea) << 23); s2 = __int_as_float((127 - e_run) << 23); }
+                }
                 mbar_wait(&tfull[b], use & 1u, err, 4);
                 tc_fence_after();
                 const uint32_t tacc = tmem_base + ((uint32_t)(q * 32) << 16) + b * (uint32_t)(MT * NPAD) + (uint32_t)(h * HC);
@@ -185,19 +227,21 @@
                         float v[16];
                         tmem_ld16(tacc + (uint32_t)(mt * NPAD + c0), v);
 #pragma unroll
-                        for (int j = 0; j < 16; ++j) acc[mt * HC + c0 + j] += v[j];
+                        for (int j = 0; j < 16; ++j) {
+                            if (F16) acc[mt * HC + c0 + j] = fmaf(v[j] * s2, s1, acc[mt * HC + c0 + j]);
+                            else acc[mt * HC + c0 + j] += v[j];
+                        }
                     }
                 }
                 tc_fence_before();
                 __syncwarp();
                 if (lane == 0) mbar_arrive(&tempty[b]);
-            }
-            const bool aux = s >= p.n_super_main;
-            if (F16) {
-                const float sb = __int_as_float((127 - *p.b_exp) << 23);
-                const float sa = aux ? sb : __int_as_float((127 - p.a_exp) << 23);
-#pragma unroll
-                for (int i = 0; i < NACC; ++i) acc[i] = acc[i] * sa * sb;
+                if (F16) {
+                    int64_t kn = -1;
+                    if (i < len) kn = down ? kc - nr : kc + nr;
+                    else if (u + len < u_end) kn = segment_first_kc(p, u + len, u_end);
+                    if (kn >= 0) e_run = __ldg(p.b_exp + (kn >> 1));
+                }
             }
             float* out = aux ? p.C2 : p.C;
             const int64_t out_ld = aux ? p.ldc2 : p.ldc;
@@ -399,7 +443,7 @@
     int cols = 32;
     while (cols < p.nbuf * MT * NPAD) cols <<= 1;
     p.tmem_cols = cols;
-    p.flush = g->flush > 0 ? (F16 ? (g->flush + 1) / 2 : g->flush) : (1 << 30);
+    p.flush = g->flush > 0 ? g->flush : (1 << 30);
     p.reverse_tail = g->reverse_tail >= 0 ? g->reverse_tail : (NPAD >= 128 ? 1 : 0);
     int64_t grid = p.units < g->sm_count ? p.units : g->sm_count;
     constexpr int EWQ = NPAD >= 128 ? 4 : 2;
@@ -474,7 +518,7 @@
                  float* C, int64_t ldc, int64_t M, int N, int64_t K, cudaStream_t st, std::string& err, const __half* A2,
                  int64_t lda2, int M2, float* C2, int64_t ldc2)
 {
-    if (!b_exp) { err = "16-bit contraction without the factor's scale"; return -1; }
+    if (!b_exp) { err = "16-bit contraction without the factor's scales"; return -1; }
     return gemm_run(g, true, A, lda, a_exp, B, ldb, b_exp, C, ldc, M, N, K, st, err, A2, lda2, M2, C2, ldc2);
 }
 
diff --git a/rri_nmf_b200/csrc/hals_kernels.cu b/rri_nmf_b200/csrc/hals_kernels.cu
--- a/rri_nmf_b200/csrc/hals_kernels.cu
+++ b/rri_nmf_b200/csrc/hals_kernels.cu
@@ -1,3 +1,5 @@
+#include <cuda_fp16.h>
+
 #include "common.cuh"
 #include "kernels.h"
 
@@ -524,13 +526,71 @@
 }
 
 template <int KM>
+__device__ __forceinline__ void update_row_x2(unsigned long long (&fp)[KM / 2], const float* __restrict__ crow,
+                                              const float* __restrict__ Ss, int k, float reg_l1, float reg_l2, float eps,
+                                              float ub, int has_ub, bool& unb)
+{
+    using U64 = unsigned long long;
+    const float4* crowv = reinterpret_cast<const float4*>(crow);
+    float cn[8];
+#pragma unroll
+    for (int v = 0; v < 2; ++v) {
+        float4 cv = make_float4(0.f, 0.f, 0.f, 0.f);
+        if (4 * v < k) cv = crowv[v];
+        cn[4 * v] = cv.x; cn[4 * v + 1] = cv.y; cn[4 * v + 2] = cv.z; cn[4 * v + 3] = cv.w;
+    }
+#pragma unroll 1
+    for (int c = 0; c < (k + 7) / 8; ++c) {
+        float cc[8];
+#pragma unroll
+        for (int u = 0; u < 8; ++u) cc[u] = cn[u];
+#pragma unroll
+        for (int v = 0; v < 2; ++v) {
+            const int jv = 2 * (c + 1) + v;
+            if (4 * jv < k) {
+                const float4 cv = crowv[jv];
+                cn[4 * v] = cv.x; cn[4 * v + 1] = cv.y; cn[4 * v + 2] = cv.z; cn[4 * v + 3] = cv.w;
+            }
+        }
+#pragma unroll
+        for (int u = 0; u < 8; ++u) {
+            const int t = 8 * c + u;
+            if (t < k) {
+                const ulonglong2* srow = reinterpret_cast<const ulonglong2*>(Ss + t * KM);
+                U64 a01 = 0ull, a23 = 0ull;
+#pragma unroll
+                for (int jv = 0; jv < KM / 4; ++jv) {
+                    const ulonglong2 sv = srow[jv];
+                    ffma2(a01, fp[2 * jv], sv.x);
+                    ffma2(a23, fp[2 * jv + 1], sv.y);
+                }
+                U64 fpair = fp[u / 2];
+#pragma unroll
+                for (int jj = 1; jj < KM / 8; ++jj) fpair = (jj == c) ? fp[4 * jj + u / 2] : fpair;
+                const float ft = (u & 1) ? hi_f(fpair) : lo_f(fpair);
+                const float stt = Ss[t * KM + t];
+                const float dot = ((lo_f(a01) + hi_f(a01)) + (lo_f(a23) + hi_f(a23))) - ft * stt;
+                const float x = solve_scalar_c<float>(cc[u] - dot - reg_l1, stt + reg_l2, eps, ub, has_ub != 0, unb);
+#pragma unroll
+                for (int jj = 0; jj < KM / 8; ++jj) {
+                    const U64 old = fp[4 * jj + u / 2];
+                    const U64 upd = (u & 1) ? pack_f(lo_f(old), x) : pack_f(x, hi_f(old));
+                    fp[4 * jj + u / 2] = (jj == c) ? upd : old;
+                }
+            }
+        }
+    }
+}
+
+template <int KM>
 __global__ void __launch_bounds__(128)
 update_rows_reg_x2_kernel(float* __restrict__ F, int64_t m, int k, const float* __restrict__ C, const float* __restrict__ S,
                           float reg_l1, float reg_l2, float eps, float ub, int has_ub, float* __restrict__ Ft, int64_t ldft,
-                          int* __restrict__ flags)
+                          int* __restrict__ flags, __half* __restrict__ h16, int64_t ldh16, int* __restrict__ h16_exp)
 {
     using U64 = unsigned long long;
     extern __shared__ __align__(16) unsigned char smem_raw[];
+    __shared__ unsigned wmax[4];
     float* Ss = reinterpret_cast<float*>(smem_raw);
     const int tid = threadIdx.x;
     for (int e = tid; e < KM * KM; e += 128) {
@@ -539,80 +599,61 @@
     }
     __syncthreads();
     bool unb = false;
-    for (int64_t row = (int64_t)blockIdx.x * 128 + tid; row < m; row += (int64_t)gridDim.x * 128) {
+    for (int64_t row0 = (int64_t)blockIdx.x * 128; row0 < m; row0 += (int64_t)gridDim.x * 128) {
+        const int64_t row = row0 + tid;
         U64 fp[KM / 2];
-        const ulonglong2* frowv = reinterpret_cast<const ulonglong2*>(F + row * k);
-#pragma unroll
-        for (int jv = 0; jv < KM / 4; ++jv) {
-            ulonglong2 v = make_ulonglong2(0ull, 0ull);
-            if (4 * jv < k) v = frowv[jv];
-            fp[2 * jv] = v.x; fp[2 * jv + 1] = v.y;
-        }
-        const float4* crowv = reinterpret_cast<const float4*>(C + row * k);
-        float cn[8];
-#pragma unroll
-        for (int v = 0; v < 2; ++v) {
-            float4 cv = make_float4(0.f, 0.f, 0.f, 0.f);
-            if (4 * v < k) cv = crowv[v];
-            cn[4 * v] = cv.x; cn[4 * v + 1] = cv.y; cn[4 * v + 2] = cv.z; cn[4 * v + 3] = cv.w;
-        }
-#pragma unroll 1
-        for (int c = 0; c < (k + 7) / 8; ++c) {
-            float cc[8];
-#pragma unroll
-            for (int u = 0; u < 8; ++u) cc[u] = cn[u];
-#pragma unroll
-            for (int v = 0; v < 2; ++v) {
-                const int jv = 2 * (c + 1) + v;
-                if (4 * jv < k) {
-                    const float4 cv = crowv[jv];
-                    cn[4 * v] = cv.x; cn[4 * v + 1] = cv.y; cn[4 * v + 2] = cv.z; cn[4 * v + 3] = cv.w;
-                }
-            }
-#pragma unroll
-            for (int u = 0; u < 8; ++u) {
-                const int t = 8 * c + u;
-                if (t < k) {
-                    const ulonglong2* srow = reinterpret_cast<const ulonglong2*>(Ss + t * KM);
-                    U64 a01 = 0ull, a23 = 0ull;
-#pragma unroll
-                    for (int jv = 0; jv < KM / 4; ++jv) {
-                        const ulonglong2 sv = srow[jv];
-                        ffma2(a01, fp[2 * jv], sv.x);
-                        ffma2(a23, fp[2 * jv + 1], sv.y);
+        if (row < m) {
+            const ulonglong2* frowv = reinterpret_cast<const ulonglong2*>(F + row * k);
+#pragma unroll
+            for (int jv = 0; jv < KM / 4; ++jv) {
+                ulonglong2 v = make_ulonglong2(0ull, 0ull);
+                if (4 * jv < k) v = frowv[jv];
+                fp[2 * jv] = v.x; fp[2 * jv + 1] = v.y;
+            }
+            update_row_x2<KM>(fp, C + row * k, Ss, k, reg_l1, reg_l2, eps, ub, has_ub, unb);
+            ulonglong2* fout = reinterpret_cast<ulonglong2*>(F + row * k);
+#pragma unroll
+            for (int jv = 0; jv < KM / 4; ++jv)
+                if (4 * jv < k) fout[jv] = make_ulonglong2(fp[2 * jv], fp[2 * jv + 1]);
+            if (Ft) {
+#pragma unroll
+                for (int t = 0; t < KM; ++t)
+                    if (t < k) Ft[(int64_t)t * ldft + row] = (t & 1) ? hi_f(fp[t / 2]) : lo_f(fp[t / 2]);
+            }
+        }
+        if (h16) {
+            unsigned mx = 0u;
+            if (row < m) {
+#pragma unroll
+                for (int t = 0; t < KM; ++t)
+                    if (t < k) {
+                        const unsigned b = __float_as_uint(fabsf(to_tf32((t & 1) ? hi_f(fp[t / 2]) : lo_f(fp[t / 2]))));
+                        mx = b > mx ? b : mx;
                     }
-                    U64 fpair = fp[u / 2];
-#pragma unroll
-                    for (int jj = 1; jj < KM / 8; ++jj) fpair = (jj == c) ? fp[4 * jj + u / 2] : fpair;
-                    const float ft = (u & 1) ? hi_f(fpair) : lo_f(fpair);
-                    const float stt = Ss[t * KM + t];
-                    const float dot = ((lo_f(a01) + hi_f(a01)) + (lo_f(a23) + hi_f(a23))) - ft * stt;
-                    const float x = solve_scalar_c<float>(cc[u] - dot - reg_l1, stt + reg_l2, eps, ub, has_ub != 0, unb);
-#pragma unroll
-                    for (int jj = 0; jj < KM / 8; ++jj) {
-                        const U64 old = fp[4 * jj + u / 2];
-                        const U64 upd = (u & 1) ? pack_f(lo_f(old), x) : pack_f(x, hi_f(old));
-                        fp[4 * jj + u / 2] = (jj == c) ? upd : old;
-                    }
-                }
-            }
-        }
-        ulonglong2* fout = reinterpret_cast<ulonglong2*>(F + row * k);
-#pragma unroll
-        for (int jv = 0; jv < KM / 4; ++jv)
-            if (4 * jv < k) fout[jv] = make_ulonglong2(fp[2 * jv], fp[2 * jv + 1]);
-        if (Ft) {
-#pragma unroll
-            for (int t = 0; t < KM; ++t)
-                if (t < k) Ft[(int64_t)t * ldft + row] = (t & 1) ? hi_f(fp[t / 2]) : lo_f(fp[t / 2]);
+            }
+            mx = __reduce_max_sync(0xffffffffu, mx);
+            if ((tid & 31) == 0) wmax[tid >> 5] = mx;
+            __syncthreads();
+            mx = wmax[0];
+#pragma unroll
+            for (int w = 1; w < 4; ++w) mx = wmax[w] > mx ? wmax[w] : mx;
+            const int e = factor_exp(mx);
+            if (tid == 0) h16_exp[row0 / 128] = e;
+            const float sc = pow2(e);
+            if (row < m) {
+#pragma unroll
+                for (int t = 0; t < KM; ++t)
+                    if (t < k) h16[(int64_t)t * ldh16 + row] = __float2half_rn(to_tf32((t & 1) ? hi_f(fp[t / 2]) : lo_f(fp[t / 2])) * sc);
+            }
+            __syncthreads();
         }
     }
     if (unb) atomicOr(flags, 4);
 }
 
 template <typename T, int KM>
-static void launch_update_rows_reg(T* F, int64_t m, int k, const T* C, const T* S, const SolveArgs& a, T* Ft, int64_t ldft,
-                                   int* flags, const ColsumOut& co, cudaStream_t st)
+static int launch_update_rows_reg(T* F, int64_t m, int k, const T* C, const T* S, const SolveArgs& a, T* Ft, int64_t ldft,
+                                  int* flags, const ColsumOut& co, cudaStream_t st, const F16Out* h16, bool& wrote16)
 {
     const size_t smem = sizeof(T) * KM * KM;
     const int64_t nb = (m + 127) / 128;
@@ -621,15 +662,18 @@
         if (x2) {
             auto kx = update_rows_reg_x2_kernel<KM>;
             if (smem > 48 * 1024) cudaFuncSetAttribute(kx, cudaFuncAttributeMaxDynamicSharedMemorySize, (int)smem);
-            kx<<<(unsigned)nb, 128, smem, st>>>(F, m, k, C, S, (T)a.reg_l1, (T)a.reg_l2, (T)a.eps, (T)a.ub, a.has_ub, Ft, ldft, flags);
+            kx<<<(unsigned)nb, 128, smem, st>>>(F, m, k, C, S, (T)a.reg_l1, (T)a.reg_l2, (T)a.eps, (T)a.ub, a.has_ub, Ft, ldft, flags,
+                                                h16 ? (__half*)h16->out : nullptr, h16 ? h16->ld : 0, h16 ? h16->exp : nullptr);
             if (co.sums) launch_rowsum_flag<T>(Ft, k, m, ldft, co.sums, co.off, co.zero_flag, flags, st);
-            return;
+            wrote16 = h16 != nullptr;
+            return co.sums ? 2 : 1;
         }
     }
     auto kern = update_rows_reg_kernel<T, KM>;
     if (smem > 48 * 1024) cudaFuncSetAttribute(kern, cudaFuncAttributeMaxDynamicSharedMemorySize, (int)smem);
     kern<<<(unsigned)nb, 128, smem, st>>>(F, m, k, C, S, (T)a.reg_l1, (T)a.reg_l2, (T)a.eps, (T)a.ub, a.has_ub, Ft, ldft, flags);
     if (co.sums) launch_rowsum_flag<T>(Ft, k, m, ldft, co.sums, co.off, co.zero_flag, flags, st);
+    return co.sums ? 2 : 1;
 }
 
 __device__ __forceinline__ void peer_flag_store(unsigned* p, unsigned v)
@@ -861,32 +905,50 @@
 }
 
 template <typename T>
-void launch_update_rows(T* F, int64_t m, int k, const T* Cpart, int parts, int64_t part_stride,
-                        const T* const* srcs, const T* S, const SolveArgs& a, T* Ft, int64_t ldft,
-                        T* colsum_part, int* flags, int blocks, const ColsumOut& co, cudaStream_t st)
+static int launch_update_rows_any(T* F, int64_t m, int k, const T* Cpart, int parts, int64_t part_stride,
+                                  const T* const* srcs, const T* S, const SolveArgs& a, T* Ft, int64_t ldft,
+                                  T* colsum_part, int* flags, int blocks, const ColsumOut& co, cudaStream_t st,
+                                  const F16Out* h16, bool& wrote16)
 {
     {
         static const bool reg_off = [] { const char* e = getenv("RRI_UPDATE_REG"); return e && *e == '0'; }();
         constexpr int VN = Vec<T>::N;
         if (!reg_off && parts == 1 && !srcs && Ft && (k % VN) == 0 && k <= (sizeof(T) == 4 ? 128 : 64)) {
-            if (k <= 16) launch_update_rows_reg<T, 16>(F, m, k, Cpart, S, a, Ft, ldft, flags, co, st);
-            else if (k <= 32) launch_update_rows_reg<T, 32>(F, m, k, Cpart, S, a, Ft, ldft, flags, co, st);
-            else if (k <= 64) launch_update_rows_reg<T, 64>(F, m, k, Cpart, S, a, Ft, ldft, flags, co, st);
-            else if constexpr (sizeof(T) == 4) launch_update_rows_reg<T, 128>(F, m, k, Cpart, S, a, Ft, ldft, flags, co, st);
-            return;
+            if (k <= 16) return launch_update_rows_reg<T, 16>(F, m, k, Cpart, S, a, Ft, ldft, flags, co, st, h16, wrote16);
+            if (k <= 32) return launch_update_rows_reg<T, 32>(F, m, k, Cpart, S, a, Ft, ldft, flags, co, st, h16, wrote16);
+            if (k <= 64) return launch_update_rows_reg<T, 64>(F, m, k, Cpart, S, a, Ft, ldft, flags, co, st, h16, wrote16);
+            if constexpr (sizeof(T) == 4) return launch_update_rows_reg<T, 128>(F, m, k, Cpart, S, a, Ft, ldft, flags, co, st, h16, wrote16);
+            return 0;
         }
     }
 #define RRI_TPR(KM) launch_update_rows_tpr<T, KM>(F, m, k, Cpart, parts, part_stride, srcs, S, a, Ft, ldft, colsum_part, flags, blocks, co, st)
-    if (k <= 16) { RRI_TPR(16); return; }
-    if (k <= 32) { RRI_TPR(32); return; }
-    if (k <= 64) { RRI_TPR(64); return; }
-    if (k <= 128 && sizeof(T) == 4) { RRI_TPR(128); return; }
+    if (k <= 16) { RRI_TPR(16); return 1; }
+    if (k <= 32) { RRI_TPR(32); return 1; }
+    if (k <= 64) { RRI_TPR(64); return 1; }
+    if (k <= 128 && sizeof(T) == 4) { RRI_TPR(128); return 1; }
 #undef RRI_TPR
     const int kl = (k + 31) / 32;
     if (kl <= 1) launch_update_rows_kl<T, 1>(F, m, k, Cpart, parts, part_stride, srcs, S, a, Ft, ldft, colsum_part, flags, blocks, co, st);
     else if (kl <= 2) launch_update_rows_kl<T, 2>(F, m, k, Cpart, parts, part_stride, srcs, S, a, Ft, ldft, colsum_part, flags, blocks, co, st);
     else if (kl <= 4) launch_update_rows_kl<T, 4>(F, m, k, Cpart, parts, part_stride, srcs, S, a, Ft, ldft, colsum_part, flags, blocks, co, st);
     else launch_update_rows_kl<T, 8>(F, m, k, Cpart, parts, part_stride, srcs, S, a, Ft, ldft, colsum_part, flags, blocks, co, st);
+    return 1;
+}
+
+template <typename T>
+int launch_update_rows(T* F, int64_t m, int k, const T* Cpart, int parts, int64_t part_stride,
+                       const T* const* srcs, const T* S, const SolveArgs& a, T* Ft, int64_t ldft,
+                       T* colsum_part, int* flags, int blocks, const ColsumOut& co, cudaStream_t st, const F16Out* h16)
+{
+    bool wrote16 = false;
+    const int nl = launch_update_rows_any<T>(F, m, k, Cpart, parts, part_stride, srcs, S, a, Ft, ldft, colsum_part, flags,
+                                             blocks, co, st, h16, wrote16);
+    if (wrote16 || !h16) return nl;
+    if constexpr (sizeof(T) == 4) {
+        launch_f16_groups(Ft, k, m, ldft, h16->out, h16->ld, h16->exp, st);
+        return nl + 1;
+    }
+    return nl;
 }
 
 constexpr int GR_ROWS = 32;
@@ -1083,9 +1145,9 @@
 #define RRI_INST(T)                                                                                       \
     template void launch_simt_gemm_nt<T>(const T*, int64_t, const T*, int64_t, T*, int64_t, int, int64_t, \
                                          int, cudaStream_t);                                              \
-    template void launch_update_rows<T>(T*, int64_t, int, const T*, int, int64_t, const T* const*,        \
-                                        const T*, const SolveArgs&, T*, int64_t, T*, int*, int,            \
-                                        const ColsumOut&, cudaStream_t);                                   \
+    template int launch_update_rows<T>(T*, int64_t, int, const T*, int, int64_t, const T* const*,         \
+                                       const T*, const SolveArgs&, T*, int64_t, T*, int*, int,             \
+                                       const ColsumOut&, cudaStream_t, const F16Out*);                     \
     template int launch_peer_update_rows<T>(const PeerExchange&, int64_t, int, const SolveArgs&, T*, T*,    \
                                             int*, double*, unsigned*, int, cudaStream_t);                  \
     template void launch_sum_sources<T>(const T* const*, int, int64_t, T*, cudaStream_t);                  \
diff --git a/rri_nmf_b200/csrc/kernels.h b/rri_nmf_b200/csrc/kernels.h
--- a/rri_nmf_b200/csrc/kernels.h
+++ b/rri_nmf_b200/csrc/kernels.h
@@ -58,10 +58,16 @@
     int off, zero_flag;
     unsigned* counter;
 };
-template <typename T>
-void launch_update_rows(T* F, int64_t m, int k, const T* Cpart, int parts, int64_t part_stride,
-                        const T* const* srcs, const T* S, const SolveArgs& a, T* Ft, int64_t ldft,
-                        T* colsum_part, int* flags, int blocks, const ColsumOut& co, cudaStream_t st);
+struct F16Out {
+    void* out;
+    int64_t ld;
+    int* exp;
+};
+template <typename T>
+int launch_update_rows(T* F, int64_t m, int k, const T* Cpart, int parts, int64_t part_stride,
+                       const T* const* srcs, const T* S, const SolveArgs& a, T* Ft, int64_t ldft,
+                       T* colsum_part, int* flags, int blocks, const ColsumOut& co, cudaStream_t st,
+                       const F16Out* h16 = nullptr);
 
 struct PeerExchange {
     int world, rank;
@@ -103,9 +109,7 @@
 bool x16_exponent(const unsigned scan[3], int* e);
 void launch_x16_copy(const float* X, int64_t rows, int64_t cols, int64_t ldx, int e, void* Y, int64_t ldy, void* Yt,
                      int64_t ldyt, cudaStream_t st);
-int f16_factor_parts(int sm_count);
-void launch_f16_factor(const float* F, int rows, int64_t cols, int64_t ld, unsigned* part, int nparts, void* out,
-                       int64_t ldo, int* e_out, cudaStream_t st);
+void launch_f16_groups(const float* F, int rows, int64_t cols, int64_t ld, void* out, int64_t ldo, int* e_out, cudaStream_t st);
 }
 
 namespace rri {
diff --git a/rri_nmf_b200/csrc/x16_kernels.cu b/rri_nmf_b200/csrc/x16_kernels.cu
--- a/rri_nmf_b200/csrc/x16_kernels.cu
+++ b/rri_nmf_b200/csrc/x16_kernels.cu
@@ -1,19 +1,11 @@
 #include <cuda_fp16.h>
 
+#include "common.cuh"
 #include "kernels.h"
 
 namespace rri {
 
 namespace {
-
-__device__ __forceinline__ float to_tf32(float x)
-{
-    const uint32_t b = __float_as_uint(x);
-    if ((b & 0x7f800000u) == 0x7f800000u) return x;
-    return __uint_as_float((b + 0xfffu + ((b >> 13) & 1u)) & ~0x1fffu);
-}
-
-__device__ __forceinline__ float pow2(int e) { return __int_as_float((127 + e) << 23); }
 
 __global__ void x16_scan_kernel(const float* __restrict__ X, int64_t rows, int64_t cols, int64_t ld, unsigned* out)
 {
@@ -61,53 +53,29 @@
     }
 }
 
-__device__ __forceinline__ int factor_exp(unsigned m)
+__global__ void __launch_bounds__(256) f16_groups_kernel(const float* __restrict__ F, int rows, int64_t cols, int64_t ld,
+                                                         __half* __restrict__ out, int64_t ldo, int* __restrict__ e_out)
 {
-    if (m == 0u || m >= 0x7f800000u) return 0;
-    const int e = 15 - ((int)(m >> 23) - 127);
-    return e < -126 ? -126 : (e > 126 ? 126 : e);
-}
-
-__device__ __forceinline__ unsigned block_max(unsigned v, unsigned* sh)
-{
-    v = __reduce_max_sync(0xffffffffu, v);
-    if ((threadIdx.x & 31) == 0) sh[threadIdx.x >> 5] = v;
-    __syncthreads();
-    if (threadIdx.x < 32) {
-        unsigned w = threadIdx.x < (blockDim.x >> 5) ? sh[threadIdx.x] : 0u;
-        w = __reduce_max_sync(0xffffffffu, w);
-        if (threadIdx.x == 0) sh[32] = w;
-    }
-    __syncthreads();
-    return sh[32];
-}
-
-__global__ void f16_absmax_kernel(const float* __restrict__ F, int rows, int64_t cols, int64_t ld, unsigned* __restrict__ part)
-{
-    __shared__ unsigned sh[33];
+    __shared__ unsigned sh[8];
+    const int64_t c = (int64_t)blockIdx.x * 128 + (threadIdx.x & 127);
+    const int r0 = threadIdx.x >> 7;
     unsigned m = 0u;
-    for (int r = 0; r < rows; ++r)
-        for (int64_t c = (int64_t)blockIdx.x * blockDim.x + threadIdx.x; c < cols; c += (int64_t)gridDim.x * blockDim.x) {
+    if (c < cols)
+        for (int r = r0; r < rows; r += 2) {
             const unsigned b = __float_as_uint(fabsf(to_tf32(F[(int64_t)r * ld + c])));
             m = b > m ? b : m;
         }
-    m = block_max(m, sh);
-    if (threadIdx.x == 0) part[blockIdx.x] = m;
-}
-
-__global__ void f16_factor_kernel(const float* __restrict__ F, int rows, int64_t cols, int64_t ld,
-                                  const unsigned* __restrict__ part, int nparts, __half* __restrict__ out, int64_t ldo,
-                                  int* __restrict__ e_out)
-{
-    __shared__ unsigned sh[33];
-    unsigned m = 0u;
-    for (int i = threadIdx.x; i < nparts; i += blockDim.x) m = part[i] > m ? part[i] : m;
-    const int e = factor_exp(block_max(m, sh));
+    m = __reduce_max_sync(0xffffffffu, m);
+    if ((threadIdx.x & 31) == 0) sh[threadIdx.x >> 5] = m;
+    __syncthreads();
+    m = sh[0];
+#pragma unroll
+    for (int w = 1; w < 8; ++w) m = sh[w] > m ? sh[w] : m;
+    const int e = factor_exp(m);
     const float s = pow2(e);
-    for (int r = 0; r < rows; ++r)
-        for (int64_t c = (int64_t)blockIdx.x * blockDim.x + threadIdx.x; c < cols; c += (int64_t)gridDim.x * blockDim.x)
-            out[(int64_t)r * ldo + c] = __float2half_rn(to_tf32(F[(int64_t)r * ld + c]) * s);
-    if (blockIdx.x == 0 && threadIdx.x == 0) *e_out = e;
+    if (c < cols)
+        for (int r = r0; r < rows; r += 2) out[(int64_t)r * ldo + c] = __float2half_rn(to_tf32(F[(int64_t)r * ld + c]) * s);
+    if (threadIdx.x == 0) e_out[blockIdx.x] = e;
 }
 
 }
@@ -145,13 +113,9 @@
     }
 }
 
-int f16_factor_parts(int sm_count) { return 4 * sm_count < 1024 ? 4 * sm_count : 1024; }
-
-void launch_f16_factor(const float* F, int rows, int64_t cols, int64_t ld, unsigned* part, int nparts, void* out,
-                       int64_t ldo, int* e_out, cudaStream_t st)
+void launch_f16_groups(const float* F, int rows, int64_t cols, int64_t ld, void* out, int64_t ldo, int* e_out, cudaStream_t st)
 {
-    f16_absmax_kernel<<<nparts, 256, 0, st>>>(F, rows, cols, ld, part);
-    f16_factor_kernel<<<nparts, 256, 0, st>>>(F, rows, cols, ld, part, nparts, (__half*)out, ldo, e_out);
+    f16_groups_kernel<<<(unsigned)((cols + 127) / 128), 256, 0, st>>>(F, rows, cols, ld, (__half*)out, ldo, e_out);
 }
 
 }
```

Measured after the change: 365.1 (median of 6 runs). 3.1% higher.
